# lucieDLE/TMRNet

Measured on AMD Instinct MI355X. Metric: train frames/sec, TMRNet ResNet50 seq=10 LFB=40, higher is better.
Workload: dtype fp32; 1 GPU; C2/C3: TMRNet ResNet50+LSTM+NLBlock train step; model=resnet_lstm (train_only_non-local_pretrained), global_batch=64, clips_per_gpu=64, seq_len=10, lfb_len=40, parallelism=dp1, input_transform=reference train transform (use_flip=1) on device

## Files before the change

include/tmr.h:

```cpp
#ifndef TMR_H_
#define TMR_H_

#ifdef TMR_HOST_ONLY
typedef struct ihipStream_t* hipStream_t;
#else
#include <hip/hip_runtime.h>
#endif
#include <stddef.h>
#include <stdint.h>

#ifdef __cplusplus
extern "C" {
#endif

#define TMR_ABI_VERSION 8

int tmr_abi_version(void);
const char* tmr_last_error(void);
void tmr_clear_error(void);

typedef struct tmr_conv_desc {
  int n, h, w, c;
  int k;
  int r, s, stride, pad;
  int ho, wo;
  int pad_w;
  int x_ld, y_ld;
  int math;
  int max_frames;
  int io;
  int groups;
} tmr_conv_desc;
#define TMR_MATH_F32 0
#define TMR_MATH_BF16 1
#define TMR_IO_X_BF16 1
#define TMR_IO_W_BF16 2
#define TMR_IO_DY_BF16 4
#define TMR_IO_Y_BF16 16
#define TMR_IO_BN_BF16 32
#define TMR_IO_G16 128
#define TMR_IO_WT_BF16 8
#define TMR_IO_ENGINE 256
#define TMR_IO_CLASSES 512
#define TMR_IO_TILES 1024
#define TMR_IO_WT_F32 64

int tmr_conv2d_fwd(const tmr_conv_desc* d, const float* x, const float* w_krsc,
                   const float* bias, float* y, float beta, hipStream_t stream);
int tmr_conv2d_fwd_fused(const tmr_conv_desc* d, const float* x, const float* w_krsc,
                         const float* scale, const float* shift, const float* residual, float* y,
                         int relu, hipStream_t stream);
int tmr_conv2d_fwd_stats_parts(const tmr_conv_desc* d);
int tmr_conv2d_fwd_bnstats(const tmr_conv_desc* d, const float* x, const float* w_krsc, float* y,
                           void* stats, size_t stats_bytes, hipStream_t stream);
int tmr_conv2d_dgrad(const tmr_conv_desc* d, const float* dy, const float* w_krsc, float* dx,
                     float beta, hipStream_t stream);
int tmr_conv2d_dgrad_bnbwd_parts(const tmr_conv_desc* d);
int tmr_conv2d_dgrad_bnbwd(const tmr_conv_desc* d, const float* dy, const float* w_krsc, float* dx,
                           float beta, const float* y, const float* z, const float* scale,
                           const float* shift, const float* mean, int mask, void* parts,
                           size_t parts_bytes, hipStream_t stream);
size_t tmr_conv2d_wgrad_ws_bytes(const tmr_conv_desc* d);
int tmr_conv2d_wgrad(const tmr_conv_desc* d, const float* x, const float* dy, float* dw_oihw,
                     int c_real, float beta, float* ws, size_t ws_bytes, hipStream_t stream);
int tmr_conv2d_wgrad_bnbwd_ok(const tmr_conv_desc* d, const void* x, const void* g, const void* y,
                              const void* dy_out);
int tmr_conv2d_wgrad_bnbwd(const tmr_conv_desc* d, const float* x, const float* g, const float* y,
                           const float* coef, float* dy_out, float* dw_oihw, int c_real,
                           float beta, float* ws, size_t ws_bytes, hipStream_t stream);
long tmr_wgrad_bnbwd_launches(void);
typedef struct tmr_conv_tile {
  int engine;
  int cfg;
  int bm, bn, waves;
  int tapv;
  int splits, kchunk;
  int classes;
} tmr_conv_tile;
int tmr_conv2d_tile(const tmr_conv_desc* d, int view, tmr_conv_tile* out);
int tmr_conv2d_dgrad_bnbwd_acc(const tmr_conv_desc* d, const float* dy, const float* w_krsc,
                               void* dx, float beta, const void* dx_old, int old_bf16,
                               const float* y, const float* z, const float* scale,
                               const float* shift, const float* mean, int mask, void* parts,
                               size_t parts_bytes, hipStream_t stream);
int tmr_gemm_nt(int M, int N, int K, const float* A, int lda, const float* B, int ldb,
                const float* bias, float* C, int ldc, float beta, hipStream_t stream);
int tmr_gemm_nn(int M, int N, int K, const float* A, int lda, const float* B, int ldb, float* C,
                int ldc, float beta, hipStream_t stream);
int tmr_gemm_tn(int M, int N, int K, const float* A, int lda, const float* B, int ldb, float* C,
                int ldc, float beta, hipStream_t stream);

int tmr_weight_oihw_to_krsc(const float* w, float* wk, int k, int c, int r, int s, int cpad,
                            hipStream_t stream);
int tmr_nchw_to_nhwc(const float* x, float* y, int n, int c, int h, int w, int cpad,
                     hipStream_t stream);
int tmr_nhwc_to_nchw(const float* x, float* y, int n, int c, int cstore, int h, int w,
                     hipStream_t stream);
int tmr_crop_normalize(const uint8_t* frames, const int32_t* offsets, float* out, int f, int hin,
                       int win, int seq_len, int crop, float m0, float m1, float m2, float s0,
                       float s1, float s2, hipStream_t stream);

typedef struct tmr_clip_aug {
  int32_t x1, y1;
  int32_t flip;
  int32_t rotate;
  int32_t a[6];
  int32_t jitter;
  int32_t hue_shift;
  float brightness, contrast, saturation;
  int32_t reserved;
} tmr_clip_aug;
int tmr_clip_augment(const uint8_t* frames, const tmr_clip_aug* params, int32_t* lmean, float* out,
                     int f, int hin, int win, int crop, float m0, float m1, float m2, float s0,
                     float s1, float s2, hipStream_t stream);

size_t tmr_bn_ws_bytes(int rows, int c);
int tmr_bn_fwd_stats(const float* y, int rows, int c, const float* gamma, const float* beta,
                     float* running_mean, float* running_var, float momentum, float eps,
                     float* save_mean, float* save_invstd, float* scale, float* shift, void* ws,
                     size_t ws_bytes, hipStream_t stream);
int tmr_bn_finalize(const void* partials, int nparts, int c, const float* gamma, const float* beta,
                    float* running_mean, float* running_var, float momentum, float eps,
                    float* save_mean, float* save_invstd, float* scale, float* shift,
                    hipStream_t stream);
size_t tmr_bn_parts_ws_bytes(int nparts, int c);
int tmr_bn_finalize_ws(const void* partials, int nparts, int c, const float* gamma,
                       const float* beta, float* running_mean, float* running_var, float momentum,
                       float eps, float* save_mean, float* save_invstd, float* scale, float* shift,
                       void* ws, size_t ws_bytes, hipStream_t stream);
int tmr_bn_eval_params(const float* gamma, const float* beta, const float* running_mean,
                       const float* running_var, float eps, int c, float* scale, float* shift,
                       hipStream_t stream);
int tmr_bn_apply(const float* y, const float* scale, const float* shift, const float* residual,
                 float* z, int rows, int c, int relu, hipStream_t stream);
int tmr_bn_apply2(const float* y, const float* scale, const float* shift, const float* yr,
                  const float* rscale, const float* rshift, float* z, int rows, int c, int relu,
                  hipStream_t stream);
int tmr_bn_bwd_maxpool(const float* dyp, const uint8_t* argmax, int n, int h, int w, int ho, int wo,
                       const float* y, const float* scale, const float* shift,
                       const float* save_mean, const float* save_invstd, const float* gamma,
                       float* dy, float* dgamma, float* dbeta, int c, void* ws, size_t ws_bytes,
                       hipStream_t stream);
int tmr_bn_bwd_parts(const float* g, const float* y, const void* parts, int nparts,
                     const float* save_mean, const float* save_invstd, const float* gamma,
                     float* dy, float* dgamma, float* dbeta, int rows, int c, void* ws,
                     size_t ws_bytes, hipStream_t stream);
int tmr_bn_bwd(const float* dz, const float* y, const float* z, const float* scale,
               const float* shift, const float* save_mean, const float* save_invstd,
               const float* gamma, float* dy, float* dres, float* dgamma, float* dbeta, int rows,
               int c, int relu, void* ws, size_t ws_bytes, hipStream_t stream);

int tmr_bn_apply_x(const float* y, const float* scale, const float* shift, const float* residual,
                   void* z, int rows, int c, int relu, int out_bf16, hipStream_t stream);
int tmr_bn_bwd_parts_x(const float* g, const float* y, const void* parts, int nparts,
                       const float* save_mean, const float* save_invstd, const float* gamma,
                       void* dy, float* dgamma, float* dbeta, int rows, int c, void* ws,
                       size_t ws_bytes, int out_bf16, hipStream_t stream);
size_t tmr_bn_parts_coef_offset(int nparts, int c);
int tmr_bn_bwd_x(const float* dz, const float* y, const float* z, const float* scale,
                 const float* shift, const float* save_mean, const float* save_invstd,
                 const float* gamma, void* dy, float* dres, float* dgamma, float* dbeta, int rows,
                 int c, int relu, void* ws, size_t ws_bytes, int out_bf16, hipStream_t stream);
int tmr_bn_bwd_maxpool_x(const float* dyp, const uint8_t* argmax, int n, int h, int w, int ho,
                         int wo, const float* y, const float* scale, const float* shift,
                         const float* save_mean, const float* save_invstd, const float* gamma,
                         void* dy, float* dgamma, float* dbeta, int c, void* ws, size_t ws_bytes,
                         int out_bf16, hipStream_t stream);
// ... 346 lines not shown
```

tmrnet_amd/_lib.py:

```python
import ctypes
import os

import torch

_HERE = os.path.dirname(os.path.abspath(__file__))
LIB_PATH = os.environ.get("TMR_LIB_PATH") or os.path.join(_HERE, "libtmr.so")

P = ctypes.c_void_p
I = ctypes.c_int
L = ctypes.c_long
F = ctypes.c_float
U64 = ctypes.c_uint64
SZ = ctypes.c_size_t


class ConvDesc(ctypes.Structure):
    _fields_ = [(n, ctypes.c_int) for n in
                ("n", "h", "w", "c", "k", "r", "s", "stride", "pad", "ho", "wo", "pad_w",
                 "x_ld", "y_ld", "math", "max_frames", "io", "groups")]


DP = ctypes.POINTER(ConvDesc)


class ConvTile(ctypes.Structure):
    _fields_ = [(n, ctypes.c_int) for n in
                ("engine", "cfg", "bm", "bn", "waves", "tapv", "splits", "kchunk", "classes")]


_NL_FIELDS = ("w1", "b1", "w2", "b2", "w3", "b3", "ln_w", "ln_b", "w4", "b4")


class NLBlockPtrs(ctypes.Structure):
    _fields_ = [(n, ctypes.c_void_p) for n in _NL_FIELDS]


class JpegInfo(ctypes.Structure):
    _fields_ = [("width", ctypes.c_int32), ("height", ctypes.c_int32), ("ncomp", ctypes.c_int32),
                ("sampling", ctypes.c_int32), ("blocks_w", ctypes.c_int32 * 3),
                ("blocks_h", ctypes.c_int32 * 3), ("qt", (ctypes.c_uint16 * 64) * 3),
                ("coef_bytes", ctypes.c_uint64)]


JP = ctypes.POINTER(JpegInfo)


class JpegHuff(ctypes.Structure):
    _fields_ = [("lut", ctypes.c_uint16 * 512), ("fast", ctypes.c_int32 * 512),
                ("maxcode", ctypes.c_int32 * 18), ("valoff", ctypes.c_int32 * 17),
                ("nsym", ctypes.c_int32), ("sym", ctypes.c_uint8 * 256)]


class JpegScanDesc(ctypes.Structure):
    _fields_ = [("bits_off", ctypes.c_uint64), ("tables_off", ctypes.c_uint64),
                ("nbits", ctypes.c_uint32), ("bits_bytes", ctypes.c_uint32),
                ("ntables", ctypes.c_int32), ("ncomp", ctypes.c_int32), ("sampling", ctypes.c_int32),
                ("width", ctypes.c_int32), ("height", ctypes.c_int32),
                ("blocks_w", ctypes.c_int32 * 3), ("blocks_h", ctypes.c_int32 * 3),
                ("mcu_blocks", ctypes.c_int32), ("slot_comp", ctypes.c_uint8 * 8),
                ("dc_table", ctypes.c_uint8 * 4), ("ac_table", ctypes.c_uint8 * 4),
                ("reserved", ctypes.c_uint32 * 2)]


JPEG_HOST_PASS = 4
JPEG_MAX_TABLES = 6
U32 = ctypes.c_uint32

SIGNATURES = {
    "tmr_abi_version": [],
    "tmr_last_error": [],
    "tmr_clear_error": [],
    "tmr_conv2d_fwd": [DP, P, P, P, P, F, P],
    "tmr_conv2d_fwd_fused": [DP, P, P, P, P, P, P, I, P],
    "tmr_conv2d_fwd_stats_parts": [DP],
    "tmr_conv2d_fwd_bnstats": [DP, P, P, P, P, SZ, P],
    "tmr_conv2d_dgrad": [DP, P, P, P, F, P],
    "tmr_conv2d_dgrad_bnbwd_parts": [DP],
    "tmr_conv2d_dgrad_bnbwd": [DP, P, P, P, F, P, P, P, P, P, I, P, SZ, P],
    "tmr_conv2d_wgrad_ws_bytes": [DP],
    "tmr_conv2d_wgrad": [DP, P, P, P, I, F, P, SZ, P],
    "tmr_conv2d_wgrad_bnbwd_ok": [DP, P, P, P, P],
    "tmr_conv2d_wgrad_bnbwd": [DP, P, P, P, P, P, P, I, F, P, SZ, P],
    "tmr_wgrad_bnbwd_launches": [],
    "tmr_conv2d_tile": [DP, I, ctypes.POINTER(ConvTile)],
    "tmr_bn_parts_coef_offset": [I, I],
    "tmr_conv2d_dgrad_bnbwd_acc": [DP, P, P, P, F, P, I, P, P, P, P, P, I, P, SZ, P],
    "tmr_bn_apply_x": [P, P, P, P, P, I, I, I, I, P],
    "tmr_bn_bwd_parts_x": [P, P, P, I, P, P, P, P, P, P, I, I, P, SZ, I, P],
    "tmr_bn_bwd_x": [P, P, P, P, P, P, P, P, P, P, P, P, I, I, I, P, SZ, I, P],
    "tmr_bn_bwd_maxpool_x": [P, P, I, I, I, I, I, P, P, P, P, P, P, P, P, P, I, P, SZ, I, P],
    "tmr_weight_oihw_to_krsc_x": [P, P, I, I, I, I, I, I, P],
    "tmr_weight_oihw_to_crsk_x": [P, P, I, I, I, I, I, P],
    "tmr_bn_apply_dual": [P, P, P, P, P, P, I, I, I, P],
    "tmr_bn_apply2_x": [P, P, P, P, P, P, P, P, I, I, I, P],
    "tmr_bn_apply_bits": [P, P, P, P, P, P, I, I, P],
    "tmr_bn_apply2_bits": [P, P, P, P, P, P, P, P, I, I, P],
    "tmr_maxpool2d_fwd_bn_x": [P, P, P, P, P, I, I, I, I, I, I, I, P],
    "tmr_bn_apply_a16": [P, P, P, P, P, I, I, I, P],
    "tmr_bn_apply2_a16": [P, P, P, P, P, P, P, I, I, I, P],
    "tmr_bn_apply_bits_a16": [P, P, P, P, P, P, I, I, P],
    "tmr_bn_apply2_bits_a16": [P, P, P, P, P, P, P, P, I, I, P],
    "tmr_bn_bwd_a16": [P, P, P, P, P, P, P, P, P, P, P, P, I, I, I, P, SZ, P],
    "tmr_bn_bwd_parts_a16": [P, P, P, I, P, P, P, P, P, P, I, I, P, SZ, P],
    "tmr_bn_bwd_parts_g16": [P, P, P, I, P, P, P, P, P, P, I, I, P, SZ, P],
    "tmr_bn_bwd_g16": [P, P, P, P, P, P, P, P, I, I, P, SZ, P],
    "tmr_weight_layouts_epb": [],
    "tmr_weight_layouts_multi": [P, I, I, P],
    "tmr_bn_bwd_parts_ds_ws_bytes": [I, I, I],
    "tmr_bn_bwd_parts_ds_coef_offset": [I, I, I, I],
    "tmr_bn_bwd_parts_ds": [P, P, P, I, P, P, P, P, P, P, P, P, P, P, P, P, P, I, I, I, P, SZ, P],
    "tmr_bn_apply_bits_dual": [P, P, P, P, P, P, P, I, I, P],
    "tmr_bn_apply2_bits_dual": [P, P, P, P, P, P, P, P, P, I, I, P],
    "tmr_maxpool2d_fwd_bn_dual": [P, P, P, P, P, P, I, I, I, I, I, I, P],
    "tmr_bn_bwd_parts_ds_d16": [P, P, P, I, P, P, P, P, P, P, P, P, P, P, P, P, P, I, I, P, SZ, P],
    "tmr_bn_bwd_maxpool_a16": [P, P, I, I, I, I, I, P, P, P, P, P, P, P, P, P, I, P, SZ, P],
    "tmr_maxpool2d_fwd_bn_a16": [P, P, P, P, P, I, I, I, I, I, I, P],
    "tmr_avgpool_fwd_a16": [P, P, I, I, I, P],
    "tmr_cast_f32_bf16": [P, P, ctypes.c_long, P],
    "tmr_nhwc4_to_bf16x8": [P, P, ctypes.c_long, P],
    "tmr_adam_step_multi": [P, I, ctypes.c_int64, P, P],
    "tmr_resize_ksize": [I, I],
    "tmr_resize_coeffs": [I, I, P, P, I],
    "tmr_resize_tmp_bytes": [I, I, I, I, I],
    "tmr_resize_u8": [P, I, I, I, P, SZ, P, I, I, P, P, I, P, P, I, I, I, P],
    "tmr_resize_u8_boxes": [P, I, I, I, P, P, P, L, P, SZ, P, I, I, P],
    "tmr_margin_ws_bytes": [I, I, I],
    "tmr_margin_boxes": [P, I, I, I, P, SZ, P, P],
    "tmr_margin_mask": [P, I, I, I, P, SZ, P, P],
    "tmr_frame_sums": [P, I, I, I, P, P],
    "tmr_jpeg_probe": [P, SZ, JP],
    "tmr_jpeg_entropy_decode": [P, SZ, JP, P, SZ],
    "tmr_jpeg_ws_bytes": [I, I, I, I],
    "tmr_jpeg_reconstruct": [P, P, I, I, I, I, P, SZ, P, P, I, P],
    "tmr_jpeg_scan_pack": [P, SZ, JP, P, SZ, U64, P, SZ, U64, P],
    "tmr_jpeg_entropy_ws_bytes": [I, U32, I],
    "tmr_jpeg_entropy_decode_device": [P, P, SZ, I, I, I, I, U32, I, P, P, P, SZ, P],
    "tmr_gemm_nt": [I, I, I, P, I, P, I, P, P, I, F, P],
    "tmr_gemm_nn": [I, I, I, P, I, P, I, P, I, F, P],
    "tmr_gemm_tn": [I, I, I, P, I, P, I, P, I, F, P],
    "tmr_weight_oihw_to_krsc": [P, P, I, I, I, I, I, P],
    "tmr_nchw_to_nhwc": [P, P, I, I, I, I, I, P],
    "tmr_nhwc_to_nchw": [P, P, I, I, I, I, I, P],
    "tmr_clip_augment": [P, P, P, P, I, I, I, I, F, F, F, F, F, F, P],
    "tmr_crop_normalize": [P, P, P, I, I, I, I, I, F, F, F, F, F, F, P],
    "tmr_bn_ws_bytes": [I, I],
    "tmr_bn_fwd_stats": [P, I, I, P, P, P, P, F, F, P, P, P, P, P, SZ, P],
    "tmr_bn_finalize": [P, I, I, P, P, P, P, F, F, P, P, P, P, P],
    "tmr_bn_finalize_ws": [P, I, I, P, P, P, P, F, F, P, P, P, P, P, SZ, P],
    "tmr_bn_parts_ws_bytes": [I, I],
    "tmr_bn_eval_params": [P, P, P, P, F, I, P, P, P],
    "tmr_bn_apply": [P, P, P, P, P, I, I, I, P],
    "tmr_bn_apply2": [P, P, P, P, P, P, P, I, I, I, P],
    "tmr_bn_bwd_parts": [P, P, P, I, P, P, P, P, P, P, I, I, P, SZ, P],
    "tmr_bn_bwd_maxpool": [P, P, I, I, I, I, I, P, P, P, P, P, P, P, P, P, I, P, SZ, P],
    "tmr_bn_bwd": [P, P, P, P, P, P, P, P, P, P, P, P, I, I, I, P, SZ, P],
    "tmr_maxpool2d_fwd": [P, P, P, I, I, I, I, I, I, P],
    "tmr_maxpool2d_fwd_bn": [P, P, P, P, P, I, I, I, I, I, I, P],
    "tmr_maxpool2d_bwd": [P, P, P, I, I, I, I, I, I, P],
    "tmr_avgpool_fwd": [P, P, I, I, I, P],
    "tmr_avgpool_bwd": [P, P, I, I, I, P],
    "tmr_splat_gap": [P, P, I, I, I, P],
    "tmr_splat_combine": [P, P, P, P, I, I, I, P],
    "tmr_splat_bwd": [P, P, P, P, I, I, I, P],
    "tmr_splat_bwd_apply": [P, P, P, P, I, I, I, P],
    "tmr_splat_gap_bn": [P, P, P, P, I, I, I, I, P],
    "tmr_splat_att": [P, P, I, I, P],
    "tmr_splat_combine_bn": [P, P, P, P, P, I, I, I, I, P],
    "tmr_splat_bwd_reduce_bn": [P, P, P, P, P, P, P, P, I, I, I, I, P],
    "tmr_splat_bn0_coefs": [P, P, P, P, P, P, P, P, P, I, I, I, P],
    "tmr_splat_bwd_apply_bn": [P, P, P, P, P, P, P, P, P, I, I, I, I, P],
    "tmr_avgpool2d_fwd_a16": [P, P, I, I, I, I, I, I, I, I, I, I, P],
    "tmr_splat_attn_inf": [P, P, P, P, P, P, P, P, I, I, I, P],
    "tmr_splat_combine_a16": [P, P, P, I, I, I, I, I, P],
    "tmr_fill_f32": [P, L, F, P],
    "tmr_seq_last": [P, P, I, I, I, P],
    "tmr_seq_last_bwd": [P, P, P, I, I, I, P],
    "tmr_counters_add": [P, I, ctypes.c_int64, P],
    "tmr_center_cols": [P, I, I, P, P, P],
    "tmr_axpy": [I, F, P, P, P],
    "tmr_avgpool2d_fwd": [P, P, I, I, I, I, I, I, I, I, I, I, P],
    "tmr_avgpool2d_bwd": [P, P, I, I, I, I, I, I, I, I, I, I, P],
    "tmr_col_sum": [P, I, I, I, P, F, P],
    "tmr_dropout_mask": [P, L, F, U64, U64, P],
    "tmr_softmax_max": [P, I, I, P, P, P, P],
    "tmr_ce_sum": [P, P, P, I, I, F, P, P, P, P],
    "tmr_sgd_chunk": [],
    "tmr_sgd_step_multi": [P, I, ctypes.c_int64, P, P],
    "tmr_sgd_step": [P, P, P, L, F, F, F, F, I, I, P],
    "tmr_lfb_index": [P, I, P, I, I, P, P],
    "tmr_lfb_gather": [P, P, P, L, I, P],
    "tmr_layernorm_relu_fwd": [P, P, P, P, P, P, I, I, F, P],
    "tmr_layernorm_relu_bwd": [P, P, P, P, P, P, P, P, P, I, I, P],
    "tmr_residual_mask": [P, P, P, P, L, P],
    "tmr_mask_relu_fwd": [P, P, P, L, P],
    "tmr_mask_relu_bwd": [P, P, P, P, L, P],
    "tmr_mul": [P, P, P, P, L, P],
    "tmr_nl_attn_ws_bytes": [I, I, I],
    "tmr_nl_attn_fwd": [P, P, P, P, P, I, I, I, F, P, SZ, P],
    "tmr_nl_attn_bwd": [P, P, P, P, P, P, P, I, I, I, F, P, SZ, P],
    "tmr_linear_fwd": [P, I, I, I, P, P, P, P],
    "tmr_linear_bwd": [P, P, I, I, I, P, P, P, P, F, P],
    "tmr_nlblock_saved_bytes": [I, I],
    "tmr_nlblock_ws_bytes": [I, I],
    "tmr_nlblock_fwd": [P, P, P, P, I, I, P, P, P, SZ, P, SZ, P],
    "tmr_nlblock_bwd": [P, P, P, P, P, I, I, P, P, SZ, P, P, P, P, SZ, P],
    "tmr_timeconv_saved_bytes": [I, I],
    "tmr_timeconv_ws_bytes": [I, I],
    "tmr_timeconv_fwd": [P, I, I, P, P, P, P, P, P, P, P, SZ, P, SZ, P],
    "tmr_timeconv_wgrad": [P, P, I, I, P, P, P, P, SZ, P, P, P, P, P, P, P, P, SZ, P],
    "tmr_lstm_saved_bytes": [I, I, I],
    "tmr_lstm_ws_bytes": [I, I, I, I],
    "tmr_lstm_fwd": [P, I, I, I, I, P, P, P, P, P, P, P, P, SZ, P, SZ, P],
    "tmr_lstm_bwd": [P, P, I, I, I, I, P, P, P, P, SZ, P, P, P, P, P, P, SZ, P],
    "tmr_lstm_window_ws_bytes": [I, I, I],
    "tmr_lstm_window_fwd": [P, L, P, I, I, I, P, P, P, P, SZ, P],
    "tmr_lstm_sync_status": [P,ctypes.POINTER(ctypes.c_uint), P],
    "tmr_lstm_status_or": [P, P, P],
    "tmr_test_hold_cus": [I, F, P],
    "tmr_dgrad_ws_launches": [],
    "tmr_timeconv_max5_fwd": [P, P, P, P, P, P, I, I, I, P],
    "tmr_timeconv_max5_bwd": [P, P, P, P, P, P, I, I, I, P],
    "tmr_lstm_cell_fwd": [P, I, P, P, P, I, P, P, I, I, P],
    "tmr_lstm_cell_bwd": [P, I, P, P, P, P, P, P, I, P, I, I, P],
}
_RESTYPES = {
    "tmr_last_error": ctypes.c_char_p,
    "tmr_clear_error": None,
    "tmr_conv2d_wgrad_ws_bytes": SZ,
    "tmr_dgrad_ws_launches": L,
    "tmr_wgrad_bnbwd_launches": L,
    "tmr_bn_parts_coef_offset": SZ,
    "tmr_resize_tmp_bytes": SZ,
    "tmr_margin_ws_bytes": SZ,
    "tmr_jpeg_ws_bytes": SZ,
    "tmr_jpeg_entropy_ws_bytes": SZ,
    "tmr_bn_ws_bytes": SZ,
    "tmr_bn_parts_ws_bytes": SZ,
    "tmr_bn_bwd_parts_ds_ws_bytes": SZ,
    "tmr_bn_bwd_parts_ds_coef_offset": SZ,
    "tmr_sgd_chunk": ctypes.c_int64,
    "tmr_nl_attn_ws_bytes": SZ,
    "tmr_nlblock_saved_bytes": SZ,
    "tmr_nlblock_ws_bytes": SZ,
    "tmr_timeconv_saved_bytes": SZ,
    "tmr_timeconv_ws_bytes": SZ,
    "tmr_lstm_saved_bytes": SZ,
    "tmr_lstm_ws_bytes": SZ,
    "tmr_lstm_window_ws_bytes": SZ,
}

_lib = None


def lib():
    global _lib
    if _lib is None:
        if not os.path.exists(LIB_PATH):
            raise RuntimeError(
                "libtmr.so not found at %s: build it with `make` or "
                "`python -c 'import __graft_entry__ as g; g.build()'` (no CPU fallback exists)"
                % LIB_PATH)
        h = ctypes.CDLL(LIB_PATH)
        for name, args in SIGNATURES.items():
            fn = getattr(h, name)
            fn.argtypes = args
            fn.restype = _RESTYPES.get(name, ctypes.c_int)
        _lib = h
    return _lib


def exported_symbols():
    return list(SIGNATURES)


def _conv(a):
    if isinstance(a, torch.Tensor):
        return ctypes.c_void_p(a.data_ptr())
    return a


def stream_ptr(device=None):
    return ctypes.c_void_p(torch.cuda.current_stream(device).cuda_stream)


def call(name, *args):
    fn = getattr(lib(), name)
    rc = fn(*[_conv(a) for a in args])
    if rc != 0:
        raise RuntimeError("%s failed (%d): %s" % (name, rc, lib().tmr_last_error().decode()))
    return rc


def query(name, *args):
    h = lib()
    h.tmr_clear_error()
    fn = getattr(h, name)
    v = fn(*[_conv(a) for a in args])
    err = h.tmr_last_error()
    if (_RESTYPES.get(name, ctypes.c_int) is ctypes.c_int and v < 0) or err:
        raise RuntimeError("%s failed (%d): %s" % (name, v, (err or b"").decode()))
    return v
```

tmrnet_amd/csrc/gemm16_dgrad_f32.hip:

```cpp
#include "gemm16_kernel.h"

namespace tmrg {
template int launch_gemm16<MODE_DGRAD, 1>(const GemmArgs& a, int splits, hipStream_t st);
}
```

tmrnet_amd/csrc/gemm16_kernel.h:

```cpp
#pragma once
#include "gemm16_select.h"
#include <cstring>
#include <type_traits>

namespace tmrg {

typedef short s16x4_t __attribute__((ext_vector_type(4)));
typedef short s16x8_t __attribute__((ext_vector_type(8)));
#define TMR_LDS_AS __attribute__((address_space(3)))

__device__ __forceinline__ void glds16(__amdgpu_buffer_rsrc_t r, unsigned char* dst, uint32_t voff) {
  __builtin_amdgcn_raw_ptr_buffer_load_lds(r, (TMR_LDS_AS void*)dst, 16, voff, 0, 0, 0);
}

template <int R>
__device__ __forceinline__ int mn_swz(int k) {
  return R >= 128 ? ((k & 3) << 2) : (((k >> 1) & 1) << 2);
}

__device__ __forceinline__ void store_g8(const GemmArgs& a, long off, const float (&v)[8]) {
  if (a.g16) {
    uint32_t w[4];
#pragma unroll
    for (int e = 0; e < 4; ++e)
      w[e] = (__float_as_uint(v[2 * e]) >> 16) | (__float_as_uint(v[2 * e + 1]) & 0xffff0000u);
    *reinterpret_cast<uint4*>(reinterpret_cast<__bf16*>(a.C) + off) = make_uint4(w[0], w[1], w[2], w[3]);
  } else {
    *reinterpret_cast<float4*>(a.C + off) = make_float4(v[0], v[1], v[2], v[3]);
    *reinterpret_cast<float4*>(a.C + off + 4) = make_float4(v[4], v[5], v[6], v[7]);
  }
}

__device__ __forceinline__ void load_old8(const GemmArgs& a, long off, uint4& c0, uint4& c1,
                                          bool c16) {
  const void* base = a.Cold ? a.Cold : (const void*)a.C;
  if (c16) {
    c0 = *reinterpret_cast<const uint4*>(reinterpret_cast<const __bf16*>(base) + off);
  } else {
    c0 = *reinterpret_cast<const uint4*>(reinterpret_cast<const float*>(base) + off);
    c1 = *reinterpret_cast<const uint4*>(reinterpret_cast<const float*>(base) + off + 4);
  }
}
__device__ __forceinline__ void load_old8(const GemmArgs& a, long off, uint4& c0, uint4& c1) {
  load_old8(a, off, c0, c1, a.cold16);
}
__device__ __forceinline__ void unpack_old8(const uint4& c0, const uint4& c1, float (&old)[8],
                                            bool c16) {
  if (c16) {
    const uint32_t u[4] = {c0.x, c0.y, c0.z, c0.w};
#pragma unroll
    for (int e = 0; e < 4; ++e) {
      old[2 * e] = __uint_as_float(u[e] << 16);
      old[2 * e + 1] = __uint_as_float(u[e] & 0xffff0000u);
    }
  } else {
    const uint32_t u[8] = {c0.x, c0.y, c0.z, c0.w, c1.x, c1.y, c1.z, c1.w};
#pragma unroll
    for (int e = 0; e < 8; ++e) old[e] = __uint_as_float(u[e]);
  }
}
__device__ __forceinline__ void unpack_old8(const GemmArgs& a, const uint4& c0, const uint4& c1,
                                            float (&old)[8]) {
  unpack_old8(c0, c1, old, a.cold16);
}

template <int EPF>
struct EpiForm {
  __device__ __forceinline__ static bool bn16(const GemmArgs& a) {
    return EPF == 1 ? true : (EPF == 2 ? false : a.bn16 != 0);
  }
  __device__ __forceinline__ static bool mask1(const GemmArgs& a) { return EPF == 2 ? false : a.bn_mask == 1; }
  __device__ __forceinline__ static bool mask3(const GemmArgs& a) { return EPF == 1 ? false : a.bn_mask == 3; }
  __device__ __forceinline__ static bool cold16(const GemmArgs& a) {
    return EPF == 1 ? true : (EPF == 2 ? false : a.cold16 != 0);
  }
};
inline int epi_form(const GemmArgs& a) {
  if (a.bn16 && a.bn_mask != 3 && (a.beta == 0.f || a.cold16)) return 1;
  if (!a.bn16 && a.bn_mask != 1 && !a.cold16) return 2;
  return 0;
}

#ifndef TMR_EPI_DEPTH
#define TMR_EPI_DEPTH 3
#endif
#ifndef TMR_EPI_LATE
#define TMR_EPI_LATE 0
#endif
#ifndef TMR_EPI_TOPUP
#define TMR_EPI_TOPUP 0
#endif
#ifndef TMR_EPI_TOPUP_F16
#define TMR_EPI_TOPUP_F16 5
#endif
#ifndef TMR_EPI_TOPUP_F32
#define TMR_EPI_TOPUP_F32 2
#endif
#ifndef TMR_EPI_FORMS
#define TMR_EPI_FORMS 1
#endif
#ifndef TMR_EPI_DEPTH_F16
#define TMR_EPI_DEPTH_F16 TMR_EPI_DEPTH
#endif
#ifndef TMR_EPI_LATE_F
#define TMR_EPI_LATE_F 0
#endif
template <int BM, int BN, int WM, int WN, int SMEMB, int DEPTH = TMR_EPI_DEPTH, int TOP = 0,
          int EPF = 0>
struct LdsBnbwd {
  using Form = EpiForm<EPF>;
  static constexpr int NT = 64 * WM * WN;
  static constexpr int LDC = BN + 4;
  static constexpr int CG = BN / 8;
  static constexpr int RPP = NT / CG;
  static constexpr int WR = BM / WM;
  static constexpr int RC0 = (SMEMB / 4 / LDC) / WR * WR;
  static constexpr int RCH = RC0 < WR ? WR : (RC0 < BM ? RC0 : BM);
  static constexpr int NCH = (BM + RCH - 1) / RCH;
  static constexpr int PC = (RCH + RPP - 1) / RPP;
  static constexpr int NR = NCH * PC;
  static constexpr int D = NR < DEPTH ? NR : DEPTH;
  static constexpr int DT = NR < D + TOP ? NR : D + TOP;
  static_assert(NT % CG == 0, "epilogue row partition");

  struct In {
    uint4 y0, y1, z0, z1, c0, c1;
    uint32_t bits;
    long off;
    bool ok;
  };

  __device__ __forceinline__ static void issue(const GemmArgs& a, int t, int m0, int n0, In& x) {
    const int etid = threadIdx.x;
    const int cg = etid % CG, rsub = etid / CG;
    const int ci = t / PC, j = t % PC;
    const int rr = rsub + j * RPP;
    const int nrow = (BM - ci * RCH) < RCH ? (BM - ci * RCH) : RCH;
    const int col = n0 + 8 * cg;
    const int row = m0 + ci * RCH + rr;
    x.ok = rr < nrow && col < a.N && row < a.M;
    long pix = row;
    if (x.ok && a.osy != 0) {
      const uint32_t n = fdiv((uint32_t)row, a.dHW);
      const uint32_t rem = row - n * a.dHW.d;
      const uint32_t y = fdiv(rem, a.dW);
      const uint32_t xx = rem - y * a.dW.d;
      pix = ((long)n * a.oH + (long)y * a.osy + a.oyc) * a.oW + (long)xx * a.osx + a.oxc;
    }
    x.off = pix * a.ldc + col;
    if (!x.ok) return;
    const long off = x.off;
    if (Form::bn16(a)) {
      x.y0 = *reinterpret_cast<const uint4*>(reinterpret_cast<const __bf16*>(a.bn_y) + off);
      if (Form::mask1(a))
        x.z0 = *reinterpret_cast<const uint4*>(reinterpret_cast<const __bf16*>(a.bn_z) + off);
    } else {
      x.y0 = *reinterpret_cast<const uint4*>(a.bn_y + off);
      x.y1 = *reinterpret_cast<const uint4*>(a.bn_y + off + 4);
      if (Form::mask1(a)) {
        x.z0 = *reinterpret_cast<const uint4*>(a.bn_z + off);
        x.z1 = *reinterpret_cast<const uint4*>(a.bn_z + off + 4);
      }
    }
    if (Form::mask3(a)) x.bits = reinterpret_cast<const uint32_t*>(a.bn_z)[off >> 5];
    if (a.beta != 0.f) load_old8(a, off, x.c0, x.c1, Form::cold16(a));
  }

  __device__ __forceinline__ static void prefetch(const GemmArgs& a, int m0, int n0, In (&pf)[DT]) {
#pragma unroll
    for (int t = 0; t < D; ++t) issue(a, t, m0, n0, pf[t]);
  }

  template <int TM, int TN>
  __device__ __forceinline__ static void run(const GemmArgs& a, floatx16 (&acc)[TM][TN], float* lds,
                                             int m0, int n0, In (&pf)[DT]) {
    int etid = threadIdx.x;
    asm volatile("" : "+v"(etid));
    const int lane = etid & 63, wave = etid >> 6;
    const int wm = wave / WN, wn = wave % WN;
    const int l31 = lane & 31, hh = lane >> 5;
    const int cg = etid % CG, rsub = etid / CG;
    const int col = n0 + 8 * cg;
    const bool okc = col < a.N;
    float mu[8], bsc[8], bsh[8], cs[8], cq[8];
#pragma unroll
    for (int e = 0; e < 8; ++e) {
      const int c = okc ? col + e : 0;
      mu[e] = okc ? a.bn_mean[c] : 0.f;
      bsc[e] = (okc && a.bn_mask == 2) ? a.bn_sc[c] : 0.f;
      bsh[e] = (okc && a.bn_mask == 2) ? a.bn_sh[c] : (a.bn_mask == 0 ? 1.f : 0.f);
      cs[e] = 0.f;
      cq[e] = 0.f;
    }
    const bool has_beta = a.beta != 0.f;
#pragma unroll
    for (int ci = 0; ci < NCH; ++ci) {
      __syncthreads();
      const int wr0 = wm * WR;
      if (wr0 >= ci * RCH && wr0 < ci * RCH + RCH) {
#pragma unroll
        for (int i = 0; i < TM; ++i)
#pragma unroll
          for (int j = 0; j < TN; ++j)
#pragma unroll
            for (int r = 0; r < 16; ++r) {
              const int row = wr0 - ci * RCH + 32 * i + (r & 3) + 8 * (r >> 2) + 4 * hh;
              lds[row * LDC + wn * (BN / WN) + 32 * j + l31] = acc[i][j][r];
            }
      }
      __syncthreads();
      if (ci == 0) {
#pragma unroll
        for (int t = D; t < DT; ++t) issue(a, t, m0, n0, pf[t]);
      }
#pragma unroll
      for (int j = 0; j < PC; ++j) {
        const int t = ci * PC + j;
        In& x = pf[t % DT];
        if (x.ok) {
          const long off = x.off;
          float yv[8], zv[8], old[8];
          if (Form::bn16(a)) {
            const uint32_t yu[4] = {x.y0.x, x.y0.y, x.y0.z, x.y0.w};
#pragma unroll
            for (int e = 0; e < 4; ++e) {
              yv[2 * e] = __uint_as_float(yu[e] << 16);
              yv[2 * e + 1] = __uint_as_float(yu[e] & 0xffff0000u);
            }
            if (Form::mask1(a)) {
              const uint32_t zu[4] = {x.z0.x, x.z0.y, x.z0.z, x.z0.w};
#pragma unroll
              for (int e = 0; e < 4; ++e) {
                zv[2 * e] = __uint_as_float(zu[e] << 16);
                zv[2 * e + 1] = __uint_as_float(zu[e] & 0xffff0000u);
              }
            }
          } else {
            const uint32_t yu[8] = {x.y0.x, x.y0.y, x.y0.z, x.y0.w, x.y1.x, x.y1.y, x.y1.z, x.y1.w};
#pragma unroll
            for (int e = 0; e < 8; ++e) yv[e] = __uint_as_float(yu[e]);
            if (Form::mask1(a)) {
              const uint32_t zu[8] = {x.z0.x, x.z0.y, x.z0.z, x.z0.w, x.z1.x, x.z1.y, x.z1.z, x.z1.w};
#pragma unroll
              for (int e = 0; e < 8; ++e) zv[e] = __uint_as_float(zu[e]);
            }
          }
          if (Form::mask3(a)) {
            const uint32_t b8 = x.bits >> (off & 31);
#pragma unroll
            for (int e = 0; e < 8; ++e) zv[e] = ((b8 >> e) & 1u) ? 1.f : 0.f;
          } else if (!Form::mask1(a)) {
#pragma unroll
            for (int e = 0; e < 8; ++e) zv[e] = 0.f;
          }
          if (has_beta) {
            unpack_old8(x.c0, x.c1, old, Form::cold16(a));
          } else {
#pragma unroll
            for (int e = 0; e < 8; ++e) old[e] = 0.f;
          }
          const int rr = rsub + j * RPP;
          const float4 a0 = *reinterpret_cast<const float4*>(lds + rr * LDC + 8 * cg);
          const float4 a1 = *reinterpret_cast<const float4*>(lds + rr * LDC + 8 * cg + 4);
          const float av[8] = {a0.x, a0.y, a0.z, a0.w, a1.x, a1.y, a1.z, a1.w};
          float v[8];
#pragma unroll
          for (int e = 0; e < 8; ++e) {
            float tv = fmaf(a.beta, old[e], av[e]);
            const bool keep = zv[e] + fmaf(yv[e], bsc[e], bsh[e]) > 0.f;
            tv = keep ? tv : 0.f;
            if (a.g16) tv = bf16_rne(tv);
            v[e] = tv;
            cs[e] += tv;
            cq[e] = fmaf(tv, yv[e] - mu[e], cq[e]);
          }
          store_g8(a, off, v);
        }
        if (t + DT < NR) issue(a, t + DT, m0, n0, x);
      }
    }
    __syncthreads();
    float* red = lds;
#pragma unroll
    for (int e = 0; e < 8; ++e) {
      red[(rsub * BN + 8 * cg + e) * 2] = cs[e];
      red[(rsub * BN + 8 * cg + e) * 2 + 1] = cq[e];
    }
    __syncthreads();
    for (int c = etid; c < BN; c += NT) {
      float t0 = 0.f, t1 = 0.f;
      for (int q = 0; q < RPP; ++q) {
        t0 += red[(q * BN + c) * 2];
        t1 += red[(q * BN + c) * 2 + 1];
      }
      if (n0 + c < a.N) a.bn_part[(long)(m0 / BM) * a.part_ld + n0 + c] = make_float2(t0, t1);
    }
  }
};

template <int BM, int BN, int WM, int WN, int TM, int TN>
__device__ __forceinline__ void epilogue_lds_bnbwd(const GemmArgs& a, floatx16 (&acc)[TM][TN],
                                                   float* lds, int lds_floats, int m0, int n0) {
  constexpr int NT = 64 * WM * WN;
  constexpr int LDC = BN + 4;
  constexpr int CG = BN / 8;
  constexpr int RPP = NT / CG;
  static_assert(NT % CG == 0, "threads per column group");
  int etid = threadIdx.x;
  asm volatile("" : "+v"(etid));
  const int lane = etid & 63, wave = etid >> 6;
  const int wm = wave / WN, wn = wave % WN;
  const int l31 = lane & 31, hh = lane >> 5;
  const int cg = etid % CG, rsub = etid / CG;
  const int col = n0 + 8 * cg;
  const bool okc = col < a.N;
  float mu[8], bsc[8], bsh[8], cs[8], cq[8];
#pragma unroll
  for (int e = 0; e < 8; ++e) {
    const int c = okc ? col + e : 0;
    mu[e] = okc ? a.bn_mean[c] : 0.f;
    bsc[e] = (okc && a.bn_mask == 2) ? a.bn_sc[c] : 0.f;
    bsh[e] = (okc && a.bn_mask == 2) ? a.bn_sh[c] : (a.bn_mask == 0 ? 1.f : 0.f);
    cs[e] = 0.f;
    cq[e] = 0.f;
  }
  const bool has_beta = a.beta != 0.f;
  const int rchunk = min(BM, (lds_floats / LDC) / (BM / WM) * (BM / WM));
  for (int r0 = 0; r0 < BM; r0 += rchunk) {
    __syncthreads();
    const int wr0 = wm * (BM / WM);
    if (wr0 >= r0 && wr0 < r0 + rchunk) {
#pragma unroll
      for (int i = 0; i < TM; ++i)
#pragma unroll
        for (int j = 0; j < TN; ++j)
#pragma unroll
          for (int r = 0; r < 16; ++r) {
            const int row = wr0 - r0 + 32 * i + (r & 3) + 8 * (r >> 2) + 4 * hh;
            lds[row * LDC + wn * (BN / WN) + 32 * j + l31] = acc[i][j][r];
          }
    }
    __syncthreads();
    const int nrow = min(rchunk, BM - r0);
    for (int rr = rsub; rr < nrow; rr += RPP) {
      const int row = m0 + r0 + rr;
      const bool ok = okc && row < a.M;
      long pix = row;
      if (ok && a.osy != 0) {
        const uint32_t n = fdiv((uint32_t)row, a.dHW);
        const uint32_t rem = row - n * a.dHW.d;
        const uint32_t y = fdiv(rem, a.dW);
        const uint32_t x = rem - y * a.dW.d;
        pix = ((long)n * a.oH + (long)y * a.osy + a.oyc) * a.oW + (long)x * a.osx + a.oxc;
      }
      const long off = pix * a.ldc + col;
      float yv[8], zv[8], old[8];
      if (ok) {
        if (a.bn16) {
          const uint4 yw = *reinterpret_cast<const uint4*>(reinterpret_cast<const __bf16*>(a.bn_y) + off);
          const uint32_t yu[4] = {yw.x, yw.y, yw.z, yw.w};
#pragma unroll
          for (int e = 0; e < 4; ++e) {
            yv[2 * e] = __uint_as_float(yu[e] << 16);
            yv[2 * e + 1] = __uint_as_float(yu[e] & 0xffff0000u);
          }
          if (a.bn_mask == 1) {
            const uint4 zw = *reinterpret_cast<const uint4*>(reinterpret_cast<const __bf16*>(a.bn_z) + off);
            const uint32_t zu[4] = {zw.x, zw.y, zw.z, zw.w};
#pragma unroll
            for (int e = 0; e < 4; ++e) {
              zv[2 * e] = __uint_as_float(zu[e] << 16);
              zv[2 * e + 1] = __uint_as_float(zu[e] & 0xffff0000u);
            }
          }
        } else {
          const float4 y0 = *reinterpret_cast<const float4*>(a.bn_y + off);
          const float4 y1 = *reinterpret_cast<const float4*>(a.bn_y + off + 4);
          yv[0] = y0.x; yv[1] = y0.y; yv[2] = y0.z; yv[3] = y0.w;
          yv[4] = y1.x; yv[5] = y1.y; yv[6] = y1.z; yv[7] = y1.w;
          if (a.bn_mask == 1) {
            const float4 z0 = *reinterpret_cast<const float4*>(a.bn_z + off);
            const float4 z1 = *reinterpret_cast<const float4*>(a.bn_z + off + 4);
            zv[0] = z0.x; zv[1] = z0.y; zv[2] = z0.z; zv[3] = z0.w;
            zv[4] = z1.x; zv[5] = z1.y; zv[6] = z1.z; zv[7] = z1.w;
          }
        }
        if (a.bn_mask == 3) {
          const uint32_t wrd = reinterpret_cast<const uint32_t*>(a.bn_z)[off >> 5];
          const uint32_t b8 = wrd >> (off & 31);
#pragma unroll
          for (int e = 0; e < 8; ++e) zv[e] = ((b8 >> e) & 1u) ? 1.f : 0.f;
        } else if (a.bn_mask != 1) {
#pragma unroll
          for (int e = 0; e < 8; ++e) zv[e] = 0.f;
        }
        if (has_beta) {
          uint4 c0, c1;
          load_old8(a, off, c0, c1);
          unpack_old8(a, c0, c1, old);
        } else {
#pragma unroll
          for (int e = 0; e < 8; ++e) old[e] = 0.f;
        }
        const float4 a0 = *reinterpret_cast<const float4*>(lds + rr * LDC + 8 * cg);
        const float4 a1 = *reinterpret_cast<const float4*>(lds + rr * LDC + 8 * cg + 4);
        const float av[8] = {a0.x, a0.y, a0.z, a0.w, a1.x, a1.y, a1.z, a1.w};
        float v[8];
#pragma unroll
        for (int e = 0; e < 8; ++e) {
          float t = fmaf(a.beta, old[e], av[e]);
          const bool keep = zv[e] + fmaf(yv[e], bsc[e], bsh[e]) > 0.f;
          t = keep ? t : 0.f;
          if (a.g16) t = bf16_rne(t);
          v[e] = t;
          cs[e] += t;
          cq[e] = fmaf(t, yv[e] - mu[e], cq[e]);
        }
        store_g8(a, off, v);
      }
    }
  }
  __syncthreads();
  float* red = lds;
#pragma unroll
  for (int e = 0; e < 8; ++e) {
    red[(rsub * BN + 8 * cg + e) * 2] = cs[e];
    red[(rsub * BN + 8 * cg + e) * 2 + 1] = cq[e];
  }
  __syncthreads();
  for (int c = etid; c < BN; c += NT) {
    float t0 = 0.f, t1 = 0.f;
    for (int q = 0; q < RPP; ++q) {
      t0 += red[(q * BN + c) * 2];
      t1 += red[(q * BN + c) * 2 + 1];
    }
    if (n0 + c < a.N) a.bn_part[(long)(m0 / BM) * a.part_ld + n0 + c] = make_float2(t0, t1);
  }
}

typedef float f32x4_t __attribute__((ext_vector_type(4)));

template <int BM, int BN, int WM, int WN, int NST>
constexpr int occ16() {
  return (WM * WN >= 16 || (WM * WN == 8 && (BM * BN <= 128 * 128 || NST == 1))) ? 4 : 2;
}

template <int MODE, int BM, int BN, int WM, int WN, int TAPV, int PIPE, int F32, int NST, int EPF = 0,
          int INF16 = 0, int BNW = 0>
__device__ __forceinline__ void gemm16_body(const GemmArgs& a, const int bid, const int split) {
  constexpr uint32_t ES = F32 ? 4u : 2u;
  constexpr int EPC = 16 / ES;
  constexpr int BK = 128 / ES;
  constexpr int NW = WM * WN;
  constexpr int TM = BM / WM / 32, TN = BN / WN / 32;
  constexpr bool MN = (MODE == MODE_WGRAD);
  constexpr int ABYTES = BM * 128, BBYTES = BN * 128, STAGE = ABYTES + BBYTES;
  constexpr int NIA = ABYTES / (1024 * NW), NIB = BBYTES / (1024 * NW);
  static_assert(NIA >= 1 && NIB >= 1 && NIA * 1024 * NW == ABYTES && NIB * 1024 * NW == BBYTES,
                "LDS-DMA pieces per wave");
  static_assert(TM >= 1 && TN >= 1, "wave tile");
  static_assert(!MN || (BM >= 64 && BN >= 64), "reduction-major images need >= 64 columns");
  constexpr int CPRA = BM * (int)ES / 16, CPRB = BN * (int)ES / 16;
  using Frag = typename std::conditional<F32 != 0, f32x4_t, bf16x8>::type;
  constexpr int EPI = WM * BN * 2 * 4;
  static_assert(NST == 2 || (NST == 1 && MODE != MODE_WGRAD), "one-stage form: FWD / DGRAD");
  static_assert(!BNW || (MN && F32 != 0 && PIPE == 1), "dY-producing form: the fp32 WGRAD view");
  static_assert(!BNW || ((64 * NW) % (2 * (BM / 4)) == 0), "dY-producing form: fixed piece columns");
  constexpr int LDSROWB = (BN + 4) * (BM / WM) * 4, LDSFULL = (BN + 4) * BM * 4;
  constexpr int LDSNEED = MODE != MODE_DGRAD ? 0 : (LDSFULL <= 70 * 1024 ? LDSFULL : LDSROWB);
  constexpr int SMEM1 = STAGE > EPI ? (STAGE > LDSNEED ? STAGE : LDSNEED) : (EPI > LDSNEED ? EPI : LDSNEED);
  constexpr int SMEM2 = 2 * STAGE > EPI ? 2 * STAGE : EPI;
  constexpr int SMEM = NST == 1 ? SMEM1 : (SMEM2 > LDSNEED ? SMEM2 : LDSNEED);
  constexpr int CFBYTES = BNW == 2 ? 3 * BM * 4 : 0;
  __shared__ __attribute__((aligned(1024))) unsigned char smem[SMEM + CFBYTES];

  const int tid = threadIdx.x;
  const int lane = tid & 63;
  const int wave = __builtin_amdgcn_readfirstlane(tid >> 6);
  const int wm = wave / WN, wn = wave % WN;
  const int l31 = lane & 31, hh = lane >> 5;

  const int nnt = (a.N + BN - 1) / BN;
  const int m0 = (bid / nnt) * BM;
  const int n0 = (bid % nnt) * BN;

  int kbeg = 0, kend = a.K;
  if (MODE == MODE_WGRAD) {
    kbeg = split * a.kchunk;
    kend = min(a.K, kbeg + a.kchunk);
  }
  const int ntiles = kend > kbeg ? (kend - kbeg + BK - 1) / BK : 0;

  const __amdgpu_buffer_rsrc_t rA = make_rsrc(a.A, a.Abytes);
  const __amdgpu_buffer_rsrc_t rB = make_rsrc(a.B, a.Bbytes);
  const int cmask = (1 << a.log2C) - 1;

  auto kc_row = [&](int q) { return 8 * (wave + NW * q) + (lane >> 3); };
  auto kc_chunk = [&](int q) { return (lane & 7) ^ ((kc_row(q) >> 1) & 7); };

  uint32_t apix[MN ? 1 : NIA];
  int ay[MN ? 1 : NIA], ax[MN ? 1 : NIA], ach[MN ? 1 : NIA];
  bool aok[MN ? 1 : NIA];
  uint32_t aco[MN ? NIA : 1];
  int akr[MN ? NIA : 1];
  bool acok[MN ? NIA : 1];
  if constexpr (!MN) {
#pragma unroll
    for (int q = 0; q < NIA; ++q) {
      const int m = m0 + kc_row(q);
      aok[q] = m < a.M;
      const uint32_t mm = aok[q] ? (uint32_t)m : 0u;
      const uint32_t n = fdiv(mm, a.dHW);
      const uint32_t rem = mm - n * a.dHW.d;
      const uint32_t y = fdiv(rem, a.dW);
      const uint32_t x = rem - y * a.dW.d;
      ay[q] = (int)y * a.sy;
      ax[q] = (int)x * a.sx;
      apix[q] = (uint32_t)(((int)n * a.Hs + ay[q]) * a.Ws + ax[q]) * (uint32_t)a.lds * ES;
      ach[q] = EPC * kc_chunk(q);
    }
  } else {
#pragma unroll
    for (int q = 0; q < NIA; ++q) {
      const int s = 64 * (wave + NW * q) + lane;
      const int k = s / CPRA;
      const int ch = (s % CPRA) ^ (F32 ? (k & 1) << 3 : mn_swz<BM>(k));
      const int i = m0 + EPC * ch;
      akr[q] = k;
      acok[q] = i < a.M;
      aco[q] = (uint32_t)i * ES;
    }
// ... 116 lines not shown
          const int k = kb + bch[q];
          int tap = tapB, co = coB + bch[q], rs = rsB;
          if (TAPV) {
            tap = k >> a.log2C;
            co = k & cmask;
            int ri, si;
            tap_split(a, tap, ri, si);
            rs = (a.wr0 + a.wst * ri) * a.wS + (a.ws0 + a.wst * si);
          }
          const bool ok = bok[q] && k < kend && tap < a.ntaps;
          const uint32_t off = brow[q] + (uint32_t)((rs << a.log2C) + co) * ES;
          glds16(rB, Bs + 1024 * (wave + NW * q), ok ? off : OOB);
        }
      }
    } else {
#pragma unroll
      for (int q = 0; q < NIA; ++q) {
        const int qs = FOLDQ ? 0 : q;
        const int m = kb + akr_of(q);
        const bool ok = acok[qs] && m < kend;
        const uint32_t off = (uint32_t)m * (uint32_t)a.ldb * ES + aco[qs];
        glds16(rA, As + 1024 * (wave + NW * q), ok ? off : OOB);
        if constexpr (BNW != 0)
          ypc[q] = __builtin_bit_cast(f32x4_t, __builtin_amdgcn_raw_buffer_load_b128(rY, ok ? off : OOB, 0, 0));
      }
#pragma unroll
      for (int q = 0; q < NIB; ++q) {
        const int qs = FOLDQ ? 0 : q;
        const int m = kb + bkr_of(q);
        const uint32_t mm = m < kend ? (uint32_t)m : 0u;
        const uint32_t n = fdiv(mm, a.dHW);
        const uint32_t rem = mm - n * a.dHW.d;
        const uint32_t y = fdiv(rem, a.dW);
        const uint32_t x = rem - y * a.dW.d;
        const int ys = (int)y * a.sy + bdy[qs], xs = (int)x * a.sx + bdx[qs];
        const bool ok = m < kend && bok[qs] && (unsigned)ys < (unsigned)a.Hs &&
                        (unsigned)xs < (unsigned)a.Ws;
        const uint32_t off = (uint32_t)(((int)n * a.Hs + ys) * a.Ws + xs) * (uint32_t)a.lds * ES + bco[qs];
        glds16(rB, Bs + 1024 * (wave + NW * q), ok ? off : OOB);
      }
    }
  };

  const int kx = (l31 >> 1) & 7;
  const int tg = lane >> 4, tq = (lane >> 2) & 3, tp = lane & 3;
  auto tr_frag = [&](const unsigned char* img, int R, int swz, int cb, int s) -> bf16x8 {
    const int col = cb + 16 * (tg & 1) + 4 * tp;
    const int k0 = 16 * s + 8 * (tg >> 1) + tq;
    const uint32_t cbyte = (uint32_t)((((col >> 3) ^ swz) << 4) + (col & 7) * 2);
    const s16x4_t v0 = __builtin_amdgcn_ds_read_tr16_b64_v4i16(
        (TMR_LDS_AS s16x4_t*)(img + k0 * R * 2 + cbyte));
    const s16x4_t v1 = __builtin_amdgcn_ds_read_tr16_b64_v4i16(
        (TMR_LDS_AS s16x4_t*)(img + (k0 + 4) * R * 2 + cbyte));
    const s16x8_t w = __builtin_shufflevector(v0, v1, 0, 1, 2, 3, 4, 5, 6, 7);
    return __builtin_bit_cast(bf16x8, w);
  };
  const int swzA = mn_swz<BM>(tq), swzB = mn_swz<BN>(tq);
  auto mn_frag32 = [&](const unsigned char* img, int R, int cb, int s) -> f32x4_t {
    const int col = cb + l31;
    const uint32_t cbyte = (uint32_t)((((col >> 2) ^ (hh << 3)) << 4) + (col & 3) * 4);
    f32x4_t v;
#pragma unroll
    for (int t = 0; t < 4; ++t)
      v[t] = *reinterpret_cast<const float*>(img + (8 * s + 2 * t + hh) * R * 4 + cbyte);
    return v;
  };

  floatx16 acc[TM][TN];
#pragma unroll
  for (int i = 0; i < TM; ++i)
#pragma unroll
    for (int j = 0; j < TN; ++j)
#pragma unroll
      for (int r = 0; r < 16; ++r) acc[i][j][r] = 0.f;

  constexpr bool LDSEPI = MODE == MODE_DGRAD && LDSROWB <= SMEM;
  constexpr bool PRE = LDSEPI && NW < 8;
  constexpr int LATED = EPF != 0 ? TMR_EPI_LATE_F : TMR_EPI_LATE;
  constexpr bool LATE = LDSEPI && NW == 8 && LDSNEED == LDSFULL && LATED > 0;
  using Epi = LdsBnbwd<BM, BN, WM, WN, SMEM,
                      PRE ? (EPF == 1 ? TMR_EPI_DEPTH_F16 : TMR_EPI_DEPTH) : (LATE ? 0 : 1),
                      PRE ? (EPF == 1 ? TMR_EPI_TOPUP_F16 : (EPF == 2 ? TMR_EPI_TOPUP_F32 : TMR_EPI_TOPUP))
                          : (LATE ? LATED : 0),
                      EPF>;
  typename Epi::In pf[(PRE || LATE) ? Epi::DT : 1];
  if constexpr (PRE) {
    if (a.bn_part != nullptr) Epi::prefetch(a, m0, n0, pf);
  }

  const int arow0 = wm * (BM / WM) + l31;
  const int brow0 = wn * (BN / WN) + l31;
  auto frags = [&](int buf, int s, Frag (&av)[TM], Frag (&bv)[TN]) {
    const unsigned char* As = smem + buf * STAGE;
    const unsigned char* Bs = As + ABYTES;
    const int ch = (2 * s + hh) ^ kx;
#pragma unroll
    for (int i = 0; i < TM; ++i) {
      if constexpr (!MN)
        av[i] = *reinterpret_cast<const Frag*>(As + (arow0 + 32 * i) * 128 + (ch << 4));
      else if constexpr (!F32)
        av[i] = tr_frag(As, BM, swzA, wm * (BM / WM) + 32 * i, s);
      else
        av[i] = mn_frag32(As, BM, wm * (BM / WM) + 32 * i, s);
    }
#pragma unroll
    for (int j = 0; j < TN; ++j) {
      if constexpr (!MN)
        bv[j] = *reinterpret_cast<const Frag*>(Bs + (brow0 + 32 * j) * 128 + (ch << 4));
      else if constexpr (!F32)
        bv[j] = tr_frag(Bs, BN, swzB, wn * (BN / WN) + 32 * j, s);
      else
        bv[j] = mn_frag32(Bs, BN, wn * (BN / WN) + 32 * j, s);
    }
  };
  auto mfmas = [&](const Frag (&av)[TM], const Frag (&bv)[TN]) {
    if (PIPE) __builtin_amdgcn_s_setprio(1);
    if constexpr (F32) {
#pragma unroll
      for (int t = 0; t < 4; ++t)
#pragma unroll
        for (int i = 0; i < TM; ++i)
#pragma unroll
          for (int j = 0; j < TN; ++j)
            acc[i][j] = __builtin_amdgcn_mfma_f32_32x32x2f32(av[i][t], bv[j][t], acc[i][j], 0, 0, 0);
    } else {
#pragma unroll
      for (int i = 0; i < TM; ++i)
#pragma unroll
        for (int j = 0; j < TN; ++j)
          acc[i][j] = __builtin_amdgcn_mfma_f32_32x32x16_bf16(av[i], bv[j], acc[i][j], 0, 0, 0);
    }
    if (PIPE) __builtin_amdgcn_s_setprio(0);
  };
  constexpr int KSTEPS = BK / (2 * EPC);
  static_assert(KSTEPS == 4, "four k-steps per k-tile (the PIPE 1 schedule)");
  auto compute = [&](int buf) {
#pragma unroll
    for (int s = 0; s < KSTEPS; ++s) {
      Frag av[TM], bv[TN];
      frags(buf, s, av, bv);
      mfmas(av, bv);
    }
  };

  f32x4_t dyo[BNW == 1 ? NIA : 1];
  auto bnw_apply = [&](int kt, int buf) {
    const int kb = kbeg + kt * BK;
    unsigned char* As = smem + buf * STAGE;
#pragma unroll
    for (int q = 0; q < NIA; ++q) {
      f32x4_t* pc = reinterpret_cast<f32x4_t*>(As + 1024 * (wave + NW * q) + 16 * lane);
      const int m = kb + akr_of(q);
      const bool ok = acok[FOLDQ ? 0 : q] && m < kend;
      const f32x4_t gv = *pc, yv = ypc[q];
      f32x4_t o;
#pragma unroll
      for (int e = 0; e < 4; ++e) o[e] = ok ? fmaf(cfA[e], gv[e], fmaf(cfB[e], yv[e], cfC[e])) : 0.f;
      *pc = o;
      if constexpr (BNW == 1) dyo[q] = o;
    }
  };
  auto bnw_store = [&](int kt) {
    const int kb = kbeg + kt * BK;
    const unsigned char* As = smem + (kt & 1) * STAGE;
#pragma unroll
    for (int q = 0; q < NIA; ++q) {
      const int m = kb + akr_of(q);
      const bool ok = acok[FOLDQ ? 0 : q] && m < kend;
      const uint32_t off = (uint32_t)m * (uint32_t)a.ldb * ES + aco[FOLDQ ? 0 : q];
      f32x4_t o;
      if constexpr (BNW == 1) o = dyo[q];
      else o = *reinterpret_cast<const f32x4_t*>(As + 1024 * (wave + NW * q) + 16 * lane);
      __builtin_amdgcn_raw_buffer_store_b128(__builtin_bit_cast(u32x4_t, o), rD, ok ? off : OOB, 0, 0);
    }
  };

  auto bnw_coefs = [&]() {
    const f32x4_t* cf = reinterpret_cast<const f32x4_t*>(smem + SMEM) + ((int)(aco[0] / 16) - m0 / 4);
    cfA = cf[0]; cfB = cf[BM / 4]; cfC = cf[2 * (BM / 4)];
  };

  if (ntiles > 0 && PIPE == 0) {
    stage(0, 0);
    for (int kt = 0; kt < ntiles; ++kt) {
      asm volatile("s_waitcnt vmcnt(0)" ::: "memory");
      __syncthreads();
      if (kt + 1 < ntiles) stage(kt + 1, (kt + 1) & 1);
      compute(kt & 1);
    }
  } else if (NST == 1 && ntiles > 0) {
    for (int kt = 0; kt < ntiles; ++kt) {
      if (kt > 0) __syncthreads();
      stage(kt, 0);
      asm volatile("s_waitcnt vmcnt(0)" ::: "memory");
      __syncthreads();
      compute(0);
    }
  } else if (ntiles > 0) {
    stage(0, 0);
    for (int kt = 0; kt < ntiles; ++kt) {
      if constexpr (BNW == 2) bnw_coefs();
      asm volatile("s_waitcnt vmcnt(0)" ::: "memory");
      if constexpr (BNW != 0) bnw_apply(kt, kt & 1);
      __syncthreads();
      const int buf = kt & 1;
      Frag a0[TM], b0[TN], a1[TM], b1[TN];
      frags(buf, 0, a0, b0);
      if constexpr (BNW != 0) {
        if (dyw) bnw_store(kt);
      }
      if (kt + 1 < ntiles) stage(kt + 1, buf ^ 1);
      frags(buf, 1, a1, b1);
      mfmas(a0, b0);
      frags(buf, 2, a0, b0);
      mfmas(a1, b1);
      frags(buf, 3, a1, b1);
      mfmas(a0, b0);
      mfmas(a1, b1);
    }
  }
  __syncthreads();

  if constexpr (LDSEPI) {
    if (a.bn_part != nullptr) {
      if constexpr (PRE) {
        Epi::run(a, acc, reinterpret_cast<float*>(smem), m0, n0, pf);
      } else if constexpr (LATE) {
        Epi::prefetch(a, m0, n0, pf);
        Epi::run(a, acc, reinterpret_cast<float*>(smem), m0, n0, pf);
      } else
        epilogue_lds_bnbwd<BM, BN, WM, WN, TM, TN>(a, acc, reinterpret_cast<float*>(smem), SMEM / 4,
                                                    m0, n0);
      return;
    }
  }
  epilogue_batched<MODE, BM, BN, WM, WN, TM, TN, INF16>(a, acc, reinterpret_cast<float*>(smem), m0,
                                                        n0, split);
}

template <int MODE, int BM, int BN, int WM, int WN, int TAPV, int PIPE = 1, int F32 = 0, int NST = 2,
          int EPF = 0>
__global__ __launch_bounds__(64 * WM * WN, (occ16<BM, BN, WM, WN, NST>()))
void gemm16_kernel(const GemmArgs a) {
  int bid, split;
  xcd_work(bid, split);
  gemm16_body<MODE, BM, BN, WM, WN, TAPV, PIPE, F32, NST, EPF>(a, bid, split);
}

template <int BM, int BN, int WM, int WN>
__global__ __launch_bounds__(64 * WM * WN, (occ16<BM, BN, WM, WN, 2>()))
void gemm16_wgrad_bnbwd_kernel(const GemmArgs a) {
  int bid, split;
  xcd_work(bid, split);
  gemm16_body<MODE_WGRAD, BM, BN, WM, WN, 0, 1, 1, 2, 0, 0, 1>(a, bid, split);
}

template <int BM, int BN, int WM, int WN>
__global__ __launch_bounds__(64 * WM * WN, (occ16<BM, BN, WM, WN, 2>()))
void gemm16_wgrad_bnbwd16_kernel(const GemmArgs a) {
  static_assert(WM * WN == 16, "the sixteen-wave form");
  int bid, split;
  xcd_work(bid, split);
  gemm16_body<MODE_WGRAD, BM, BN, WM, WN, 0, 1, 1, 2, 0, 0, 2>(a, bid, split);
}

__device__ __forceinline__ void par_tile(const GemmPar& p, int w, int& cls, int& t) {
  const int ch = w / PAR_G, off = w - ch * PAR_G;
  int base = 0, prev = 0;
  cls = 0;
  t = 1 << 30;
  for (int n = p.n; n > 0; --n) {
    const int tn = (p.c[n - 1].tiles + PAR_G - 1) / PAR_G;
    const int span = n * (tn - prev);
    if (ch < base + span) {
      const int q = ch - base;
      cls = q % n;
      t = (prev + q / n) * PAR_G + off;
      return;
    }
    base += span;
    prev = tn;
  }
}

template <int BM, int BN, int WM, int WN, int F32, int EPF = 0>
__global__ __launch_bounds__(64 * WM * WN, (occ16<BM, BN, WM, WN, 2>()))
void gemm16_par_kernel(const GemmPar p) {
  int w, split;
  xcd_work(w, split);
  int cls, t;
  par_tile(p, w, cls, t);
  cls = __builtin_amdgcn_readfirstlane(cls);
  t = __builtin_amdgcn_readfirstlane(t);
  if (t >= p.c[cls].tiles) return;
  GemmArgs a = p.a;
  const ParClass& c = p.c[cls];
  auto own = [](auto v) {
    asm volatile("" : "+s"(v));
    return v;
  };
  a.M = own(c.M);
  a.K = own(c.K);
  a.ntaps = own(c.ntaps);
  a.tapS = own(c.tapS);
  a.tapSinv = own(c.tapSinv);
  a.oy0 = own(c.oy0);
  a.ox0 = own(c.ox0);
  a.wr0 = own(c.wr0);
  a.ws0 = own(c.ws0);
  a.oyc = own(c.oyc);
  a.oxc = own(c.oxc);
  a.dHW = FastDiv{own(c.dHW.d), own(c.dHW.m), own(c.dHW.s)};
  a.dW = FastDiv{own(c.dW.d), own(c.dW.m), own(c.dW.s)};
  a.bn_part = own(c.bn_part);
  gemm16_body<MODE_DGRAD, BM, BN, WM, WN, 0, 1, F32, 2, EPF>(a, t, 0);
}

}
#include "gemm16_ws.h"
namespace tmrg {

template <int MODE, int BM, int BN, int WM, int WN, int F32>
int launch16_cfg(const GemmArgs& a, bool tapv, dim3 grid, hipStream_t st) {
  const dim3 blk(64 * WM * WN);
  if constexpr (MODE == MODE_FWD && F32 == 0) {
    if (a.c16 && a.scale) return launch16_inf16<BM, BN, WM, WN>(a, tapv, grid, st);
  }
  constexpr int kmax = 64;
  if constexpr (MODE == MODE_FWD && F32 == 0 && WM * WN == 4 &&
                ((BM == 128 && BN == 128) || (BM == 256 && BN == 64))) {
    if (!tapv && a.K > 0 && a.K <= kmax) {
      hipLaunchKernelGGL((gemm16_kernel<MODE, BM, BN, WM, WN, 0, 1, F32, 1>), grid, blk, 0, st, a);
      TMR_CHECK_LAUNCH("gemm16_kernel (one stage)");
      return 0;
    }
  }
  if constexpr (MODE == MODE_FWD && F32 == 0 && BM == 256 && BN == 256) {
    if (!tapv && a.K > 0 && a.K <= kmax) {
      const dim3 g2((unsigned)(cdiv(a.M, 256) * cdiv(a.N, 128)), grid.y, 1);
      hipLaunchKernelGGL((gemm16_kernel<MODE, 256, 128, 4, 2, 0, 1, F32, 1>), g2, dim3(512), 0, st, a);
      TMR_CHECK_LAUNCH("gemm16_kernel (one stage, 256x128)");
      return 0;
    }
  }
  constexpr bool FORMS = MODE == MODE_DGRAD && TMR_EPI_FORMS &&
                         (WM * WN == 4 || (WM * WN == 8 && TMR_EPI_LATE_F > 0));
// ... 166 lines not shown
```

tmrnet_amd/csrc/gemm16_select.h:

```cpp
#pragma once
#include "gemm_kernel.h"

namespace tmrg {

struct Cfg16 { int bm, bn, waves; };
constexpr Cfg16 kCfgs16[] = {{256, 256, 8}, {256, 128, 8}, {128, 128, 4}, {256, 64, 4},
                              {64, 256, 4}, {64, 64, 4},
                              {256, 256, 16},
                              {128, 128, 8}};

inline bool use32(const GemmArgs& a, int mode) {
  if (a.prec != TMR_MATH_F32 || a.sab) return false;
  if (mode == MODE_DGRAD) return a.wt != 0;
  if (!a.dma32) return false;
  if ((((uintptr_t)a.A | (uintptr_t)a.B) & 15) != 0) return false;
  if (mode == MODE_WGRAD)
    return a.M % 4 == 0 && a.log2C >= 2 && a.ldb % 4 == 0 && a.lds % 4 == 0 && a.N % 4 == 0;
  return a.lds % 4 == 0 && a.ldb % 4 == 0 && a.log2C >= 2 && (a.ntaps != 1 || a.K % 4 == 0);
}

inline bool use16(const GemmArgs& a, int mode) {
  if (a.prec == TMR_MATH_F32) return use32(a, mode);
  if (a.prec != TMR_MATH_BF16 || a.sab != 3) return false;
  if (mode == MODE_DGRAD && !a.wt) return false;
// ... 13 lines not shown
  if (forced >= 0 && forced < (int)(sizeof(kCfgs16) / sizeof(kCfgs16[0]))) return forced;
  int cfg;
  if (f32 && mode == MODE_WGRAD) {
    if (M <= 64) return (N <= 64 || N >= 512) ? 5 : 4;
    if (N <= 64) return 5;
    if (M >= 256 && N >= 256 && 2.0 * M * N * K >= 100e9) return 6;
    return 7;
  }
  if (f32 && M >= 256 && mode == MODE_DGRAD && N >= 512) {
    static const int wide = env_int("TMR_DGRAD32_WIDE_CFG", 7);
    return cfg16_tiles(M, N, wide) >= 256 ? wide : 2;
  }
  if (f32 && M >= 256 && mode == MODE_FWD && N == 128)
    return cfg16_tiles(M, N, 7) >= 256 ? 7 : 2;
  if (mode == MODE_WGRAD) {
    if (M <= 64) cfg = N <= 64 ? 5 : (N >= 512 ? 4 : 2);
    else if (N <= 64) cfg = 3;
    else cfg = (M >= 256 && N >= 1024 && K * cfg16_tiles(M, N, 6) >= (1L << 21)) ? 6 : 7;
  } else if (N <= 64) {
    cfg = M >= 256 ? 3 : 5;
  } else if (mode == MODE_FWD && N >= 256 && M >= 256) {
    cfg = 6;
  } else {
    cfg = 2;
  }
  if (mode != MODE_WGRAD && cfg16_tiles(M, N, cfg) < (f32 && cfg == 6 ? 224 : 256)) {
    for (const int c2 : {1, 2, 5}) {
      if ((long)kCfgs16[c2].bm * kCfgs16[c2].bn >= (long)kCfgs16[cfg].bm * kCfgs16[cfg].bn ||
          cfg16_tiles(M, N, c2) <= cfg16_tiles(M, N, cfg))
        continue;
      cfg = c2;
      if (cfg16_tiles(M, N, cfg) >= 256) break;
    }
  }
  return cfg;
}

inline bool tapv16(const GemmArgs& a, int mode, bool f32) {
  const int bk = f32 ? 32 : 64;
  return mode != MODE_WGRAD && a.ntaps > 1 && ((1 << a.log2C) % bk) != 0;
}

inline int gemm_tile_bm(const GemmArgs& a, int mode) {
  return use16(a, mode) ? kCfgs16[pick_cfg16(a.M, a.N, a.K, mode, a.prec == TMR_MATH_F32)].bm
                        : kCfgs[pick_cfg(a.M, a.N, a.K, mode)].bm;
}
inline long gemm_tiles(const GemmArgs& a, int mode) {
  return use16(a, mode) ? cfg16_tiles(a.M, a.N, pick_cfg16(a.M, a.N, a.K, mode, a.prec == TMR_MATH_F32))
                        : cfg_tiles(a.M, a.N, pick_cfg(a.M, a.N, a.K, mode));
}

constexpr int PAR_MAX = 4;
struct ParClass {
  int M, K, ntaps, tapS, tapSinv, oy0, ox0, wr0, ws0, oyc, oxc, tiles;
  FastDiv dHW, dW;
  float2* bn_part;
};
struct GemmPar {
  GemmArgs a;
  ParClass c[PAR_MAX];
  int n;
};
constexpr int PAR_G = 64;

extern long g_dgrad_ws_launches;

template <int F32>
int launch_gemm16_par(const GemmArgs* as, int n, hipStream_t st);
extern template int launch_gemm16_par<0>(const GemmArgs*, int, hipStream_t);
extern template int launch_gemm16_par<1>(const GemmArgs*, int, hipStream_t);
template <int MODE, int F32>
int launch_gemm16(const GemmArgs& a, int splits, hipStream_t st);
extern template int launch_gemm16<MODE_FWD, 0>(const GemmArgs&, int, hipStream_t);
extern template int launch_gemm16<MODE_FWD, 1>(const GemmArgs&, int, hipStream_t);
extern template int launch_gemm16<MODE_DGRAD, 0>(const GemmArgs&, int, hipStream_t);
extern template int launch_gemm16<MODE_DGRAD, 1>(const GemmArgs&, int, hipStream_t);
extern template int launch_gemm16<MODE_WGRAD, 0>(const GemmArgs&, int, hipStream_t);
extern template int launch_gemm16<MODE_WGRAD, 1>(const GemmArgs&, int, hipStream_t);

inline bool wgrad_bnbwd_cfg(int cfg) { return cfg == 4 || cfg == 5 || cfg == 6 || cfg == 7; }
int launch_gemm16_wgrad_bnbwd(const GemmArgs& a, int splits, hipStream_t st);
extern long g_wgrad_bnbwd_launches;

template <int BM, int BN, int WM, int WN>
int launch16_inf16(const GemmArgs& a, bool tapv, dim3 grid, hipStream_t st);
extern template int launch16_inf16<256, 128, 4, 2>(const GemmArgs&, bool, dim3, hipStream_t);
extern template int launch16_inf16<128, 128, 2, 2>(const GemmArgs&, bool, dim3, hipStream_t);
extern template int launch16_inf16<256, 64, 4, 1>(const GemmArgs&, bool, dim3, hipStream_t);
extern template int launch16_inf16<64, 256, 1, 4>(const GemmArgs&, bool, dim3, hipStream_t);
extern template int launch16_inf16<128, 128, 4, 2>(const GemmArgs&, bool, dim3, hipStream_t);
extern template int launch16_inf16<64, 64, 2, 2>(const GemmArgs&, bool, dim3, hipStream_t);
extern template int launch16_inf16<256, 256, 2, 4>(const GemmArgs&, bool, dim3, hipStream_t);
extern template int launch16_inf16<256, 256, 4, 4>(const GemmArgs&, bool, dim3, hipStream_t);

}
```

tmrnet_amd/csrc/gemm16_ws.h:

```cpp
#pragma once

namespace tmrg {

#ifndef TMR_DGRAD_WS
#define TMR_DGRAD_WS 1
#endif
constexpr int WS_NWG = 256;
#ifndef TMR_WS_EXP
#define TMR_WS_EXP 0
#endif

__device__ __forceinline__ void ws_barrier() {
  asm volatile("s_waitcnt lgkmcnt(0)" ::: "memory");
  __builtin_amdgcn_s_barrier();
  asm volatile("" ::: "memory");
}

template <int F32, int NKC, int MSK, int BETA>
__global__ __launch_bounds__(512) void dgrad_ws_kernel(const GemmArgs a) {
  constexpr bool BN16 = !F32, C16 = !F32, G16 = !F32;
  constexpr int BM = 128, BN = 128, NW = 4, WN = 2;
  constexpr uint32_t ES = F32 ? 4u : 2u;
  constexpr int EPC = 16 / ES, BK = 128 / ES;
  constexpr int TM = 2, TN = 2;
  constexpr int ABYTES = BM * 128, STAGE = 2 * ABYTES;
  constexpr int NIA = ABYTES / (1024 * NW);
  constexpr int NST = 3;
  constexpr int LDC = BN;
  constexpr int STG = BM * LDC * 4;
  constexpr int CG = BN / 8, RPP = 256 / CG, NR = BM / RPP;
  constexpr int R = NR / NKC;
  static_assert(NR == 8 && R * NKC == NR, "consumer row groups");
  static_assert(RPP * BN * 8 <= STAGE, "the partial sums fit a stage");
  using Frag = typename std::conditional<F32 != 0, f32x4_t, bf16x8>::type;
  __shared__ __attribute__((aligned(1024))) unsigned char smem[NST * STAGE + STG];
  float* const stg = reinterpret_cast<float*>(smem + NST * STAGE);
  auto scol = [](int row, int c) { return c ^ (((row >> 2) & 1) << 5); };

  const int tid = threadIdx.x;
  const int wave = __builtin_amdgcn_readfirstlane(tid >> 6);
  const int nnt = a.N / BN;
  const int mt = (a.M + BM - 1) / BM;
  const int xcd = blockIdx.x & 7, slot = blockIdx.x >> 3;
  const int mlo = (int)((long)mt * xcd / 8), mhi = (int)((long)mt * (xcd + 1) / 8);
  const int nt = slot % nnt, ms = slot / nnt, mstr = (WS_NWG / 8) / nnt;
  const int ntl = mhi - mlo > ms ? (mhi - mlo - ms + mstr - 1) / mstr : 0;
  const int n0 = nt * BN;
  const int nk = (a.K + BK - 1) / BK;
  const int kpg = nk / NKC;

  if (wave < NW) {
    const int lane = tid & 63;
    const int wm = wave / WN, wn = wave % WN;
    const int l31 = lane & 31, hh = lane >> 5;
    const __amdgpu_buffer_rsrc_t rA = make_rsrc(a.A, a.Abytes);
    const __amdgpu_buffer_rsrc_t rB = make_rsrc(a.B, a.Bbytes);
    int prow[NIA], pch[NIA];
    uint32_t boff[NIA];
#pragma unroll
    for (int q = 0; q < NIA; ++q) {
      prow[q] = 8 * (wave + NW * q) + (lane >> 3);
      pch[q] = EPC * ((lane & 7) ^ ((prow[q] >> 1) & 7));
      boff[q] = (uint32_t)(n0 + prow[q]) * (uint32_t)a.ldbt * ES + (uint32_t)pch[q] * ES;
    }
    auto stage_q = [&](int m0, int kt, int buf, int q) {
      const int kb = kt * BK;
      unsigned char* As = smem + buf * STAGE;
      unsigned char* Bs = As + ABYTES;
      const int m = m0 + prow[q];
      const bool ok = m < a.M && kb + pch[q] < a.K;
      const uint32_t off = (uint32_t)m * (uint32_t)a.lds * ES + (uint32_t)(kb + pch[q]) * ES;
      glds16(rA, As + 1024 * (wave + NW * q), ok ? off : OOB);
      const bool okb = kb + pch[q] < a.K;
      glds16(rB, Bs + 1024 * (wave + NW * q), okb ? boff[q] + (uint32_t)kb * ES : OOB);
    };
    auto stage = [&](int m0, int kt, int buf) {
#pragma unroll
      for (int q = 0; q < NIA; ++q) stage_q(m0, kt, buf, q);
    };
    const int kx = (l31 >> 1) & 7;
    const int arow0 = wm * (BM / 2) + l31;
    const int brow0 = wn * (BN / WN) + l31;
    auto frags = [&](int buf, int s, Frag (&av)[TM], Frag (&bv)[TN]) {
      const unsigned char* As = smem + buf * STAGE;
      const unsigned char* Bs = As + ABYTES;
      const int ch = (2 * s + hh) ^ kx;
#pragma unroll
      for (int i = 0; i < TM; ++i)
        av[i] = *reinterpret_cast<const Frag*>(As + (arow0 + 32 * i) * 128 + (ch << 4));
#pragma unroll
      for (int j = 0; j < TN; ++j)
        bv[j] = *reinterpret_cast<const Frag*>(Bs + (brow0 + 32 * j) * 128 + (ch << 4));
    };
    floatx16 acc[TM][TN];
#pragma unroll
    for (int i = 0; i < TM; ++i)
#pragma unroll
      for (int j = 0; j < TN; ++j)
#pragma unroll
        for (int r = 0; r < 16; ++r) acc[i][j][r] = 0.f;
    auto mfmas = [&](const Frag (&av)[TM], const Frag (&bv)[TN]) {
      if constexpr (TMR_WS_EXP == 2) {
        asm volatile("" ::"v"(av[0]), "v"(bv[0]), "v"(av[TM - 1]), "v"(bv[TN - 1]));
        return;
      }
      __builtin_amdgcn_s_setprio(1);
      if constexpr (F32) {
#pragma unroll
        for (int t = 0; t < 4; ++t)
#pragma unroll
          for (int i = 0; i < TM; ++i)
#pragma unroll
            for (int j = 0; j < TN; ++j)
              acc[i][j] = __builtin_amdgcn_mfma_f32_32x32x2f32(av[i][t], bv[j][t], acc[i][j], 0, 0, 0);
      } else {
#pragma unroll
        for (int i = 0; i < TM; ++i)
#pragma unroll
          for (int j = 0; j < TN; ++j)
            acc[i][j] = __builtin_amdgcn_mfma_f32_32x32x16_bf16(av[i], bv[j], acc[i][j], 0, 0, 0);
      }
      __builtin_amdgcn_s_setprio(0);
    };
    const int ng = ntl * nk;
    auto stage_g = [&](int G) {
      const int ti = G / nk;
      stage((mlo + ms + ti * mstr) * BM, G - ti * nk, G % NST);
    };

    if (ntl > 0) {
      stage_g(0);
      if (ng > 1) stage_g(1);
      int g = 0;
      for (int i = 0; i < ntl; ++i) {
        for (int kt = 0; kt < nk; ++kt) {
          if (g + 1 < ng)
            asm volatile("s_waitcnt vmcnt(%0)" ::"n"(2 * NIA) : "memory");
          else
            asm volatile("s_waitcnt vmcnt(0)" ::: "memory");
          ws_barrier();
          const int buf = g % NST;
          Frag a0[TM], b0[TN], a1[TM], b1[TN];
          frags(buf, 0, a0, b0);
          if (g + 2 < ng) stage_g(g + 2);
          frags(buf, 1, a1, b1);
          mfmas(a0, b0);
          frags(buf, 2, a0, b0);
          mfmas(a1, b1);
          frags(buf, 3, a1, b1);
          mfmas(a0, b0);
          mfmas(a1, b1);
          ++g;
        }
        ws_barrier();
#pragma unroll
        for (int i2 = 0; i2 < TM; ++i2)
#pragma unroll
          for (int j = 0; j < TN; ++j)
#pragma unroll
            for (int r = 0; r < 16; ++r) {
              const int row = wm * (BM / 2) + 32 * i2 + (r & 3) + 8 * (r >> 2) + 4 * hh;
              stg[row * LDC + scol(row, wn * (BN / WN) + 32 * j + l31)] = acc[i2][j][r];
              acc[i2][j][r] = 0.f;
            }
        ws_barrier();
      }
    }
    ws_barrier();
    ws_barrier();
    return;
  }

  const int etid = tid - 64 * NW;
  const int cg = etid % CG, rsub = etid / CG;
  const int col = n0 + 8 * cg;
  float mu[8], bsc[8], bsh[8], cs[8], cq[8];
#pragma unroll
  for (int e = 0; e < 8; ++e) {
    mu[e] = a.bn_mean[col + e];
    bsc[e] = MSK == 2 ? a.bn_sc[col + e] : 0.f;
    bsh[e] = MSK == 2 ? a.bn_sh[col + e] : (MSK == 0 ? 1.f : 0.f);
    cs[e] = 0.f;
    cq[e] = 0.f;
  }
  const uint32_t span = G16 ? a.Cbytes / 2u : a.Cbytes / 4u;
  constexpr uint32_t ey = BN16 ? 2u : 4u, eo = C16 ? 2u : 4u, ec = G16 ? 2u : 4u;
  auto rsrc = [](const void* p, uint32_t bytes) {
    return __builtin_amdgcn_make_buffer_rsrc(const_cast<void*>(p), (short)0, (int)bytes, 0x00020000);
  };
  const __amdgpu_buffer_rsrc_t rY = rsrc(a.bn_y, span * ey);
  const __amdgpu_buffer_rsrc_t rZ = rsrc(a.bn_z ? (const void*)a.bn_z : (const void*)a.bn_y,
                                         MSK == 3 ? (span + 31u) / 32u * 4u : span * ey);
  const __amdgpu_buffer_rsrc_t rO = rsrc(a.Cold ? a.Cold : (const void*)a.C, span * eo);
  const __amdgpu_buffer_rsrc_t rC = rsrc(a.C, span * ec);
  auto ld16 = [](__amdgpu_buffer_rsrc_t r, uint32_t off) {
    return __builtin_bit_cast(uint4, __builtin_amdgcn_raw_buffer_load_b128(r, off, 0, 0));
  };
  struct In {
    uint4 y0, y1, z0, z1, c0, c1;
    uint32_t bits;
    uint32_t off;
    bool ok;
  };
  In pf[NR];
  auto issue = [&](int m0, int j, In& x, bool live) {
    const int row = m0 + rsub + j * RPP;
    x.ok = live && row < a.M;
    x.off = (uint32_t)row * (uint32_t)a.ldc + (uint32_t)col;
    const uint32_t o = x.off;
    x.y0 = ld16(rY, x.ok ? o * ey : OOB);
    if constexpr (!BN16) x.y1 = ld16(rY, x.ok ? o * ey + 16u : OOB);
    if constexpr (MSK == 1) {
      x.z0 = ld16(rZ, x.ok ? o * ey : OOB);
      if constexpr (!BN16) x.z1 = ld16(rZ, x.ok ? o * ey + 16u : OOB);
    }
    if constexpr (MSK == 3)
      x.bits = __builtin_amdgcn_raw_buffer_load_b32(rZ, x.ok ? (o >> 5) * 4u : OOB, 0, 0);
    if constexpr (BETA != 0) {
      x.c0 = ld16(rO, x.ok ? o * eo : OOB);
      if constexpr (!C16) x.c1 = ld16(rO, x.ok ? o * eo + 16u : OOB);
    }
  };
  auto consume = [&](const In& x, int j) {
    float yv[8], zv[8], old[8];
    if constexpr (BN16) {
      const uint32_t yu[4] = {x.y0.x, x.y0.y, x.y0.z, x.y0.w};
#pragma unroll
      for (int e = 0; e < 4; ++e) {
        yv[2 * e] = __uint_as_float(yu[e] << 16);
        yv[2 * e + 1] = __uint_as_float(yu[e] & 0xffff0000u);
      }
      if constexpr (MSK == 1) {
        const uint32_t zu[4] = {x.z0.x, x.z0.y, x.z0.z, x.z0.w};
#pragma unroll
        for (int e = 0; e < 4; ++e) {
          zv[2 * e] = __uint_as_float(zu[e] << 16);
          zv[2 * e + 1] = __uint_as_float(zu[e] & 0xffff0000u);
        }
      }
    } else {
      const uint32_t yu[8] = {x.y0.x, x.y0.y, x.y0.z, x.y0.w, x.y1.x, x.y1.y, x.y1.z, x.y1.w};
#pragma unroll
      for (int e = 0; e < 8; ++e) yv[e] = __uint_as_float(yu[e]);
      if constexpr (MSK == 1) {
        const uint32_t zu[8] = {x.z0.x, x.z0.y, x.z0.z, x.z0.w, x.z1.x, x.z1.y, x.z1.z, x.z1.w};
#pragma unroll
        for (int e = 0; e < 8; ++e) zv[e] = __uint_as_float(zu[e]);
      }
    }
    if constexpr (MSK == 3) {
      const uint32_t b8 = x.bits >> (x.off & 31u);
#pragma unroll
      for (int e = 0; e < 8; ++e) zv[e] = ((b8 >> e) & 1u) ? 1.f : 0.f;
    } else if constexpr (MSK != 1) {
#pragma unroll
      for (int e = 0; e < 8; ++e) zv[e] = 0.f;
    }
    if constexpr (BETA != 0) {
      unpack_old8(x.c0, x.c1, old, C16);
    } else {
#pragma unroll
      for (int e = 0; e < 8; ++e) old[e] = 0.f;
    }
    const int rr = rsub + j * RPP;
    const float* srow = stg + rr * LDC + scol(rr, 8 * cg);
    const float4 a0 = *reinterpret_cast<const float4*>(srow);
    const float4 a1 = *reinterpret_cast<const float4*>(srow + 4);
    const float av[8] = {a0.x, a0.y, a0.z, a0.w, a1.x, a1.y, a1.z, a1.w};
    float v[8];
#pragma unroll
    for (int e = 0; e < 8; ++e) {
      float tv = fmaf(a.beta, old[e], av[e]);
      const bool keep = zv[e] + fmaf(yv[e], bsc[e], bsh[e]) > 0.f;
      tv = keep ? tv : 0.f;
      if constexpr (G16) tv = bf16_rne(tv);
      v[e] = tv;
      const float s1 = cs[e] + tv, s2 = fmaf(tv, yv[e] - mu[e], cq[e]);
      cs[e] = x.ok ? s1 : cs[e];
      cq[e] = x.ok ? s2 : cq[e];
    }
    const uint32_t so = x.ok ? x.off * ec : OOB;
    if constexpr (G16) {
      uint32_t w[4];
#pragma unroll
      for (int e = 0; e < 4; ++e)
        w[e] = (__float_as_uint(v[2 * e]) >> 16) | (__float_as_uint(v[2 * e + 1]) & 0xffff0000u);
      const u32x4_t q = {w[0], w[1], w[2], w[3]};
      __builtin_amdgcn_raw_buffer_store_b128(q, rC, so, 0, 0);
    } else {
      const u32x4_t q0 = {__float_as_uint(v[0]), __float_as_uint(v[1]), __float_as_uint(v[2]),
                          __float_as_uint(v[3])};
      const u32x4_t q1 = {__float_as_uint(v[4]), __float_as_uint(v[5]), __float_as_uint(v[6]),
                          __float_as_uint(v[7])};
      __builtin_amdgcn_raw_buffer_store_b128(q0, rC, so, 0, 0);
      __builtin_amdgcn_raw_buffer_store_b128(q1, rC, x.ok ? so + 16u : OOB, 0, 0);
    }
  };
  float* red = nullptr;
  auto put_red = [&](int gl) {
    red = reinterpret_cast<float*>(smem + (gl % NST) * STAGE);
#pragma unroll
    for (int e = 0; e < 8; ++e) {
      red[(rsub * BN + 8 * cg + e) * 2] = cs[e];
      red[(rsub * BN + 8 * cg + e) * 2 + 1] = cq[e];
      cs[e] = 0.f;
      cq[e] = 0.f;
    }
  };
  auto finalize = [&](int mi) {
    if (etid < BN) {
      float t0 = 0.f, t1 = 0.f;
      for (int q = 0; q < RPP; ++q) {
        t0 += red[(q * BN + etid) * 2];
        t1 += red[(q * BN + etid) * 2 + 1];
      }
      a.bn_part[(long)mi * a.part_ld + n0 + etid] = make_float2(t0, t1);
    }
  };
  if (ntl > 0) {
#pragma unroll
    for (int j = 0; j < NR; ++j) issue((mlo + ms) * BM, j, pf[j], true);
    for (int kt = 0; kt < nk; ++kt) ws_barrier();
    ws_barrier();
    ws_barrier();
    for (int i = 1; i <= ntl; ++i) {
      const bool more = i < ntl;
      const int m0 = (mlo + ms + i * mstr) * BM;
      const int kg = more ? kpg : 0;
#pragma unroll
      for (int jj = 0; jj < NKC; ++jj) {
        for (int u = 0; u < kg; ++u) ws_barrier();
#pragma unroll
        for (int r = 0; r < R; ++r) {
          const int j = jj * R + r;
          if constexpr (TMR_WS_EXP == 1) continue;
          consume(pf[j], j);
          __builtin_amdgcn_sched_barrier(0);
          issue(m0, j, pf[j], more);
          __builtin_amdgcn_sched_barrier(0);
        }
      }
      ws_barrier();
      put_red(more ? (i + 1) * nk - 1 : i * nk - 1);
      ws_barrier();
      finalize(mlo + ms + (i - 1) * mstr);
    }
  } else {
    ws_barrier();
    ws_barrier();
  }

}

template <int F32>
int launch_dgrad_ws(const GemmArgs& a, int cfg, hipStream_t st) {
  static const int on = env_int("TMR_DGRAD_WS", TMR_DGRAD_WS);
  if (!on || a.io_tiles || a.bn_part == nullptr) return -1;
  if (kCfgs16[cfg].bm != 128) return -1;
  if (a.ntaps != 1 || a.osy != 1 || a.osx != 1 || a.oyc != 0 || a.oxc != 0 || a.oy0 != 0 ||
      a.ox0 != 0 || a.wr0 != 0 || a.ws0 != 0 || a.sy != 1 || a.sx != 1 ||
      (long)a.Hs * a.Ws != (long)a.dHW.d || a.Ws != (int)a.dW.d || a.oH != a.Hs || a.oW != a.Ws)
    return -1;
  if (a.N % 128 != 0 || (WS_NWG / 8) % (a.N / 128) != 0) return -1;
  constexpr int bk = F32 ? 32 : 64;
  if (a.K <= 0 || a.K % bk != 0) return -1;
  const int nk = a.K / bk;
  if (cdiv(a.M, 128) * (long)(a.N / 128) < 2L * WS_NWG) return -1;
  const bool beta1 = a.beta == 1.f;
  const dim3 grid(WS_NWG), blk(512);
  auto go = [&](auto kern) {
    hipLaunchKernelGGL(kern, grid, blk, 0, st, a);
    TMR_CHECK_LAUNCH("dgrad_ws_kernel");
    __atomic_fetch_add(&g_dgrad_ws_launches, 1L, __ATOMIC_RELAXED);
    return 0;
  };
  if constexpr (F32) {
    if (a.bn16 || a.g16 || a.cold16) return -1;
    static const int mfma_bound = env_int("TMR_DGRAD_WS_MFMA", 0);
    if (a.bn_mask == 3 && beta1) {
      if (nk == 2) return go(dgrad_ws_kernel<1, 2, 3, 1>);
      if (nk == 4) return go(dgrad_ws_kernel<1, 4, 3, 1>);
      if (mfma_bound && nk % 8 == 0) return go(dgrad_ws_kernel<1, 8, 3, 1>);
    } else if (mfma_bound && a.bn_mask == 2 && a.beta == 0.f && nk % 8 == 0) {
      return go(dgrad_ws_kernel<1, 8, 2, 0>);
    }
  } else {
    if (!a.bn16 || !a.g16 || a.bn_mask != 1 || !beta1 || !(a.Cold == nullptr || a.cold16))
      return -1;
    if (nk == 1) return go(dgrad_ws_kernel<0, 1, 1, 1>);
    if (nk == 2) return go(dgrad_ws_kernel<0, 2, 1, 1>);
    if (nk == 4) return go(dgrad_ws_kernel<0, 4, 1, 1>);
  }
  return -1;
}

}
```

tmrnet_amd/csrc/gemm_conv.hip:

```cpp
#include "direct_conv.h"
#include "gemm16_select.h"

#include <type_traits>

using namespace tmrg;

namespace {

__device__ __forceinline__ float split_sum(const float* __restrict__ slabs, int nsplit, long slab,
                                           long src) {
  float s = 0.f;
  int p = 0;
  for (; p + 8 <= nsplit; p += 8) {
    float v[8];
#pragma unroll
    for (int u = 0; u < 8; ++u) v[u] = slabs[(p + u) * slab + src];
#pragma unroll
    for (int u = 0; u < 8; ++u) s += v[u];
  }
  for (; p < nsplit; ++p) s += slabs[p * slab + src];
  return s;
}

__global__ void wgrad_reduce_kernel(const float* __restrict__ slabs, int nsplit, long slab,
// ... 196 lines not shown
    TMR_CHECK_ARG(!(a.c16 && (beta != 0.f || bias)),
                  "tmr_conv2d_fwd: a bf16 output (TMR_IO_Y_BF16) takes no beta / bias");
    return launch_gemm<MODE_FWD>(a, al, 1, stream);
  });
}

TMR_API int tmr_conv2d_fwd_fused(const tmr_conv_desc* d, const float* x, const float* w_krsc,
                                 const float* scale, const float* shift, const float* residual,
                                 float* y, int relu, hipStream_t stream) {
  TMR_CHECK_ARG(d, "tmr_conv2d_fwd_fused: null descriptor");
  TMR_CHECK_ARG(scale && shift, "tmr_conv2d_fwd_fused: null BatchNorm scale/shift");
  TMR_CHECK_ARG(!residual || residual != y, "tmr_conv2d_fwd_fused: residual must not alias y");
  return for_slices(d, [&](const tmr_conv_desc& c, int g, int f0) -> int {
    const long o = (long)g * c.k;
    GemmArgs a;
    bool al;
    const int rc = conv_fwd_args(&c, adv(x, x_off(c, g, f0), esz_x(d)), adv(w_krsc, w_off(c, g), esz_w(d)),
                                 shift + o, adv(y, y_off(c, g, f0), esz_y(d)), 0.f, a, al);
    if (rc) return rc;
    a.scale = scale + o;
    a.res = adv(residual, y_off(c, g, f0), esz_y(d));
    a.relu = relu;
    if (a.c16) {
      TMR_CHECK_ARG(use16(a, MODE_FWD),
                    "tmr_conv2d_fwd_fused: a bf16 output (TMR_IO_Y_BF16) needs bf16 x and w "
                    "(TMR_IO_X_BF16 | TMR_IO_W_BF16), channels and row strides multiples of 8");
      TMR_CHECK_ARG(a.N % 2 == 0 && a.ldc % 2 == 0 && (((uintptr_t)a.C | (uintptr_t)a.res) & 3) == 0,
                    "tmr_conv2d_fwd_fused: a bf16 output needs even channels / y_ld and 4-B "
                    "aligned y and residual");
      a.Cbytes = clamp_bytes_e(span((long)c.n * c.ho * c.wo, a.ldc, c.k), 2);
    }
    return launch_gemm<MODE_FWD>(a, al, 1, stream);
  });
}

TMR_API int tmr_conv2d_fwd_stats_parts(const tmr_conv_desc* d) {
  if (!d || d->n <= 0) {
    tmr_set_error("tmr_conv2d_fwd_stats_parts: null or empty descriptor");
    return -1;
  }
  if (const auto* f = direct_view(d, &DirectConv::fwd)) return f->parts(d);
  int parts = 0;
  const auto count = [&](const tmr_conv_desc& c, int, int) {
    parts += stats_parts_of(&c);
    return 0;
  };
  return for_slices(d, count, true) ? -1 : parts;
}

TMR_API int tmr_conv2d_fwd_bnstats(const tmr_conv_desc* d, const float* x, const float* w_krsc,
                                   float* y, void* stats, size_t stats_bytes, hipStream_t stream) {
  TMR_CHECK_ARG(d, "tmr_conv2d_fwd_bnstats: null descriptor");
  TMR_CHECK_ARG(yld_of(d) == d->k, "tmr_conv2d_fwd_bnstats: output must be dense (y_ld == k)");
  const int np = tmr_conv2d_fwd_stats_parts(d);
  TMR_CHECK_ARG(np >= 0, "tmr_conv2d_fwd_bnstats: bad descriptor");
  const size_t need = (size_t)np * d->k * sizeof(float4);
  TMR_CHECK_ARG(stats && stats_bytes >= need, "tmr_conv2d_fwd_bnstats: stats buffer too small (%zu < %zu)",
                stats_bytes, need);
  if (const auto* f = direct_view(d, &DirectConv::fwd)) return f->run(d, x, w_krsc, y, stats, stream);
  float4* st = nullptr;
  return for_slices(d, [&](const tmr_conv_desc& c, int g, int f0) -> int {
    if (f0 == 0) st = (float4*)stats + (long)g * c.k;
    GemmArgs a;
    bool al;
    const int rc = conv_fwd_args(&c, adv(x, x_off(c, g, f0), esz_x(d)), adv(w_krsc, w_off(c, g), esz_w(d)),
                                 nullptr, adv(y, y_off(c, g, f0), esz_y(d)), 0.f, a, al);
    if (rc) return rc;
    a.stats = st;
    a.part_ld = d->k;
    st += (long)stats_parts_of(&c) * d->k;
    return launch_gemm<MODE_FWD>(a, al, 1, stream);
  });
}

struct BnBwdFuse {
  const float *y, *z, *sc, *sh, *mean;
  int mask;
  float2* part;
  long nparts;
  bool count_only;
  int part_ld;
  const void* old;
  int old16;
};

static void tile_of(const GemmArgs& a, int mode, tmr_conv_tile* t) {
  const bool f32 = a.prec == TMR_MATH_F32;
  if (use16(a, mode)) {
    t->engine = 2;
    t->cfg = pick_cfg16(a.M, a.N, a.K, mode, f32);
    const Cfg16 c = kCfgs16[t->cfg];
    t->bm = c.bm; t->bn = c.bn; t->waves = c.waves;
    t->tapv = tapv16(a, mode, f32) ? 1 : 0;
  } else {
    t->engine = 1;
    t->cfg = pick_cfg(a.M, a.N, a.K, mode);
    const TileCfg c = kCfgs[t->cfg];
    t->bm = c.bm; t->bn = c.bn; t->waves = c.waves;
    t->tapv = 0;
  }
}

static int conv_dgrad_impl(const tmr_conv_desc* d, const float* dy, const float* w_krsc,
                           float* dx, float beta, hipStream_t stream, BnBwdFuse* fz = nullptr,
                           tmr_conv_tile* plan = nullptr) {
  TMR_CHECK_ARG(d->math == TMR_MATH_F32 || d->math == TMR_MATH_BF16, "tmr_conv2d: bad math mode %d", d->math);
  const int lk = ilog2_exact(d->k);
  TMR_CHECK_ARG(lk >= 2, "tmr_conv2d_dgrad: output channels %d must be a power of two >= 4", d->k);
  TMR_CHECK_ARG(d->c % 4 == 0, "tmr_conv2d_dgrad: input channels %d must be a multiple of 4", d->c);
  TMR_CHECK_ARG(!(d->io & TMR_IO_WT_BF16) || !(d->io & TMR_IO_W_BF16),
                "tmr_conv2d_dgrad: TMR_IO_WT_BF16 and TMR_IO_W_BF16 are exclusive weight layouts");
  TMR_CHECK_ARG(!(d->io & TMR_IO_WT_F32) ||
                    (d->math == TMR_MATH_F32 && (d->io & ~(TMR_IO_ENGINE | TMR_IO_CLASSES | TMR_IO_TILES)) == TMR_IO_WT_F32),
                "tmr_conv2d_dgrad: TMR_IO_WT_F32 (fp32 transposed weights) needs TMR_MATH_F32 and "
                "no bf16-stored operand");
  TMR_CHECK_ARG((d->io & ~(TMR_IO_WT_F32 | TMR_IO_ENGINE | TMR_IO_CLASSES | TMR_IO_TILES)) == 0 ||
                    d->math == TMR_MATH_BF16,
                "tmr_conv2d: bf16-stored operands (io %d) need TMR_MATH_BF16", d->io);
  const int st = d->stride;
  const bool par = st == 2 && !(d->io & TMR_IO_CLASSES);
  GemmArgs pend[PAR_MAX];
  bool pend_al[PAR_MAX];
  int npend = 0;
  long best_m = -1;
  for (int ph = 0; ph < st; ++ph) {
    for (int pw = 0; pw < st; ++pw) {
      int r0 = -1, nR = 0, s0 = -1, nS = 0;
      for (int r = 0; r < d->r; ++r)
        if (((ph + d->pad - r) % st + st) % st == 0) { if (r0 < 0) r0 = r; ++nR; }
      for (int s = 0; s < d->s; ++s)
        if (((pw + d->pad_w - s) % st + st) % st == 0) { if (s0 < 0) s0 = s; ++nS; }
      const int hg = (d->h - ph + st - 1) / st, wg = (d->w - pw + st - 1) / st;
      if (hg <= 0 || wg <= 0) continue;
      GemmArgs a{};
      a.A = dy; a.B = w_krsc; a.C = dx; a.bias = nullptr;
      a.M = d->n * hg * wg; a.N = d->c; a.K = nR * nS * d->k;
      a.log2C = lk;
      set_taps(a, nR, nS);
      if (nR == 0 || nS == 0) { a.K = 0; a.ntaps = 0; }
      a.oy0 = nR ? (ph + d->pad - r0) / st : 0;
      a.ox0 = nS ? (pw + d->pad_w - s0) / st : 0;
      a.dyr = -1; a.dxs = -1;
      a.wr0 = r0 < 0 ? 0 : r0; a.ws0 = s0 < 0 ? 0 : s0; a.wst = st; a.wS = d->s;
      set_grid(a, d->n, hg, wg);
      a.Hs = d->ho; a.Ws = d->wo; a.sy = 1; a.sx = 1;
      a.lds = yld_of(d); a.ldb = d->r * d->s * d->c; a.ldc = xld_of(d); a.beta = beta;
      a.Abytes = clamp_bytes_e(span((long)d->n * d->ho * d->wo, a.lds, d->k), esz_dy(d));
      a.prec = d->math;
      a.Bbytes = clamp_bytes_e((long)d->k * d->r * d->s * d->c, esz_w(d));
      a.sab = ((d->io & TMR_IO_DY_BF16) ? 1 : 0) | ((d->io & (TMR_IO_W_BF16 | TMR_IO_WT_BF16)) ? 2 : 0);
      if (d->io & (TMR_IO_WT_BF16 | TMR_IO_WT_F32)) {
        a.wt = 1;
        a.ldbt = d->r * d->s * d->k;
      }
      a.Cbytes = clamp_bytes(span((long)d->n * d->h * d->w, a.ldc, d->c));
      a.oH = d->h; a.oW = d->w; a.osy = st; a.osx = st; a.oyc = ph; a.oxc = pw;
      if (plan) {
        if (a.K > 0) {
          ++plan->classes;
          if (a.M > best_m) {
            best_m = a.M;
            tile_of(a, MODE_DGRAD, plan);
          }
        }
        continue;
      }
      if (a.K == 0 && beta == 1.f && !fz) continue;
      if (fz) {
        const long nmt = cdiv(a.M, gemm_tile_bm(a, MODE_DGRAD));
        if (fz->count_only) { fz->nparts += nmt; continue; }
        a.bn_y = fz->y; a.bn_z = fz->z; a.bn_sc = fz->sc; a.bn_sh = fz->sh; a.bn_mean = fz->mean;
        a.bn_mask = fz->mask;
        a.bn16 = (d->io & TMR_IO_BN_BF16) ? 1 : 0;
        if (d->io & TMR_IO_G16) {
          a.g16 = 1;
          a.Cbytes = clamp_bytes_e(span((long)d->n * d->h * d->w, a.ldc, d->c), 2);
        }
        a.bn_part = fz->part;
        a.part_ld = fz->part_ld;
        a.Cold = fz->old;
        a.cold16 = fz->old16;
        a.io_tiles = (d->io & TMR_IO_TILES) ? 1 : 0;
        fz->part += nmt * fz->part_ld;
        fz->nparts += nmt;
      }
      bool al = aligned16(dy) && aligned16(w_krsc) && aligned16(dx) && a.lds % 4 == 0;
      if (par) {
        pend[npend] = a;
        pend_al[npend++] = al;
        continue;
      }
      const int rc = launch_gemm<MODE_DGRAD>(a, al, 1, stream);
      if (rc) return rc;
    }
  }
  if (npend > 0) {
    int rc = launch_gemm_dgrad_par(pend, npend, stream);
    if (rc < 0) {
      rc = 0;
      for (int i = 0; i < npend && rc == 0; ++i)
        rc = launch_gemm<MODE_DGRAD>(pend[i], pend_al[i], 1, stream);
    }
    if (rc) return rc;
  }
  return 0;
}

static int dgrad_bnbwd_run(const tmr_conv_desc* d, const float* dy, const float* w_krsc, float* dx,
                           float beta, const BnBwdFuse& fz, long* nparts, hipStream_t stream) {
  float2* part = nullptr;
  const auto slice = [&](const tmr_conv_desc& c, int g, int f0) -> int {
    const long o = (long)g * c.c, px = x_off(c, g, f0);
    if (f0 == 0) part = adv(fz.part, o, sizeof(float2));
    BnBwdFuse s = fz;
    s.y = adv(fz.y, px, esz_bn(d));
    s.z = fz.mask == 3 ? (const float*)((const uint32_t*)fz.z + px / 32) : adv(fz.z, px, esz_bn(d));
    s.sc = adv(fz.sc, o, 4); s.sh = adv(fz.sh, o, 4); s.mean = adv(fz.mean, o, 4);
    s.old = adv(fz.old, px, fz.old16 ? 2 : 4);
    s.part = part;
    s.nparts = 0;
    const int rc = conv_dgrad_impl(&c, adv(dy, y_off(c, g, f0), esz_dy(d)), adv(w_krsc, w_off(c, g), esz_w(d)),
                                   adv(dx, px, esz_dx(d)), beta, stream, &s);
    part = s.part;
    if (nparts) *nparts += s.nparts;
    return rc;
  };
  return for_slices(d, slice, fz.count_only);
}

long tmrg::g_dgrad_ws_launches = 0;
TMR_API long tmr_dgrad_ws_launches(void) { return __atomic_load_n(&g_dgrad_ws_launches, __ATOMIC_RELAXED); }

TMR_API int tmr_conv2d_dgrad_bnbwd_parts(const tmr_conv_desc* d) {
  if (!d || d->n <= 0) {
    tmr_set_error("tmr_conv2d_dgrad_bnbwd_parts: null or empty descriptor");
    return -1;
  }
  if (const auto* f = direct_view(d, &DirectConv::dgrad)) return f->parts(d);
  BnBwdFuse fz{};
  fz.count_only = true;
  long np = 0;
  if (dgrad_bnbwd_run(d, nullptr, nullptr, nullptr, 1.f, fz, &np, nullptr)) return -1;
  return (int)np;
}

static int dgrad_bnbwd_entry(const tmr_conv_desc* d, const float* dy, const float* w_krsc,
                             float* dx, float beta, const void* dx_old, int old_bf16,
                             const float* y, const float* z, const float* scale,
                             const float* shift, const float* mean, int mask, void* parts,
                             size_t parts_bytes, hipStream_t stream) {
  TMR_CHECK_ARG(xld_of(d) == d->c, "tmr_conv2d_dgrad_bnbwd: dx must be dense (x_ld == c)");
  TMR_CHECK_ARG(ngroups(d) == 1 || mask != 3,
                "tmr_conv2d_dgrad_bnbwd: a grouped dgrad takes no ReLU-mask bits");
  TMR_CHECK_ARG(y && mean && parts, "tmr_conv2d_dgrad_bnbwd: null y / mean / parts");
  TMR_CHECK_ARG(!(d->io & TMR_IO_G16) ||
                    (d->math == TMR_MATH_BF16 && (d->io & TMR_IO_WT_BF16) &&
                     (d->c / ngroups(d)) % 8 == 0),
                "tmr_conv2d_dgrad_bnbwd: a bf16 gradient (TMR_IO_G16) needs bf16 math on the LDS-DMA "
                "engine (TMR_IO_WT_BF16), channels per group a multiple of 8");
  TMR_CHECK_ARG(!dx_old || ngroups(d) == 1, "tmr_conv2d_dgrad_bnbwd: a separate old dx takes no groups");
  TMR_CHECK_ARG(ngroups(d) == 1 || beta == 0.f || !(d->io & TMR_IO_G16),
                "tmr_conv2d_dgrad_bnbwd: a grouped dgrad accumulates (beta != 0) into fp32 dx only");
  TMR_CHECK_ARG(mask == 0 || (mask == 1 && z) || (mask == 2 && scale && shift) || (mask == 3 && z),
                "tmr_conv2d_dgrad_bnbwd: mask %d needs z (1, 3: bits) or scale/shift (2)", mask);
  TMR_CHECK_ARG(mask != 3 || ((d->io & (TMR_IO_WT_F32 | TMR_IO_WT_BF16)) &&
                              ((long)d->h * d->w * d->c) % 32 == 0),
                "tmr_conv2d_dgrad_bnbwd: ReLU-mask bits (mask 3) need the LDS-DMA dgrad "
                "(TMR_IO_WT_F32 / TMR_IO_WT_BF16) and h*w*c a multiple of 32");
  const int np = tmr_conv2d_dgrad_bnbwd_parts(d);
  TMR_CHECK_ARG(np >= 0 && parts_bytes >= (size_t)np * d->c * sizeof(float2),
                "tmr_conv2d_dgrad_bnbwd: parts buffer too small");
  if (const auto* f = direct_view(d, &DirectConv::dgrad)) {
    TMR_CHECK_ARG(!dx_old && !((d->io & TMR_IO_G16) && beta != 0.f),
                  "tmr_conv2d_dgrad_bnbwd: the direct 3x3 dgrad takes no old dx / "
                  "accumulating bf16 gradient");
    return f->run(d, dy, w_krsc, dx, beta, y, z, scale, shift, mean, mask, parts, stream);
  }
  BnBwdFuse fz{};
  fz.y = y; fz.z = z; fz.sc = scale; fz.sh = shift; fz.mean = mean; fz.mask = mask;
  fz.part = (float2*)parts;
  fz.part_ld = d->c;
  fz.old = dx_old;
  fz.old16 = beta != 0.f ? old_bf16 : 0;
  return dgrad_bnbwd_run(d, dy, w_krsc, dx, beta, fz, nullptr, stream);
}

TMR_API int tmr_conv2d_dgrad_bnbwd(const tmr_conv_desc* d, const float* dy, const float* w_krsc,
                                   float* dx, float beta, const float* y, const float* z,
                                   const float* scale, const float* shift, const float* mean,
                                   int mask, void* parts, size_t parts_bytes, hipStream_t stream) {
  TMR_CHECK_ARG(d, "tmr_conv2d_dgrad_bnbwd: null descriptor");
  return dgrad_bnbwd_entry(d, dy, w_krsc, dx, beta, nullptr, (d->io & TMR_IO_G16) ? 1 : 0, y, z,
                           scale, shift, mean, mask, parts, parts_bytes, stream);
}

TMR_API int tmr_conv2d_dgrad_bnbwd_acc(const tmr_conv_desc* d, const float* dy,
                                       const float* w_krsc, void* dx, float beta,
                                       const void* dx_old, int old_bf16, const float* y,
                                       const float* z, const float* scale, const float* shift,
                                       const float* mean, int mask, void* parts,
                                       size_t parts_bytes, hipStream_t stream) {
  TMR_CHECK_ARG(d, "tmr_conv2d_dgrad_bnbwd_acc: null descriptor");
  TMR_CHECK_ARG(beta != 0.f && dx_old && ((uintptr_t)dx_old & 15) == 0 &&
                    (d->io & TMR_IO_G16) && (d->io & TMR_IO_WT_BF16),
                "tmr_conv2d_dgrad_bnbwd_acc: needs beta != 0, a 16-B aligned old dx and a bf16 "
                "output (TMR_IO_G16) on the bf16 LDS-DMA engine (TMR_IO_WT_BF16)");
  return dgrad_bnbwd_entry(d, dy, w_krsc, (float*)dx, beta, dx_old, old_bf16 ? 1 : 0, y, z, scale,
                           shift, mean, mask, parts, parts_bytes, stream);
}

TMR_API int tmr_conv2d_dgrad(const tmr_conv_desc* d, const float* dy, const float* w_krsc,
                             float* dx, float beta, hipStream_t stream) {
  TMR_CHECK_ARG(d, "tmr_conv2d_dgrad: null descriptor");
  return for_slices(d, [&](const tmr_conv_desc& c, int g, int f0) {
    return conv_dgrad_impl(&c, adv(dy, y_off(c, g, f0), esz_dy(d)), adv(w_krsc, w_off(c, g), esz_w(d)),
                           dx + x_off(c, g, f0), beta, stream);
  });
}

static void wgrad_fill(const tmr_conv_desc* d, GemmArgs& a) {
  a = GemmArgs{};
  a.M = d->k; a.N = d->r * d->s * d->c; a.K = d->n * d->ho * d->wo;
  a.log2C = ilog2_exact(d->c);
  set_taps(a, d->r, d->s);
  a.oy0 = -d->pad; a.ox0 = -d->pad_w; a.dyr = 1; a.dxs = 1;
  set_grid(a, d->n, d->ho, d->wo);
  a.Hs = d->h; a.Ws = d->w; a.sy = d->stride; a.sx = d->stride;
  a.lds = xld_of(d); a.ldb = yld_of(d); a.ldc = a.N; a.beta = 0.f;
  a.Abytes = clamp_bytes_e(span((long)d->n * d->ho * d->wo, a.ldb, d->k), esz_dy(d));
  a.prec = d->math;
  a.Bbytes = clamp_bytes_e(span((long)d->n * d->h * d->w, a.lds, d->c), esz_x(d));
  a.sab = ((d->io & TMR_IO_DY_BF16) ? 1 : 0) | ((d->io & TMR_IO_X_BF16) ? 2 : 0);
  a.dma32 = d->math == TMR_MATH_F32;
}

static int wgrad_plan(const tmr_conv_desc* d, int* splits, int* kchunk, long* slab) {
  const long Mred = (long)d->n * d->ho * d->wo;
  const long Mo = d->k, No = (long)d->r * d->s * d->c;
  GemmArgs a;
  wgrad_fill(d, a);
  const long tiles = gemm_tiles(a, MODE_WGRAD);
  static const long target = env_int("TMR_WGRAD_TARGET", 512);
  static const long minrows = env_int("TMR_WGRAD_MINROWS", 1024);
  long sp = target / (tiles > 0 ? tiles : 1);
  if (sp < 1) sp = 1;
  long maxsp = Mred / minrows;
  if (maxsp < 1) maxsp = 1;
  if (sp > maxsp) sp = maxsp;
  long kc = (Mred + sp - 1) / sp;
  kc = (kc + 63) / 64 * 64;
  sp = (Mred + kc - 1) / kc;
  *splits = (int)sp;
  *kchunk = (int)kc;
  *slab = Mo * No;
  return 0;
}

static const DirectConv::Wgrad* direct_wgrad(const tmr_conv_desc* d, int c_real) {
  const DirectConv::Wgrad* f = direct_view(d, &DirectConv::wgrad);
  return f && (c_real == 0 || f->c_real == 0 || f->c_real == c_real) ? f : nullptr;
}

TMR_API size_t tmr_conv2d_wgrad_ws_bytes(const tmr_conv_desc* d) {
  if (!d || d->n <= 0 || d->k <= 0 || d->c <= 0 || d->r <= 0 || d->s <= 0) {
    tmr_set_error("tmr_conv2d_wgrad_ws_bytes: null or empty descriptor");
    return 0;
  }
  size_t bytes = 0;
  const auto plan = [&](const tmr_conv_desc& c, int, int) {
    int sp, kc;
    long slab;
    wgrad_plan(&c, &sp, &kc, &slab);
    if ((size_t)sp * slab * sizeof(float) > bytes) bytes = (size_t)sp * slab * sizeof(float);
    return 0;
  };
  if (for_slices(d, plan, true)) return 0;
  if (const auto* f = direct_wgrad(d, 0))
    if (bytes < f->ws_bytes(d)) bytes = f->ws_bytes(d);
  return bytes;
}

static int wgrad_reduce(const tmr_conv_desc* d, const float* ws, int sp, long slab, float* dw_oihw,
                        int c_real, float beta, hipStream_t stream) {
  const int ntaps = d->r * d->s;
  if (ntaps > 1 && ntaps <= kReduceTaps) {
    hipLaunchKernelGGL(wgrad_reduce_taps_kernel, dim3(d->k, cdiv(c_real, 64)), dim3(256), 0,
                       stream, ws, sp, slab, dw_oihw, ntaps, d->c, c_real, beta);
    TMR_CHECK_LAUNCH("wgrad_reduce_taps_kernel");
    return 0;
  }
  long total = (long)d->k * ntaps * c_real;
// ... 211 lines not shown
```

tmrnet_amd/ops.py:

```python
import contextlib
import threading
import weakref

import numpy as np
import torch

from ._lib import call, query, stream_ptr, ConvDesc, ConvTile
from . import health
import ctypes

f32 = torch.float32

PROF = None


class _prof:
    def __init__(self, kind, flops, shape=None, nbytes=0):
        self.kind, self.flops, self.shape, self.nbytes = kind, flops, shape, nbytes

    def __enter__(self):
        if PROF is not None:
            self.e0 = torch.cuda.Event(enable_timing=True)
            self.e1 = torch.cuda.Event(enable_timing=True)
            self.e0.record()
# ... 233 lines not shown
         float(momentum), float(eps), mean, inv, scale, shift, ws, ctypes.c_size_t(ws.numel() * 8),
         stream_ptr())
    return mean, inv, scale, shift


def conv_dgrad(dy, w_krsc, in_hw, stride, pad, out=None, beta=0.0, pad_w=None, math="fp32",
               wt=False, groups=1):
    _req_op(w_krsc, "w")
    n, ho, wo, k = dy.shape
    k2, r, s, c = _dgrad_w(w_krsc, wt, groups)
    h, w = in_hw
    d = conv_desc(n, h, w, c, k, r, s, stride, pad, pad_w, math=math, io=_io(None, w_krsc, dy, wt),
                  groups=groups)
    assert (d.ho, d.wo) == (ho, wo), ((d.ho, d.wo), (ho, wo))
    if out is None:
        out = _empty((n, h, w, c), dy)
    d.x_ld = _nhwc_ld(out, "dx")
    d.y_ld = _nhwc_ld(dy, "dy")
    with _prof("conv_dgrad" + _SUFFIX[math], 2.0 * n * ho * wo * k * r * s * c / groups, (n, h, w, c, k, r, stride),
               _esz(dy) * n * ho * wo * k + _esz(w_krsc) * w_krsc.numel()
               + 4 * n * h * w * c * (2 if beta else 1)):
        call("tmr_conv2d_dgrad", ctypes.byref(d), dy, w_krsc, out, float(beta), stream_ptr())
    return out


def conv_dgrad_bnbwd(dy, w_krsc, in_hw, stride, pad, y, mean, mask, z=None, scale=None,
                     shift=None, out=None, beta=0.0, math="fp32", wt=False, groups=1,
                     g16=False, old=None):
    if old is not None:
        if not (g16 and beta != 0.0 and out is None and groups == 1):
            raise RuntimeError("conv_dgrad_bnbwd: a separate old dx needs g16, beta, no out / "
                               "groups")
        if old.dtype not in (f32, BF16) or not old.is_contiguous():
            raise RuntimeError("conv_dgrad_bnbwd: old dx must be a contiguous fp32 / bf16 tensor")
    if g16 and groups > 1 and beta != 0.0:
        raise RuntimeError("conv_dgrad_bnbwd: a grouped dgrad accumulates (beta != 0) into an fp32 "
                           "dx only")
    _req_op(w_krsc, "w"); _req_op(y, "y"); _req(mean, "mean")
    if mask == 3:
        if z is None or z.dtype != torch.int32 or z.numel() * 32 < y.numel():
            raise RuntimeError("conv_dgrad_bnbwd: mask 3 takes the int32 ReLU-mask bits of y's shape")
    elif z is not None and z.dtype != y.dtype:
        raise RuntimeError("conv_dgrad_bnbwd: y and z must have one dtype")
    n, ho, wo, k = dy.shape
    k2, r, s, c = _dgrad_w(w_krsc, wt, groups)
    h, w = in_hw
    d = conv_desc(n, h, w, c, k, r, s, stride, pad, math=math,
                  io=_io(None, w_krsc, dy, wt) | (IO_BN if y.dtype == BF16 else 0)
                  | (IO_G16 if g16 else 0), groups=groups)
    assert (d.ho, d.wo) == (ho, wo), ((d.ho, d.wo), (ho, wo))
    if out is None:
        out = _empty((n, h, w, c), dy, dtype=BF16 if g16 else f32)
    elif out.dtype != (BF16 if g16 else f32):
        raise RuntimeError("conv_dgrad_bnbwd: dx must be %s" % ("bf16 (g16)" if g16 else "fp32"))
    if tuple(y.shape) != tuple(out.shape) or (z is not None and mask != 3
                                              and tuple(z.shape) != tuple(out.shape)):
        raise RuntimeError("conv_dgrad_bnbwd: y/z must have dx's shape %s" % (tuple(out.shape),))
    if old is not None and tuple(old.shape) != tuple(out.shape):
        raise RuntimeError("conv_dgrad_bnbwd: old dx must have dx's shape %s" % (tuple(out.shape),))
    d.x_ld = _nhwc_ld(out, "dx")
    d.y_ld = _nhwc_ld(dy, "dy")
    nparts = query("tmr_conv2d_dgrad_bnbwd_parts", ctypes.byref(d))
    if nparts < 0:
        raise RuntimeError("tmr_conv2d_dgrad_bnbwd_parts failed")
    parts = torch.empty((max(nparts, 1), c, 2), dtype=f32, device=dy.device)
    with _prof("conv_dgrad" + _SUFFIX[math], 2.0 * n * ho * wo * k * r * s * c / groups, (n, h, w, c, k, r, stride),
               _esz(dy) * n * ho * wo * k + _esz(w_krsc) * w_krsc.numel()
               + (2 if g16 else 4) * n * h * w * c
               + ((old.element_size() if old is not None else (2 if g16 else 4)) * n * h * w * c
                  if beta else 0)
               + y.element_size() * n * h * w * c * (2 if z is not None and mask != 3 else 1)
               + (n * h * w * c // 8 if mask == 3 else 0)):
        if old is not None:
            call("tmr_conv2d_dgrad_bnbwd_acc", ctypes.byref(d), dy, w_krsc, out, float(beta), old,
                 int(old.dtype == BF16), y, z, scale, shift, mean, int(mask), parts,
                 ctypes.c_size_t(parts.numel() * 4), stream_ptr())
        else:
            call("tmr_conv2d_dgrad_bnbwd", ctypes.byref(d), dy, w_krsc, out, float(beta), y, z,
                 scale, shift, mean, int(mask), parts, ctypes.c_size_t(parts.numel() * 4),
                 stream_ptr())
    return out, parts, nparts


def bn_bwd_maxpool(dyp, am, y, scale, shift, mean, inv, gamma, bf16=False):
    n, h, w, c = y.shape
    _, ho, wo, _ = dyp.shape
    ws, nb = _bn_ws(n * h * w, c, y.device)
    if y.dtype == BF16:
        dy = torch.empty_like(y)
        dgamma = _empty((c,), dyp); dbeta = _empty((c,), dyp)
        call("tmr_bn_bwd_maxpool_a16", dyp, am, n, h, w, ho, wo, y, scale, shift, mean, inv, gamma,
             dy, dgamma, dbeta, c, ws, ctypes.c_size_t(nb), stream_ptr())
        return dy, dgamma, dbeta
    dy = torch.empty_like(y, dtype=torch.bfloat16 if bf16 else y.dtype)
    dgamma = _empty((c,), y); dbeta = _empty((c,), y)
    call("tmr_bn_bwd_maxpool_x", dyp, am, n, h, w, ho, wo, y, scale, shift, mean, inv, gamma, dy,
         dgamma, dbeta, c, ws, ctypes.c_size_t(nb), int(bf16), stream_ptr())
    return dy, dgamma, dbeta


def bn_bwd_parts_ds(g, y, parts, nparts, mean, inv, gamma, yd, mean_d, inv_d, gamma_d,
                    fold3=False, foldd=False, dy16=False):
    if dy16:
        if fold3 or foldd:
            raise RuntimeError("bn_bwd_parts_ds: bf16 dy's (dy16) take no wgrad fold")
        c = y.shape[-1]
        rows = y.numel() // c
        if not (g.dtype == y.dtype == yd.dtype == f32 and g.shape == y.shape == yd.shape
                and g.is_contiguous() and y.is_contiguous() and yd.is_contiguous()):
            raise RuntimeError("bn_bwd_parts_ds: dy16 takes contiguous fp32 g, y and y_ds of one "
                               "shape")
        nb = query("tmr_bn_bwd_parts_ds_ws_bytes", int(nparts), rows, c)
        ws = torch.empty(((nb + 7) // 8,), dtype=torch.float64, device=y.device)
        dy, dyd = torch.empty_like(y, dtype=BF16), torch.empty_like(yd, dtype=BF16)
        dg, db = _empty((c,), mean), _empty((c,), mean)
        dgd, dbd = _empty((c,), mean), _empty((c,), mean)
        call("tmr_bn_bwd_parts_ds_d16", g, y, parts, int(nparts), mean, inv, gamma, dy, dg, db, yd,
             mean_d, inv_d, gamma_d, dyd, dgd, dbd, rows, c, ws, ctypes.c_size_t(ws.numel() * 8),
             stream_ptr())
        return dy, dg, db, dyd, dgd, dbd
    if fold3 or foldd:
        return bn_bwd_parts_ds_coef(g, y, parts, nparts, mean, inv, gamma, yd, mean_d, inv_d,
                                    gamma_d, apply3=not fold3, applyd=not foldd)
    c = y.shape[-1]
    rows = y.numel() // c
    t = y.dtype
    if not (g.dtype == t and yd.dtype == t and t in (f32, BF16) and g.shape == y.shape == yd.shape
            and g.is_contiguous() and y.is_contiguous() and yd.is_contiguous()):
        raise RuntimeError("bn_bwd_parts_ds: g, y and y_ds must be contiguous tensors of one shape "
                           "and one dtype (fp32 or bf16)")
    nb = query("tmr_bn_bwd_parts_ds_ws_bytes", int(nparts), rows, c)
    ws = torch.empty(((nb + 7) // 8,), dtype=torch.float64, device=y.device)
    dy, dyd = torch.empty_like(y), torch.empty_like(yd)
    dg, db = _empty((c,), mean), _empty((c,), mean)
    dgd, dbd = _empty((c,), mean), _empty((c,), mean)
    call("tmr_bn_bwd_parts_ds", g, y, parts, int(nparts), mean, inv, gamma, dy, dg, db, yd, mean_d,
         inv_d, gamma_d, dyd, dgd, dbd, rows, c, int(t == BF16), ws, ctypes.c_size_t(ws.numel() * 8),
         stream_ptr())
    return dy, dg, db, dyd, dgd, dbd


def bn_bwd_parts_ds_coef(g, y, parts, nparts, mean, inv, gamma, yd, mean_d, inv_d, gamma_d,
                         apply3=False, applyd=False):
    c = y.shape[-1]
    rows = y.numel() // c
    if not (g.dtype == y.dtype == yd.dtype == f32 and g.shape == y.shape == yd.shape
            and g.is_contiguous() and y.is_contiguous() and yd.is_contiguous()):
        raise RuntimeError("bn_bwd_parts_ds_coef: g, y and y_ds must be contiguous fp32 tensors of "
                           "one shape")
    if apply3 and applyd:
        raise RuntimeError("bn_bwd_parts_ds_coef: both outputs are bn_bwd_parts_ds")
    nb = query("tmr_bn_bwd_parts_ds_ws_bytes", int(nparts), rows, c)
    off3 = query("tmr_bn_bwd_parts_ds_coef_offset", int(nparts), rows, c, 0)
    offd = query("tmr_bn_bwd_parts_ds_coef_offset", int(nparts), rows, c, 1)
    ws = torch.empty(((nb + 7) // 8,), dtype=torch.float64, device=y.device)
    dy = torch.empty_like(y) if apply3 else None
    dyd = torch.empty_like(yd) if applyd else None
    dg, db = _empty((c,), mean), _empty((c,), mean)
    dgd, dbd = _empty((c,), mean), _empty((c,), mean)
    call("tmr_bn_bwd_parts_ds", g, y, parts, int(nparts), mean, inv, gamma, dy, dg, db, yd, mean_d,
         inv_d, gamma_d, dyd, dgd, dbd, rows, c, 0, ws, ctypes.c_size_t(ws.numel() * 8),
         stream_ptr())
    wf = ws.view(f32)
    return (wf[off3 // 4: off3 // 4 + 3 * c], dg, db, wf[offd // 4: offd // 4 + 3 * c], dgd, dbd,
            dy, dyd)

# ... 966 lines not shown
```

tmrnet_amd/trunk.py:

```python
import os
import weakref

import torch
import torch.nn as nn

from . import ops


class Bottleneck(nn.Module):
    expansion = 4

    def __init__(self, inplanes, planes, stride=1, downsample=None):
        super().__init__()
        self.conv1 = nn.Conv2d(inplanes, planes, 1, bias=False)
        self.bn1 = nn.BatchNorm2d(planes)
        self.conv2 = nn.Conv2d(planes, planes, 3, stride=stride, padding=1, bias=False)
        self.bn2 = nn.BatchNorm2d(planes)
        self.conv3 = nn.Conv2d(planes, planes * 4, 1, bias=False)
        self.bn3 = nn.BatchNorm2d(planes * 4)
        self.relu = nn.ReLU(inplace=True)
        self.downsample = downsample
        self.stride = stride


def _make_layer(inplanes, planes, blocks, stride):
    downsample = None
    if stride != 1 or inplanes != planes * 4:
        downsample = nn.Sequential(nn.Conv2d(inplanes, planes * 4, 1, stride=stride, bias=False),
                                   nn.BatchNorm2d(planes * 4))
    layers = [Bottleneck(inplanes, planes, stride, downsample)]
    for _ in range(1, blocks):
        layers.append(Bottleneck(planes * 4, planes))
    return nn.Sequential(*layers)


_GRAD_READY = weakref.WeakKeyDictionary()


def set_grad_ready(share, fn):
    if fn is None:
        _GRAD_READY.pop(share, None)
    else:
        _GRAD_READY[share] = fn


def get_grad_ready(share):
    return _GRAD_READY.get(share, getattr(share, "grad_ready", None))

def _bn_momentum(bn):
    if bn.momentum is None:
        raise NotImplementedError("BatchNorm2d(momentum=None) (cumulative average) is not supported")
    return bn.momentum


BF16_STORE = os.environ.get("TMR_BF16_STORE", "1") != "0"


def _store16(math):
    return math == "bf16" and BF16_STORE


FULL16 = True

ACT16 = os.environ.get("TMR_BF16_ACT", "1") != "0"


G16 = os.environ.get("TMR_G16", "1") != "0"

R16 = os.environ.get("TMR_BF16_RESGRAD", "1") != "0"

DS_DUAL = True

WGRAD_BNBWD = True

WGRAD_BNBWD_DS = True
WGRAD_BNBWD_DS_MIN = 8_000_000


def _ds_fold(g, r3, rd):
    if not (WGRAD_BNBWD and WGRAD_BNBWD_DS and g.dtype == torch.float32
            and r3["math"] == "fp32" and rd["math"] == "fp32" and g.numel() >= WGRAD_BNBWD_DS_MIN):
        return False, False

    def ok(rec):
        kr, ks = rec["conv"].weight.shape[2:]
        return (rec.get("groups", 1) == 1 and
                ops.conv_wgrad_bnbwd_ok(rec["x"], g, rec["y"], kr, ks, rec["stride"], rec["pad"]))
    return ok(r3), ok(rd)


def _ds_dual(g, r3, rd):
    y = r3["y"]
    return (DS_DUAL and g.is_contiguous() and g.dtype == y.dtype == rd["y"].dtype
            and y.shape == rd["y"].shape and y.shape[-1] % 8 == 0
            and (_ds_dy16(r3, rd) or not (_store16(r3["math"]) and y.dtype == torch.float32)))


def _ds_dy16(r3, rd):
    return bool(r3.get("dy16") and rd.get("dy16") and r3["y"].dtype == torch.float32)



def _dma32(math):
    return math == "fp32"




def _full16(math):
    return _store16(math) and FULL16


BWD16 = "bf16-bwd"


def _fwd_math(precision):
    return "fp32" if precision == BWD16 else precision


def _act16(math):
    return _full16(math) and ACT16


def _infer16(share):
    return bool(not share.training and share.precision != BWD16 and _full16(share.precision)
                and getattr(share, "infer_act16", False))


def _conv_bn(x, conv, bn, stride, pad, relu, training, residual=None, recs=None, math="fp32",
             defer=False, branch=None, nbt=None, dual=False, groups=1, y16=False, bwd16=False,
             x16=None):
    w = conv.weight
    k, c, r, s = w.shape
    if bwd16 and not (training and recs is not None and math == "fp32" and groups == 1
                      and not dual and not y16):
        raise RuntimeError("bwd16 is the train-mode fp32 forward of an ungrouped conv with a "
                           "recorded backward")
    cs = x.shape[3]
    s16 = _store16(math)
    if r == 1 and s == 1 and c == cs and not s16:
        wk = w.detach().contiguous().view(k, 1, 1, c)
    else:
        wk = ops.weight_to_krsc(w.detach().contiguous(), cpad=cs // groups, bf16=s16)
    if groups > 1 and not training and not y16:
        raise RuntimeError("grouped convs run in the train-mode trunk and the bf16-activation "
                           "inference trunk (y16) only")
    if training:
        y, stats, nparts = ops.conv_fwd_bnstats(x, wk, stride, pad, c_real=c * groups, math=math,
                                                y16=_act16(math), groups=groups)
        mean, inv, scale, shift = ops.bn_finalize(
            stats, nparts, bn.weight.detach(), bn.bias.detach(), bn.running_mean,
            bn.running_var, _bn_momentum(bn), bn.eps)
        if nbt is None:
            bn.num_batches_tracked.add_(1)
        else:
            nbt.append(bn.num_batches_tracked)
    else:
        scale, shift = ops.bn_eval_params(bn.weight.detach(), bn.bias.detach(), bn.running_mean,
                                          bn.running_var, bn.eps)
        return ops.conv_fwd_fused(x, wk, stride, pad, scale, shift, residual, relu, c_real=c,
                                  math=math, y16=y16, groups=groups)
    zbits = None
    bits = (recs is not None and relu and not dual and _dma32(math) and y.dtype == torch.float32
            and (residual is not None or branch is not None))
    z16 = None
    if defer:
        z = None
    elif bwd16 and bits and branch is not None:
        z, zbits, z16 = ops.bn_apply2_bits_dual(y, scale, shift, branch[0], branch[1], branch[2])
    elif bwd16 and bits:
        z, zbits, z16 = ops.bn_apply_bits_dual(y, scale, shift, residual)
    elif bwd16:
        if residual is not None or branch is not None:
            raise RuntimeError("bwd16: a residual unit without ReLU has no dual apply")
        z, z16 = ops.bn_apply_dual(y, scale, shift, None, relu)
    elif branch is not None and bits:
        z, zbits = ops.bn_apply2_bits(y, scale, shift, branch[0], branch[1], branch[2])
    elif bits:
        z, zbits = ops.bn_apply_bits(y, scale, shift, residual)
    elif branch is not None:
        z = ops.bn_apply2(y, scale, shift, branch[0], branch[1], branch[2], relu, dual=dual)
    elif dual:
        z = ops.bn_apply_dual(y, scale, shift, residual, relu)
    else:
        z = ops.bn_apply(y, scale, shift, residual, relu, bf16=s16 and residual is None)
    if recs is not None:
        has_res = residual is not None or branch is not None
        if bwd16:
            wt = ops.weight_to_crsk(w.detach().contiguous()) if c % 8 == 0 else None
        elif groups > 1 and ((_full16(math) and x.dtype == torch.bfloat16) or _dma32(math)):
            wt = ops.weight_to_crsk_grouped(w.detach().contiguous(), groups,
                                            bf16=x.dtype == torch.bfloat16)
        elif _full16(math) and x.dtype == torch.bfloat16:
            wt = ops.weight_to_crsk(w.detach().contiguous())
        elif _dma32(math) and c % 8 == 0 and x.dtype == torch.float32:
            wt = ops.weight_to_crsk(w.detach().contiguous(), bf16=False)
        else:
            wt = None
        recs.append({"x": x16 if (bwd16 and x16 is not None) else x, "wk": wk, "wt": wt, "y": y,
                     "z": (z[0] if dual else z) if has_res else None, "zbits": zbits,
                     "scale": scale, "shift": shift, "mean": mean, "inv": inv,
                     "stride": stride, "pad": pad, "relu": relu, "conv": conv, "bn": bn,
                     "c_real": c, "math": "bf16" if bwd16 else math, "groups": groups,
                     "res": has_res, "dy16": bwd16})
    if defer:
        return y, scale, shift
    return (z, z16) if bwd16 else z


def _conv_bn_bwd(rec, dz, grads, want_dres=False, dx_out=None, dx_beta=0.0, need_dx=True,
                 dres_inplace=False, parts=None, fuse_prev=None, pool=None, dy=None, g16=False,
                 r16=False, fold=False, gcoef=None):
    conv, bn = rec["conv"], rec["bn"]
    s16 = rec.get("dy16", False) or _store16(rec["math"])
    dy_given = dy is not None or gcoef is not None
    dw = None
    kr, ks = conv.weight.shape[2:]
    if gcoef is not None:
        dw, dy = ops.conv_wgrad_bnbwd(rec["x"], gcoef[0], rec["y"], gcoef[1], kr, ks, rec["stride"],
                                      rec["pad"], c_real=rec["c_real"])
        dres = None
    elif dy_given:
        dres = None
    elif pool is not None:
        dy, dg, db = ops.bn_bwd_maxpool(pool[0], pool[1], rec["y"], rec["scale"], rec["shift"],
                                        rec["mean"], rec["inv"], bn.weight.detach(), bf16=s16)
        dres = None
    elif (parts is not None and fold and WGRAD_BNBWD and rec["math"] == "fp32"
          and rec.get("groups", 1) == 1
          and ops.conv_wgrad_bnbwd_ok(rec["x"], dz, rec["y"], kr, ks, rec["stride"], rec["pad"])):
        coef, dg, db = ops.bn_bwd_parts_coef(rec["y"], parts[0], parts[1], rec["mean"],
                                             rec["inv"], bn.weight.detach())
        dw, dy = ops.conv_wgrad_bnbwd(rec["x"], dz, rec["y"], coef, kr, ks, rec["stride"],
                                      rec["pad"], c_real=rec["c_real"])
        dres = dz if want_dres else None
    elif parts is not None:
        dy, dg, db = ops.bn_bwd_parts(dz, rec["y"], parts[0], parts[1], rec["mean"], rec["inv"],
                                      bn.weight.detach(), bf16=s16)
        dres = dz if want_dres else None
    else:
        dy, dres, dg, db = ops.bn_bwd(dz, rec["y"], rec["z"], rec["mean"], rec["inv"],
                                      bn.weight.detach(), rec["relu"], want_dres=want_dres,
                                      dres_out=dz if dres_inplace else None,
                                      scale=rec["scale"], shift=rec["shift"], bf16=s16)
    if not dy_given:
        grads[bn.weight] = dg
        grads[bn.bias] = db
    x = rec["x"]
    k, c, r, s = conv.weight.shape
    grp = rec.get("groups", 1)
    grads[conv.weight] = dw if dw is not None else ops.conv_wgrad(
        x, dy, r, s, rec["stride"], rec["pad"], c_real=rec["c_real"], math=rec["math"],
        groups=grp)
    dx, fused = None, None
    if need_dx:
        hw = (x.shape[1], x.shape[2])
        wt = rec.get("wt") is not None
        wdg = rec["wt"] if wt else rec["wk"]
        if fuse_prev is not None:
            p = fuse_prev
            mask = (1 if p.get("res", p["z"] is not None) else 2) if p["relu"] else 0
            zm = p["z"]
            if mask == 1 and wt and p.get("zbits") is not None:
                mask, zm = 3, p["zbits"]
            elif mask == 1 and zm is None:
                raise RuntimeError("a residual unit's ReLU mask needs its saved z or its bits on "
                                   "the LDS-DMA dgrad")
            bf8 = (wt and p["y"].dtype == torch.bfloat16 and
                   (p["y"].shape[-1] // grp) % 8 == 0)
            gb = (g16 and G16 and mask == 2 and dx_out is None and dx_beta == 0.0 and bf8)
            rb = (r16 and R16 and mask in (1, 3) and dx_out is not None and dx_beta == 1.0 and bf8
                  and grp == 1)
            old = None
            if rb and dx_out.dtype != torch.bfloat16:
                old, dx_out = dx_out, None
            dx, pp, npp = ops.conv_dgrad_bnbwd(dy, wdg, hw, rec["stride"], rec["pad"],
                                               p["y"], p["mean"], mask, z=zm,
                                               scale=p["scale"], shift=p["shift"], out=dx_out,
                                               beta=dx_beta, math=rec["math"],
                                               wt=wt, groups=grp, g16=gb or rb, old=old)
            fused = (pp, npp)
        else:
            dx = ops.conv_dgrad(dy, wdg, hw, rec["stride"], rec["pad"], out=dx_out,
                                beta=dx_beta, math=rec["math"], wt=wt, groups=grp)
    return dx, dres, fused


class TrunkFn(torch.autograd.Function):

    @staticmethod
    def forward(ctx, x4, share, keep, *params):
        with ops.layout_session(share, ("resnet50", share.training, bool(keep),
                                 share.precision, _infer16(share))):
            return TrunkFn._forward(ctx, x4, share, keep, params)

    @staticmethod
    def _forward(ctx, x4, share, keep, params):
        training = share.training
        keep = keep and training
        recs = [] if keep else None
        nbt = []
        conv1, bn1, layers = share.trunk_parts()
        mt = _fwd_math(share.precision)
        bw = bool(keep and share.precision == BWD16)
        a16 = training and _act16(mt)
        f16 = training and _full16(mt) and not a16
        i16 = _infer16(share)
        if training:
            xs = ops.nhwc4_to_bf16x8(x4) if (a16 and ops.engine_forced()) else x4
            y0, sc0, sh0 = _conv_bn(xs, conv1, bn1, 2, 3, True, training, recs=recs, math=mt,
                                    defer=True, nbt=nbt, bwd16=bw)
            if bw:
                p, h16, am = ops.maxpool_fwd_bn_dual(y0, sc0, sh0)
            else:
                p, am = ops.maxpool_fwd_bn(y0, sc0, sh0, bf16=f16)
            stem_hw = (y0.shape[1], y0.shape[2])
        elif i16:
            z = _conv_bn(ops.nhwc4_to_bf16x8(x4), conv1, bn1, 2, 3, True, training, math=mt,
                         y16=True)
            p, am = ops.maxpool_fwd_bn(z, torch.ones_like(bn1.running_mean),
                                       torch.zeros_like(bn1.running_mean))
            stem_hw = (z.shape[1], z.shape[2])
        else:
            z = _conv_bn(x4, conv1, bn1, 2, 3, True, training, recs=recs, math=mt, nbt=nbt)
            p, am = ops.maxpool_fwd(z)
            stem_hw = (z.shape[1], z.shape[2])
        h, hx = (None, p) if f16 else (p, p)
        if not bw:
            h16 = None
        z1h = z2h = None
        blocks = []
        for layer in layers:
            for blk in layer:
                brec = [] if keep else None
                z1 = _conv_bn(hx, blk.conv1, blk.bn1, 1, 0, True, training, recs=brec, math=mt,
                              nbt=nbt, y16=i16, bwd16=bw, x16=h16)
                if bw:
                    z1, z1h = z1
                z2 = _conv_bn(z1, blk.conv2, blk.bn2, blk.stride, 1, True, training, recs=brec,
                              math=mt, nbt=nbt, y16=i16, bwd16=bw, x16=z1h)
                if bw:
                    z2, z2h = z2
                if blk.downsample is not None:
                    idn = _conv_bn(hx, blk.downsample[0], blk.downsample[1], blk.stride, 0, False,
                                   training, recs=brec, math=mt, defer=training, nbt=nbt,
                                   y16=i16, bwd16=bw, x16=h16)
                else:
                    if h is None:
                        raise RuntimeError("identity residual of the stem output (no downsample)")
                    idn = h
                if isinstance(idn, tuple):
                    h = _conv_bn(z2, blk.conv3, blk.bn3, 1, 0, True, training, branch=idn,
                                 recs=brec, math=mt, nbt=nbt, dual=f16, bwd16=bw, x16=z2h)
                else:
                    h = _conv_bn(z2, blk.conv3, blk.bn3, 1, 0, True, training, residual=idn,
                                 recs=brec, math=mt, nbt=nbt, dual=f16, y16=i16, bwd16=bw,
                                 x16=z2h)
                if bw:
                    h, h16 = h
                    hx = h
                    if blocks:
                        blocks[-1][1][-1]["z"] = None
                    del z1, z2, idn
                else:
                    h, hx = h if f16 else (h, h)
                blocks.append((blk, brec))
        feat = ops.avgpool_fwd(h)
        ops.counters_add_one(nbt)
        ctx.keep = keep
        if keep:
            ctx.share = share
            ctx.params = params
            ctx.stem = recs
            ctx.pool = (am, stem_hw)
            ctx.blocks = blocks
            ctx.last_hw = (h.shape[1], h.shape[2])
        return feat

    @staticmethod
    def backward(ctx, dfeat):
        if not ctx.keep:
            raise RuntimeError("trunk backward needs train mode and a forward with grad enabled")
        grads = {}
        g = ops.avgpool_bwd(dfeat.contiguous(), ctx.last_hw)
        blocks = ctx.blocks
        pending = None
        ready = get_grad_ready(ctx.share)
        while blocks:
            blk, brec = blocks.pop()
            has_ds = blk.downsample is not None
            r1, r2 = brec[0], brec[1]
            rd = brec[2] if has_ds else None
            r3 = brec[-1]
            prev3 = blocks[-1][1][-1] if blocks else None
            dyd = gcd = None
            if (has_ds and _ds_dual(g, r3, rd) and pending is not None):
                bargs = (g, r3["y"], pending[0], pending[1], r3["mean"], r3["inv"],
                         r3["bn"].weight.detach(), rd["y"], rd["mean"], rd["inv"],
                         rd["bn"].weight.detach())
                f3, fd = _ds_fold(g, r3, rd)
                gc3 = None
                if f3 or fd:
                    c3, dg3, db3, cd, dgd, dbd, dy3, dyd = ops.bn_bwd_parts_ds(
                        *bargs, fold3=f3, foldd=fd)
                    gc3 = (g, c3) if f3 else None
                    gcd = (g, cd) if fd else None
                else:
                    dy3, dg3, db3, dyd, dgd, dbd = ops.bn_bwd_parts_ds(
                        *bargs, dy16=_ds_dy16(r3, rd))
                grads[r3["bn"].weight], grads[r3["bn"].bias] = dg3, db3
                grads[rd["bn"].weight], grads[rd["bn"].bias] = dgd, dbd
                dz2, _, fz2 = _conv_bn_bwd(r3, None, grads, fuse_prev=r2, g16=True, dy=dy3, gcoef=gc3)
                dres = g
                del dy3, gc3
            else:
                dz2, dres, fz2 = _conv_bn_bwd(r3, g, grads, want_dres=True, dres_inplace=True,
                                              parts=pending, fuse_prev=r2, g16=True, fold=True)
            dz1, _, fz1 = _conv_bn_bwd(r2, dz2, grads, parts=fz2, fuse_prev=r1, g16=True,
                                      fold=True)
            del dz2
            if has_ds:
                if dyd is not None or gcd is not None:
                    dx, _, _ = _conv_bn_bwd(rd, None, grads, dy=dyd, gcoef=gcd)
                    del dyd, gcd
                else:
                    dx, _, _ = _conv_bn_bwd(rd, dres, grads)
                dx, _, pending = _conv_bn_bwd(r1, dz1, grads, parts=fz1, dx_out=dx, dx_beta=1.0,
                                              fuse_prev=prev3, r16=True, fold=True)
            else:
                dx, _, pending = _conv_bn_bwd(r1, dz1, grads, parts=fz1, dx_out=dres, dx_beta=1.0,
                                              fuse_prev=prev3, r16=True, fold=True)
            del dz1, brec, dres
            g = dx
            if ready is not None:
                ready([(p, grads[p]) for p in blk.parameters() if p in grads])
        dh = g
        am, stem_hw = ctx.pool
        _conv_bn_bwd(ctx.stem[0], None, grads, need_dx=False, pool=(dh, am))
        out = [grads.get(p) for p in ctx.params]
        ctx.blocks = ctx.stem = None
        return (None, None, None) + tuple(out)


_CHILD_NAMES = ("conv1", "bn1", "relu", "maxpool", "layer1", "layer2", "layer3", "layer4",
                "avgpool")


class ResNet50Share(nn.Sequential):

    def __init__(self, indexed=False, precision="fp32"):
        super().__init__()
        if precision not in ("fp32", "bf16", BWD16):
            raise ValueError("precision must be 'fp32', 'bf16' or 'bf16-bwd', got %r" % (precision,))
        self.precision = precision
        self.infer_act16 = False
        mods = (nn.Conv2d(3, 64, 7, stride=2, padding=3, bias=False), nn.BatchNorm2d(64),
                nn.ReLU(inplace=True), nn.MaxPool2d(3, stride=2, padding=1),
                _make_layer(64, 64, 3, 1), _make_layer(256, 128, 4, 2),
                _make_layer(512, 256, 6, 2), _make_layer(1024, 512, 3, 2),
                nn.AdaptiveAvgPool2d((1, 1)))
        for i, (name, m) in enumerate(zip(_CHILD_NAMES, mods)):
            self.add_module(str(i) if indexed else name, m)
        for m in self.modules():
            if isinstance(m, nn.Conv2d):
                nn.init.kaiming_normal_(m.weight, mode="fan_out", nonlinearity="relu")
            elif isinstance(m, nn.BatchNorm2d):
                nn.init.constant_(m.weight, 1)
                nn.init.constant_(m.bias, 0)

    def trunk_parts(self):
        ch = list(self.children())
        return ch[0], ch[1], ch[4:8]

    def features_nhwc4(self, x4):
        params = list(self.parameters())
        keep = torch.is_grad_enabled() and any(p.requires_grad for p in params)
        return TrunkFn.apply(x4, self, keep, *params)

    def forward(self, x):
        x = x.reshape(-1, 3, x.shape[-2], x.shape[-1]).contiguous()
        x4 = ops.nchw_to_nhwc(x, cpad=4)
        feat = self.features_nhwc4(x4)
        return feat.view(feat.shape[0], feat.shape[1], 1, 1)


def resnet50_share():
    return ResNet50Share()
```

Before: 3888 frames/s.

## Keep strided downsample dgrad compact and fold it into conv1 dgrad epilogue

In bottleneck blocks with a stride-2 1x1 downsample, the downsample dgrad is now computed at the output resolution instead of being scattered into a full-resolution dx that is three-quarters zeros. The following conv1 dgrad with fused BN backward then reads this compact tensor as its beta=1 'old' input. An even-row/column parity test selects the rows that carry a value, and the others load out-of-bounds as zero. This is meant to cut writing and reading a large, mostly zero fp32 tensor in the largest downsample blocks. In exchange it adds new kernel instantiations, a shared included kernel body, and a size threshold that limits the path to big activations.

New measurement: 3909 frames/s, median of 6. No clear change (+0.5%).

```diff
diff --git a/include/tmr.h b/include/tmr.h
--- a/include/tmr.h
+++ b/include/tmr.h
@@ -83,6 +83,13 @@
                                const float* y, const float* z, const float* scale,
                                const float* shift, const float* mean, int mask, void* parts,
                                size_t parts_bytes, hipStream_t stream);
+int tmr_conv2d_dgrad_bnbwd_oldc_ok(const tmr_conv_desc* d, const void* dx, const void* old_compact,
+                                   size_t old_bytes, float beta, int mask);
+int tmr_conv2d_dgrad_bnbwd_oldc(const tmr_conv_desc* d, const float* dy, const float* w_crsk,
+                                float* dx, float beta, const float* old_compact, size_t old_bytes,
+                                const float* y, const void* zbits, const float* mean, int mask,
+                                void* parts, size_t parts_bytes, hipStream_t stream);
+long tmr_dgrad_oldc_launches(void);
 int tmr_gemm_nt(int M, int N, int K, const float* A, int lda, const float* B, int ldb,
                 const float* bias, float* C, int ldc, float beta, hipStream_t stream);
 int tmr_gemm_nn(int M, int N, int K, const float* A, int lda, const float* B, int ldb, float* C,
diff --git a/tmrnet_amd/_lib.py b/tmrnet_amd/_lib.py
--- a/tmrnet_amd/_lib.py
+++ b/tmrnet_amd/_lib.py
@@ -82,6 +82,9 @@
     "tmr_conv2d_wgrad_bnbwd_ok": [DP, P, P, P, P],
     "tmr_conv2d_wgrad_bnbwd": [DP, P, P, P, P, P, P, I, F, P, SZ, P],
     "tmr_wgrad_bnbwd_launches": [],
+    "tmr_conv2d_dgrad_bnbwd_oldc_ok": [DP, P, P, SZ, F, I],
+    "tmr_conv2d_dgrad_bnbwd_oldc": [DP, P, P, P, F, P, SZ, P, P, P, I, P, SZ, P],
+    "tmr_dgrad_oldc_launches": [],
     "tmr_conv2d_tile": [DP, I, ctypes.POINTER(ConvTile)],
     "tmr_bn_parts_coef_offset": [I, I],
     "tmr_conv2d_dgrad_bnbwd_acc": [DP, P, P, P, F, P, I, P, P, P, P, P, I, P, SZ, P],
@@ -229,6 +232,7 @@
     "tmr_conv2d_wgrad_ws_bytes": SZ,
     "tmr_dgrad_ws_launches": L,
     "tmr_wgrad_bnbwd_launches": L,
+    "tmr_dgrad_oldc_launches": L,
     "tmr_bn_parts_coef_offset": SZ,
     "tmr_resize_tmp_bytes": SZ,
     "tmr_margin_ws_bytes": SZ,
diff --git a/tmrnet_amd/csrc/gemm16_dgrad_f32.hip b/tmrnet_amd/csrc/gemm16_dgrad_f32.hip
--- a/tmrnet_amd/csrc/gemm16_dgrad_f32.hip
+++ b/tmrnet_amd/csrc/gemm16_dgrad_f32.hip
@@ -2,4 +2,34 @@
 
 namespace tmrg {
 template int launch_gemm16<MODE_DGRAD, 1>(const GemmArgs& a, int splits, hipStream_t st);
+
+int launch_gemm16_dgrad_oldc(const GemmArgs& a, hipStream_t st) {
+  TMR_CHECK_ARG(use16(a, MODE_DGRAD) && a.prec == TMR_MATH_F32, "dgrad_oldc: not an fp32 LDS-DMA dgrad");
+  TMR_CHECK_ARG(dgrad_rows_identity(a) && a.dW.d % 2 == 0 && (a.dHW.d / a.dW.d) % 2 == 0,
+                "dgrad_oldc: a 1x1 stride-1 dgrad on an even grid");
+  TMR_CHECK_ARG(a.bn_part && a.bn_mask == 3 && a.beta == 1.f && !a.bn16 && !a.g16 && !a.cold16,
+                "dgrad_oldc: the fp32 mask-bits beta-1 form only");
+  TMR_CHECK_ARG(a.Cold && ((uintptr_t)a.Cold & 15) == 0, "dgrad_oldc: D must be 16-B aligned");
+  const int cfg = pick_cfg16(a.M, a.N, a.K, MODE_DGRAD, true);
+  TMR_CHECK_ARG(dgrad_oldc_cfg(cfg), "dgrad_oldc: tile config %d has no compact-old form", cfg);
+  if (const int rc = check16<MODE_DGRAD, 1>(a, cfg)) return rc;
+  const Cfg16 c = kCfgs16[cfg];
+  const dim3 grid(cdiv(a.M, c.bm) * cdiv(a.N, c.bn), 1, 1);
+  if (grid.x == 0) return 0;
+  const int nk = a.K / 32;
+  if (dgrad_ws_shape<1>(a, cfg) && (nk == 2 || nk == 4)) {
+    if (nk == 2) hipLaunchKernelGGL((dgrad_ws_oldc_kernel<2>), dim3(WS_NWG), dim3(512), 0, st, a);
+    else hipLaunchKernelGGL((dgrad_ws_oldc_kernel<4>), dim3(WS_NWG), dim3(512), 0, st, a);
+    TMR_CHECK_LAUNCH("dgrad_ws_oldc_kernel");
+    return 0;
+  }
+  switch (cfg) {
+    case 2: hipLaunchKernelGGL((gemm16_dgrad_oldc_kernel<128, 128, 2, 2>), grid, dim3(256), 0, st, a); break;
+    case 5: hipLaunchKernelGGL((gemm16_dgrad_oldc_kernel<64, 64, 2, 2>), grid, dim3(256), 0, st, a); break;
+    case 7: hipLaunchKernelGGL((gemm16_dgrad_oldc_kernel<128, 128, 4, 2>), grid, dim3(512), 0, st, a); break;
+    default: break;
+  }
+  TMR_CHECK_LAUNCH("gemm16_dgrad_oldc_kernel");
+  return 0;
 }
+}
diff --git a/tmrnet_amd/csrc/gemm16_kernel.h b/tmrnet_amd/csrc/gemm16_kernel.h
--- a/tmrnet_amd/csrc/gemm16_kernel.h
+++ b/tmrnet_amd/csrc/gemm16_kernel.h
@@ -105,9 +105,29 @@
 #ifndef TMR_EPI_LATE_F
 #define TMR_EPI_LATE_F 0
 #endif
+__device__ __forceinline__ bool old_compact_row(const GemmArgs& a, uint32_t row, uint32_t& drow) {
+  const uint32_t q = fdiv(row, a.dW);
+  const uint32_t w = row - q * a.dW.d;
+  drow = (q >> 1) * (a.dW.d >> 1) + (w >> 1);
+  return ((q | w) & 1u) == 0u;
+}
+__device__ __forceinline__ __amdgpu_buffer_rsrc_t old_compact_rsrc(const GemmArgs& a) {
+  return make_rsrc(reinterpret_cast<const float*>(a.Cold), (uint32_t)a.M * (uint32_t)a.ldc);
+}
+__device__ __forceinline__ void load_old8_compact(const GemmArgs& a, uint32_t row, int col, uint4& c0,
+                                                  uint4& c1) {
+  uint32_t drow;
+  const bool tap = old_compact_row(a, row, drow);
+  const __amdgpu_buffer_rsrc_t rD = old_compact_rsrc(a);
+  const uint32_t od = (drow * (uint32_t)a.ldc + (uint32_t)col) * 4u;
+  c0 = __builtin_bit_cast(uint4, __builtin_amdgcn_raw_buffer_load_b128(rD, tap ? od : OOB, 0, 0));
+  c1 = __builtin_bit_cast(uint4, __builtin_amdgcn_raw_buffer_load_b128(rD, tap ? od + 16u : OOB, 0, 0));
+}
+
 template <int BM, int BN, int WM, int WN, int SMEMB, int DEPTH = TMR_EPI_DEPTH, int TOP = 0,
-          int EPF = 0>
+          int EPF = 0, int OSP = 0>
 struct LdsBnbwd {
+  static_assert(!OSP || EPF != 1, "the parity-sparse old dx: fp32 forms");
   using Form = EpiForm<EPF>;
   static constexpr int NT = 64 * WM * WN;
   static constexpr int LDC = BN + 4;
@@ -140,7 +160,7 @@
     const int row = m0 + ci * RCH + rr;
     x.ok = rr < nrow && col < a.N && row < a.M;
     long pix = row;
-    if (x.ok && a.osy != 0) {
+    if (!OSP && x.ok && a.osy != 0) {
       const uint32_t n = fdiv((uint32_t)row, a.dHW);
       const uint32_t rem = row - n * a.dHW.d;
       const uint32_t y = fdiv(rem, a.dW);
@@ -163,7 +183,11 @@
       }
     }
     if (Form::mask3(a)) x.bits = reinterpret_cast<const uint32_t*>(a.bn_z)[off >> 5];
-    if (a.beta != 0.f) load_old8(a, off, x.c0, x.c1, Form::cold16(a));
+    if constexpr (OSP) {
+      load_old8_compact(a, (uint32_t)row, col, x.c0, x.c1);
+    } else if (a.beta != 0.f) {
+      load_old8(a, off, x.c0, x.c1, Form::cold16(a));
+    }
   }
 
   __device__ __forceinline__ static void prefetch(const GemmArgs& a, int m0, int n0, In (&pf)[DT]) {
@@ -298,7 +322,7 @@
   }
 };
 
-template <int BM, int BN, int WM, int WN, int TM, int TN>
+template <int BM, int BN, int WM, int WN, int TM, int TN, int OSP = 0>
 __device__ __forceinline__ void epilogue_lds_bnbwd(const GemmArgs& a, floatx16 (&acc)[TM][TN],
                                                    float* lds, int lds_floats, int m0, int n0) {
   constexpr int NT = 64 * WM * WN;
@@ -346,7 +370,7 @@
       const int row = m0 + r0 + rr;
       const bool ok = okc && row < a.M;
       long pix = row;
-      if (ok && a.osy != 0) {
+      if (!OSP && ok && a.osy != 0) {
         const uint32_t n = fdiv((uint32_t)row, a.dHW);
         const uint32_t rem = row - n * a.dHW.d;
         const uint32_t y = fdiv(rem, a.dW);
@@ -394,7 +418,11 @@
 #pragma unroll
           for (int e = 0; e < 8; ++e) zv[e] = 0.f;
         }
-        if (has_beta) {
+        if constexpr (OSP) {
+          uint4 c0, c1;
+          load_old8_compact(a, (uint32_t)row, col, c0, c1);
+          unpack_old8(c0, c1, old, false);
+        } else if (has_beta) {
           uint4 c0, c1;
           load_old8(a, off, c0, c1);
           unpack_old8(a, c0, c1, old);
@@ -446,7 +474,7 @@
 }
 
 template <int MODE, int BM, int BN, int WM, int WN, int TAPV, int PIPE, int F32, int NST, int EPF = 0,
-          int INF16 = 0, int BNW = 0>
+          int INF16 = 0, int BNW = 0, int OSP = 0>
 __device__ __forceinline__ void gemm16_body(const GemmArgs& a, const int bid, const int split) {
   constexpr uint32_t ES = F32 ? 4u : 2u;
   constexpr int EPC = 16 / ES;
@@ -729,7 +757,8 @@
                       PRE ? (EPF == 1 ? TMR_EPI_DEPTH_F16 : TMR_EPI_DEPTH) : (LATE ? 0 : 1),
                       PRE ? (EPF == 1 ? TMR_EPI_TOPUP_F16 : (EPF == 2 ? TMR_EPI_TOPUP_F32 : TMR_EPI_TOPUP))
                           : (LATE ? LATED : 0),
-                      EPF>;
+                      EPF, OSP>;
+  static_assert(!OSP || (LDSEPI && F32 != 0), "the parity-sparse old dx: fp32 LDS-staged dgrads");
   typename Epi::In pf[(PRE || LATE) ? Epi::DT : 1];
   if constexpr (PRE) {
     if (a.bn_part != nullptr) Epi::prefetch(a, m0, n0, pf);
@@ -876,8 +905,8 @@
         Epi::prefetch(a, m0, n0, pf);
         Epi::run(a, acc, reinterpret_cast<float*>(smem), m0, n0, pf);
       } else
-        epilogue_lds_bnbwd<BM, BN, WM, WN, TM, TN>(a, acc, reinterpret_cast<float*>(smem), SMEM / 4,
-                                                    m0, n0);
+        epilogue_lds_bnbwd<BM, BN, WM, WN, TM, TN, OSP>(a, acc, reinterpret_cast<float*>(smem),
+                                                         SMEM / 4, m0, n0);
       return;
     }
   }
@@ -909,6 +938,15 @@
   int bid, split;
   xcd_work(bid, split);
   gemm16_body<MODE_WGRAD, BM, BN, WM, WN, 0, 1, 1, 2, 0, 0, 2>(a, bid, split);
+}
+
+template <int BM, int BN, int WM, int WN>
+__global__ __launch_bounds__(64 * WM * WN, (occ16<BM, BN, WM, WN, 2>()))
+void gemm16_dgrad_oldc_kernel(const GemmArgs a) {
+  int bid, split;
+  xcd_work(bid, split);
+  gemm16_body<MODE_DGRAD, BM, BN, WM, WN, 0, 1, 1, 2, (WM * WN == 4 && TMR_EPI_FORMS) ? 2 : 0, 0, 0, 1>(
+      a, bid, split);
 }
 
 __device__ __forceinline__ void par_tile(const GemmPar& p, int w, int& cls, int& t) {
diff --git a/tmrnet_amd/csrc/gemm16_select.h b/tmrnet_amd/csrc/gemm16_select.h
--- a/tmrnet_amd/csrc/gemm16_select.h
+++ b/tmrnet_amd/csrc/gemm16_select.h
@@ -119,6 +119,10 @@
 int launch_gemm16_wgrad_bnbwd(const GemmArgs& a, int splits, hipStream_t st);
 extern long g_wgrad_bnbwd_launches;
 
+inline bool dgrad_oldc_cfg(int cfg) { return cfg == 2 || cfg == 5 || cfg == 7; }
+int launch_gemm16_dgrad_oldc(const GemmArgs& a, hipStream_t st);
+extern long g_dgrad_oldc_launches;
+
 template <int BM, int BN, int WM, int WN>
 int launch16_inf16(const GemmArgs& a, bool tapv, dim3 grid, hipStream_t st);
 extern template int launch16_inf16<256, 128, 4, 2>(const GemmArgs&, bool, dim3, hipStream_t);
diff --git a/tmrnet_amd/csrc/gemm16_ws.h b/tmrnet_amd/csrc/gemm16_ws.h
--- a/tmrnet_amd/csrc/gemm16_ws.h
+++ b/tmrnet_amd/csrc/gemm16_ws.h
@@ -18,354 +18,40 @@
 
 template <int F32, int NKC, int MSK, int BETA>
 __global__ __launch_bounds__(512) void dgrad_ws_kernel(const GemmArgs a) {
-  constexpr bool BN16 = !F32, C16 = !F32, G16 = !F32;
-  constexpr int BM = 128, BN = 128, NW = 4, WN = 2;
-  constexpr uint32_t ES = F32 ? 4u : 2u;
-  constexpr int EPC = 16 / ES, BK = 128 / ES;
-  constexpr int TM = 2, TN = 2;
-  constexpr int ABYTES = BM * 128, STAGE = 2 * ABYTES;
-  constexpr int NIA = ABYTES / (1024 * NW);
-  constexpr int NST = 3;
-  constexpr int LDC = BN;
-  constexpr int STG = BM * LDC * 4;
-  constexpr int CG = BN / 8, RPP = 256 / CG, NR = BM / RPP;
-  constexpr int R = NR / NKC;
-  static_assert(NR == 8 && R * NKC == NR, "consumer row groups");
-  static_assert(RPP * BN * 8 <= STAGE, "the partial sums fit a stage");
-  using Frag = typename std::conditional<F32 != 0, f32x4_t, bf16x8>::type;
-  __shared__ __attribute__((aligned(1024))) unsigned char smem[NST * STAGE + STG];
-  float* const stg = reinterpret_cast<float*>(smem + NST * STAGE);
-  auto scol = [](int row, int c) { return c ^ (((row >> 2) & 1) << 5); };
+  constexpr int OSP = 0;
+#include "gemm16_ws_body.h"
+}
 
-  const int tid = threadIdx.x;
-  const int wave = __builtin_amdgcn_readfirstlane(tid >> 6);
-  const int nnt = a.N / BN;
-  const int mt = (a.M + BM - 1) / BM;
-  const int xcd = blockIdx.x & 7, slot = blockIdx.x >> 3;
-  const int mlo = (int)((long)mt * xcd / 8), mhi = (int)((long)mt * (xcd + 1) / 8);
-  const int nt = slot % nnt, ms = slot / nnt, mstr = (WS_NWG / 8) / nnt;
-  const int ntl = mhi - mlo > ms ? (mhi - mlo - ms + mstr - 1) / mstr : 0;
-  const int n0 = nt * BN;
-  const int nk = (a.K + BK - 1) / BK;
-  const int kpg = nk / NKC;
+template <int NKC>
+__global__ __launch_bounds__(512) void dgrad_ws_oldc_kernel(const GemmArgs a) {
+  constexpr int F32 = 1, MSK = 3, BETA = 1, OSP = 1;
+#include "gemm16_ws_body.h"
+}
 
-  if (wave < NW) {
-    const int lane = tid & 63;
-    const int wm = wave / WN, wn = wave % WN;
-    const int l31 = lane & 31, hh = lane >> 5;
-    const __amdgpu_buffer_rsrc_t rA = make_rsrc(a.A, a.Abytes);
-    const __amdgpu_buffer_rsrc_t rB = make_rsrc(a.B, a.Bbytes);
-    int prow[NIA], pch[NIA];
-    uint32_t boff[NIA];
-#pragma unroll
-    for (int q = 0; q < NIA; ++q) {
-      prow[q] = 8 * (wave + NW * q) + (lane >> 3);
-      pch[q] = EPC * ((lane & 7) ^ ((prow[q] >> 1) & 7));
-      boff[q] = (uint32_t)(n0 + prow[q]) * (uint32_t)a.ldbt * ES + (uint32_t)pch[q] * ES;
-    }
-    auto stage_q = [&](int m0, int kt, int buf, int q) {
-      const int kb = kt * BK;
-      unsigned char* As = smem + buf * STAGE;
-      unsigned char* Bs = As + ABYTES;
-      const int m = m0 + prow[q];
-      const bool ok = m < a.M && kb + pch[q] < a.K;
-      const uint32_t off = (uint32_t)m * (uint32_t)a.lds * ES + (uint32_t)(kb + pch[q]) * ES;
-      glds16(rA, As + 1024 * (wave + NW * q), ok ? off : OOB);
-      const bool okb = kb + pch[q] < a.K;
-      glds16(rB, Bs + 1024 * (wave + NW * q), okb ? boff[q] + (uint32_t)kb * ES : OOB);
-    };
-    auto stage = [&](int m0, int kt, int buf) {
-#pragma unroll
-      for (int q = 0; q < NIA; ++q) stage_q(m0, kt, buf, q);
-    };
-    const int kx = (l31 >> 1) & 7;
-    const int arow0 = wm * (BM / 2) + l31;
-    const int brow0 = wn * (BN / WN) + l31;
-    auto frags = [&](int buf, int s, Frag (&av)[TM], Frag (&bv)[TN]) {
-      const unsigned char* As = smem + buf * STAGE;
-      const unsigned char* Bs = As + ABYTES;
-      const int ch = (2 * s + hh) ^ kx;
-#pragma unroll
-      for (int i = 0; i < TM; ++i)
-        av[i] = *reinterpret_cast<const Frag*>(As + (arow0 + 32 * i) * 128 + (ch << 4));
-#pragma unroll
-      for (int j = 0; j < TN; ++j)
-        bv[j] = *reinterpret_cast<const Frag*>(Bs + (brow0 + 32 * j) * 128 + (ch << 4));
-    };
-    floatx16 acc[TM][TN];
-#pragma unroll
-    for (int i = 0; i < TM; ++i)
-#pragma unroll
-      for (int j = 0; j < TN; ++j)
-#pragma unroll
-        for (int r = 0; r < 16; ++r) acc[i][j][r] = 0.f;
-    auto mfmas = [&](const Frag (&av)[TM], const Frag (&bv)[TN]) {
-      if constexpr (TMR_WS_EXP == 2) {
-        asm volatile("" ::"v"(av[0]), "v"(bv[0]), "v"(av[TM - 1]), "v"(bv[TN - 1]));
-        return;
-      }
-      __builtin_amdgcn_s_setprio(1);
-      if constexpr (F32) {
-#pragma unroll
-        for (int t = 0; t < 4; ++t)
-#pragma unroll
-          for (int i = 0; i < TM; ++i)
-#pragma unroll
-            for (int j = 0; j < TN; ++j)
-              acc[i][j] = __builtin_amdgcn_mfma_f32_32x32x2f32(av[i][t], bv[j][t], acc[i][j], 0, 0, 0);
-      } else {
-#pragma unroll
-        for (int i = 0; i < TM; ++i)
-#pragma unroll
-          for (int j = 0; j < TN; ++j)
-            acc[i][j] = __builtin_amdgcn_mfma_f32_32x32x16_bf16(av[i], bv[j], acc[i][j], 0, 0, 0);
-      }
-      __builtin_amdgcn_s_setprio(0);
-    };
-    const int ng = ntl * nk;
-    auto stage_g = [&](int G) {
-      const int ti = G / nk;
-      stage((mlo + ms + ti * mstr) * BM, G - ti * nk, G % NST);
-    };
+inline bool dgrad_rows_identity(const GemmArgs& a) {
+  return a.ntaps == 1 && a.osy == 1 && a.osx == 1 && a.oyc == 0 && a.oxc == 0 && a.oy0 == 0 &&
+         a.ox0 == 0 && a.wr0 == 0 && a.ws0 == 0 && a.sy == 1 && a.sx == 1 &&
+         (long)a.Hs * a.Ws == (long)a.dHW.d && a.Ws == (int)a.dW.d && a.oH == a.Hs && a.oW == a.Ws;
+}
 
-    if (ntl > 0) {
-      stage_g(0);
-      if (ng > 1) stage_g(1);
-      int g = 0;
-      for (int i = 0; i < ntl; ++i) {
-        for (int kt = 0; kt < nk; ++kt) {
-          if (g + 1 < ng)
-            asm volatile("s_waitcnt vmcnt(%0)" ::"n"(2 * NIA) : "memory");
-          else
-            asm volatile("s_waitcnt vmcnt(0)" ::: "memory");
-          ws_barrier();
-          const int buf = g % NST;
-          Frag a0[TM], b0[TN], a1[TM], b1[TN];
-          frags(buf, 0, a0, b0);
-          if (g + 2 < ng) stage_g(g + 2);
-          frags(buf, 1, a1, b1);
-          mfmas(a0, b0);
-          frags(buf, 2, a0, b0);
-          mfmas(a1, b1);
-          frags(buf, 3, a1, b1);
-          mfmas(a0, b0);
-          mfmas(a1, b1);
-          ++g;
-        }
-        ws_barrier();
-#pragma unroll
-        for (int i2 = 0; i2 < TM; ++i2)
-#pragma unroll
-          for (int j = 0; j < TN; ++j)
-#pragma unroll
-            for (int r = 0; r < 16; ++r) {
-              const int row = wm * (BM / 2) + 32 * i2 + (r & 3) + 8 * (r >> 2) + 4 * hh;
-              stg[row * LDC + scol(row, wn * (BN / WN) + 32 * j + l31)] = acc[i2][j][r];
-              acc[i2][j][r] = 0.f;
-            }
-        ws_barrier();
-      }
-    }
-    ws_barrier();
-    ws_barrier();
-    return;
-  }
-
-  const int etid = tid - 64 * NW;
-  const int cg = etid % CG, rsub = etid / CG;
-  const int col = n0 + 8 * cg;
-  float mu[8], bsc[8], bsh[8], cs[8], cq[8];
-#pragma unroll
-  for (int e = 0; e < 8; ++e) {
-    mu[e] = a.bn_mean[col + e];
-    bsc[e] = MSK == 2 ? a.bn_sc[col + e] : 0.f;
-    bsh[e] = MSK == 2 ? a.bn_sh[col + e] : (MSK == 0 ? 1.f : 0.f);
-    cs[e] = 0.f;
-    cq[e] = 0.f;
-  }
-  const uint32_t span = G16 ? a.Cbytes / 2u : a.Cbytes / 4u;
-  constexpr uint32_t ey = BN16 ? 2u : 4u, eo = C16 ? 2u : 4u, ec = G16 ? 2u : 4u;
-  auto rsrc = [](const void* p, uint32_t bytes) {
-    return __builtin_amdgcn_make_buffer_rsrc(const_cast<void*>(p), (short)0, (int)bytes, 0x00020000);
-  };
-  const __amdgpu_buffer_rsrc_t rY = rsrc(a.bn_y, span * ey);
-  const __amdgpu_buffer_rsrc_t rZ = rsrc(a.bn_z ? (const void*)a.bn_z : (const void*)a.bn_y,
-                                         MSK == 3 ? (span + 31u) / 32u * 4u : span * ey);
-  const __amdgpu_buffer_rsrc_t rO = rsrc(a.Cold ? a.Cold : (const void*)a.C, span * eo);
-  const __amdgpu_buffer_rsrc_t rC = rsrc(a.C, span * ec);
-  auto ld16 = [](__amdgpu_buffer_rsrc_t r, uint32_t off) {
-    return __builtin_bit_cast(uint4, __builtin_amdgcn_raw_buffer_load_b128(r, off, 0, 0));
-  };
-  struct In {
-    uint4 y0, y1, z0, z1, c0, c1;
-    uint32_t bits;
-    uint32_t off;
-    bool ok;
-  };
-  In pf[NR];
-  auto issue = [&](int m0, int j, In& x, bool live) {
-    const int row = m0 + rsub + j * RPP;
-    x.ok = live && row < a.M;
-    x.off = (uint32_t)row * (uint32_t)a.ldc + (uint32_t)col;
-    const uint32_t o = x.off;
-    x.y0 = ld16(rY, x.ok ? o * ey : OOB);
-    if constexpr (!BN16) x.y1 = ld16(rY, x.ok ? o * ey + 16u : OOB);
-    if constexpr (MSK == 1) {
-      x.z0 = ld16(rZ, x.ok ? o * ey : OOB);
-      if constexpr (!BN16) x.z1 = ld16(rZ, x.ok ? o * ey + 16u : OOB);
-    }
-    if constexpr (MSK == 3)
-      x.bits = __builtin_amdgcn_raw_buffer_load_b32(rZ, x.ok ? (o >> 5) * 4u : OOB, 0, 0);
-    if constexpr (BETA != 0) {
-      x.c0 = ld16(rO, x.ok ? o * eo : OOB);
-      if constexpr (!C16) x.c1 = ld16(rO, x.ok ? o * eo + 16u : OOB);
-    }
-  };
-  auto consume = [&](const In& x, int j) {
-    float yv[8], zv[8], old[8];
-    if constexpr (BN16) {
-      const uint32_t yu[4] = {x.y0.x, x.y0.y, x.y0.z, x.y0.w};
-#pragma unroll
-      for (int e = 0; e < 4; ++e) {
-        yv[2 * e] = __uint_as_float(yu[e] << 16);
-        yv[2 * e + 1] = __uint_as_float(yu[e] & 0xffff0000u);
-      }
-      if constexpr (MSK == 1) {
-        const uint32_t zu[4] = {x.z0.x, x.z0.y, x.z0.z, x.z0.w};
-#pragma unroll
-        for (int e = 0; e < 4; ++e) {
-          zv[2 * e] = __uint_as_float(zu[e] << 16);
-          zv[2 * e + 1] = __uint_as_float(zu[e] & 0xffff0000u);
-        }
-      }
-    } else {
-      const uint32_t yu[8] = {x.y0.x, x.y0.y, x.y0.z, x.y0.w, x.y1.x, x.y1.y, x.y1.z, x.y1.w};
-#pragma unroll
-      for (int e = 0; e < 8; ++e) yv[e] = __uint_as_float(yu[e]);
-      if constexpr (MSK == 1) {
-        const uint32_t zu[8] = {x.z0.x, x.z0.y, x.z0.z, x.z0.w, x.z1.x, x.z1.y, x.z1.z, x.z1.w};
-#pragma unroll
-        for (int e = 0; e < 8; ++e) zv[e] = __uint_as_float(zu[e]);
-      }
-    }
-    if constexpr (MSK == 3) {
-      const uint32_t b8 = x.bits >> (x.off & 31u);
-#pragma unroll
-      for (int e = 0; e < 8; ++e) zv[e] = ((b8 >> e) & 1u) ? 1.f : 0.f;
-    } else if constexpr (MSK != 1) {
-#pragma unroll
-      for (int e = 0; e < 8; ++e) zv[e] = 0.f;
-    }
-    if constexpr (BETA != 0) {
-      unpack_old8(x.c0, x.c1, old, C16);
-    } else {
-#pragma unroll
-      for (int e = 0; e < 8; ++e) old[e] = 0.f;
-    }
-    const int rr = rsub + j * RPP;
-    const float* srow = stg + rr * LDC + scol(rr, 8 * cg);
-    const float4 a0 = *reinterpret_cast<const float4*>(srow);
-    const float4 a1 = *reinterpret_cast<const float4*>(srow + 4);
-    const float av[8] = {a0.x, a0.y, a0.z, a0.w, a1.x, a1.y, a1.z, a1.w};
-    float v[8];
-#pragma unroll
-    for (int e = 0; e < 8; ++e) {
-      float tv = fmaf(a.beta, old[e], av[e]);
-      const bool keep = zv[e] + fmaf(yv[e], bsc[e], bsh[e]) > 0.f;
-      tv = keep ? tv : 0.f;
-      if constexpr (G16) tv = bf16_rne(tv);
-      v[e] = tv;
-      const float s1 = cs[e] + tv, s2 = fmaf(tv, yv[e] - mu[e], cq[e]);
-      cs[e] = x.ok ? s1 : cs[e];
-      cq[e] = x.ok ? s2 : cq[e];
-    }
-    const uint32_t so = x.ok ? x.off * ec : OOB;
-    if constexpr (G16) {
-      uint32_t w[4];
-#pragma unroll
-      for (int e = 0; e < 4; ++e)
-        w[e] = (__float_as_uint(v[2 * e]) >> 16) | (__float_as_uint(v[2 * e + 1]) & 0xffff0000u);
-      const u32x4_t q = {w[0], w[1], w[2], w[3]};
-      __builtin_amdgcn_raw_buffer_store_b128(q, rC, so, 0, 0);
-    } else {
-      const u32x4_t q0 = {__float_as_uint(v[0]), __float_as_uint(v[1]), __float_as_uint(v[2]),
-                          __float_as_uint(v[3])};
-      const u32x4_t q1 = {__float_as_uint(v[4]), __float_as_uint(v[5]), __float_as_uint(v[6]),
-                          __float_as_uint(v[7])};
-      __builtin_amdgcn_raw_buffer_store_b128(q0, rC, so, 0, 0);
-      __builtin_amdgcn_raw_buffer_store_b128(q1, rC, x.ok ? so + 16u : OOB, 0, 0);
-    }
-  };
-  float* red = nullptr;
-  auto put_red = [&](int gl) {
-    red = reinterpret_cast<float*>(smem + (gl % NST) * STAGE);
-#pragma unroll
-    for (int e = 0; e < 8; ++e) {
-      red[(rsub * BN + 8 * cg + e) * 2] = cs[e];
-      red[(rsub * BN + 8 * cg + e) * 2 + 1] = cq[e];
-      cs[e] = 0.f;
-      cq[e] = 0.f;
-    }
-  };
-  auto finalize = [&](int mi) {
-    if (etid < BN) {
-      float t0 = 0.f, t1 = 0.f;
-      for (int q = 0; q < RPP; ++q) {
-        t0 += red[(q * BN + etid) * 2];
-        t1 += red[(q * BN + etid) * 2 + 1];
-      }
-      a.bn_part[(long)mi * a.part_ld + n0 + etid] = make_float2(t0, t1);
-    }
-  };
-  if (ntl > 0) {
-#pragma unroll
-    for (int j = 0; j < NR; ++j) issue((mlo + ms) * BM, j, pf[j], true);
-    for (int kt = 0; kt < nk; ++kt) ws_barrier();
-    ws_barrier();
-    ws_barrier();
-    for (int i = 1; i <= ntl; ++i) {
-      const bool more = i < ntl;
-      const int m0 = (mlo + ms + i * mstr) * BM;
-      const int kg = more ? kpg : 0;
-#pragma unroll
-      for (int jj = 0; jj < NKC; ++jj) {
-        for (int u = 0; u < kg; ++u) ws_barrier();
-#pragma unroll
-        for (int r = 0; r < R; ++r) {
-          const int j = jj * R + r;
-          if constexpr (TMR_WS_EXP == 1) continue;
-          consume(pf[j], j);
-          __builtin_amdgcn_sched_barrier(0);
-          issue(m0, j, pf[j], more);
-          __builtin_amdgcn_sched_barrier(0);
-        }
-      }
-      ws_barrier();
-      put_red(more ? (i + 1) * nk - 1 : i * nk - 1);
-      ws_barrier();
-      finalize(mlo + ms + (i - 1) * mstr);
-    }
-  } else {
-    ws_barrier();
-    ws_barrier();
-  }
-
+template <int F32>
+bool dgrad_ws_shape(const GemmArgs& a, int cfg) {
+  static const int on = env_int("TMR_DGRAD_WS", TMR_DGRAD_WS);
+  if (!on || a.io_tiles || a.bn_part == nullptr) return false;
+  if (kCfgs16[cfg].bm != 128) return false;
+  if (!dgrad_rows_identity(a)) return false;
+  if (a.N % 128 != 0 || (WS_NWG / 8) % (a.N / 128) != 0) return false;
+  constexpr int bk = F32 ? 32 : 64;
+  if (a.K <= 0 || a.K % bk != 0) return false;
+  if (cdiv(a.M, 128) * (long)(a.N / 128) < 2L * WS_NWG) return false;
+  return true;
 }
 
 template <int F32>
 int launch_dgrad_ws(const GemmArgs& a, int cfg, hipStream_t st) {
-  static const int on = env_int("TMR_DGRAD_WS", TMR_DGRAD_WS);
-  if (!on || a.io_tiles || a.bn_part == nullptr) return -1;
-  if (kCfgs16[cfg].bm != 128) return -1;
-  if (a.ntaps != 1 || a.osy != 1 || a.osx != 1 || a.oyc != 0 || a.oxc != 0 || a.oy0 != 0 ||
-      a.ox0 != 0 || a.wr0 != 0 || a.ws0 != 0 || a.sy != 1 || a.sx != 1 ||
-      (long)a.Hs * a.Ws != (long)a.dHW.d || a.Ws != (int)a.dW.d || a.oH != a.Hs || a.oW != a.Ws)
-    return -1;
-  if (a.N % 128 != 0 || (WS_NWG / 8) % (a.N / 128) != 0) return -1;
+  if (!dgrad_ws_shape<F32>(a, cfg)) return -1;
   constexpr int bk = F32 ? 32 : 64;
-  if (a.K <= 0 || a.K % bk != 0) return -1;
   const int nk = a.K / bk;
-  if (cdiv(a.M, 128) * (long)(a.N / 128) < 2L * WS_NWG) return -1;
   const bool beta1 = a.beta == 1.f;
   const dim3 grid(WS_NWG), blk(512);
   auto go = [&](auto kern) {
diff --git a/tmrnet_amd/csrc/gemm16_ws_body.h b/tmrnet_amd/csrc/gemm16_ws_body.h
--- /dev/null
+++ b/tmrnet_amd/csrc/gemm16_ws_body.h
@@ -0,0 +1,338 @@
+  static_assert(!OSP || (F32 != 0 && MSK == 3 && BETA != 0), "the parity-sparse old gradient's form");
+  constexpr bool BN16 = !F32, C16 = !F32, G16 = !F32;
+  constexpr int BM = 128, BN = 128, NW = 4, WN = 2;
+  constexpr uint32_t ES = F32 ? 4u : 2u;
+  constexpr int EPC = 16 / ES, BK = 128 / ES;
+  constexpr int TM = 2, TN = 2;
+  constexpr int ABYTES = BM * 128, STAGE = 2 * ABYTES;
+  constexpr int NIA = ABYTES / (1024 * NW);
+  constexpr int NST = 3;
+  constexpr int LDC = BN;
+  constexpr int STG = BM * LDC * 4;
+  constexpr int CG = BN / 8, RPP = 256 / CG, NR = BM / RPP;
+  constexpr int R = NR / NKC;
+  static_assert(NR == 8 && R * NKC == NR, "consumer row groups");
+  static_assert(RPP * BN * 8 <= STAGE, "the partial sums fit a stage");
+  using Frag = typename std::conditional<F32 != 0, f32x4_t, bf16x8>::type;
+  __shared__ __attribute__((aligned(1024))) unsigned char smem[NST * STAGE + STG];
+  float* const stg = reinterpret_cast<float*>(smem + NST * STAGE);
+  auto scol = [](int row, int c) { return c ^ (((row >> 2) & 1) << 5); };
+
+  const int tid = threadIdx.x;
+  const int wave = __builtin_amdgcn_readfirstlane(tid >> 6);
+  const int nnt = a.N / BN;
+  const int mt = (a.M + BM - 1) / BM;
+  const int xcd = blockIdx.x & 7, slot = blockIdx.x >> 3;
+  const int mlo = (int)((long)mt * xcd / 8), mhi = (int)((long)mt * (xcd + 1) / 8);
+  const int nt = slot % nnt, ms = slot / nnt, mstr = (WS_NWG / 8) / nnt;
+  const int ntl = mhi - mlo > ms ? (mhi - mlo - ms + mstr - 1) / mstr : 0;
+  const int n0 = nt * BN;
+  const int nk = (a.K + BK - 1) / BK;
+  const int kpg = nk / NKC;
+
+  if (wave < NW) {
+    const int lane = tid & 63;
+    const int wm = wave / WN, wn = wave % WN;
+    const int l31 = lane & 31, hh = lane >> 5;
+    const __amdgpu_buffer_rsrc_t rA = make_rsrc(a.A, a.Abytes);
+    const __amdgpu_buffer_rsrc_t rB = make_rsrc(a.B, a.Bbytes);
+    int prow[NIA], pch[NIA];
+    uint32_t boff[NIA];
+#pragma unroll
+    for (int q = 0; q < NIA; ++q) {
+      prow[q] = 8 * (wave + NW * q) + (lane >> 3);
+      pch[q] = EPC * ((lane & 7) ^ ((prow[q] >> 1) & 7));
+      boff[q] = (uint32_t)(n0 + prow[q]) * (uint32_t)a.ldbt * ES + (uint32_t)pch[q] * ES;
+    }
+    auto stage_q = [&](int m0, int kt, int buf, int q) {
+      const int kb = kt * BK;
+      unsigned char* As = smem + buf * STAGE;
+      unsigned char* Bs = As + ABYTES;
+      const int m = m0 + prow[q];
+      const bool ok = m < a.M && kb + pch[q] < a.K;
+      const uint32_t off = (uint32_t)m * (uint32_t)a.lds * ES + (uint32_t)(kb + pch[q]) * ES;
+      glds16(rA, As + 1024 * (wave + NW * q), ok ? off : OOB);
+      const bool okb = kb + pch[q] < a.K;
+      glds16(rB, Bs + 1024 * (wave + NW * q), okb ? boff[q] + (uint32_t)kb * ES : OOB);
+    };
+    auto stage = [&](int m0, int kt, int buf) {
+#pragma unroll
+      for (int q = 0; q < NIA; ++q) stage_q(m0, kt, buf, q);
+    };
+    const int kx = (l31 >> 1) & 7;
+    const int arow0 = wm * (BM / 2) + l31;
+    const int brow0 = wn * (BN / WN) + l31;
+    auto frags = [&](int buf, int s, Frag (&av)[TM], Frag (&bv)[TN]) {
+      const unsigned char* As = smem + buf * STAGE;
+      const unsigned char* Bs = As + ABYTES;
+      const int ch = (2 * s + hh) ^ kx;
+#pragma unroll
+      for (int i = 0; i < TM; ++i)
+        av[i] = *reinterpret_cast<const Frag*>(As + (arow0 + 32 * i) * 128 + (ch << 4));
+#pragma unroll
+      for (int j = 0; j < TN; ++j)
+        bv[j] = *reinterpret_cast<const Frag*>(Bs + (brow0 + 32 * j) * 128 + (ch << 4));
+    };
+    floatx16 acc[TM][TN];
+#pragma unroll
+    for (int i = 0; i < TM; ++i)
+#pragma unroll
+      for (int j = 0; j < TN; ++j)
+#pragma unroll
+        for (int r = 0; r < 16; ++r) acc[i][j][r] = 0.f;
+    auto mfmas = [&](const Frag (&av)[TM], const Frag (&bv)[TN]) {
+      if constexpr (TMR_WS_EXP == 2) {
+        asm volatile("" ::"v"(av[0]), "v"(bv[0]), "v"(av[TM - 1]), "v"(bv[TN - 1]));
+        return;
+      }
+      __builtin_amdgcn_s_setprio(1);
+      if constexpr (F32) {
+#pragma unroll
+        for (int t = 0; t < 4; ++t)
+#pragma unroll
+          for (int i = 0; i < TM; ++i)
+#pragma unroll
+            for (int j = 0; j < TN; ++j)
+              acc[i][j] = __builtin_amdgcn_mfma_f32_32x32x2f32(av[i][t], bv[j][t], acc[i][j], 0, 0, 0);
+      } else {
+#pragma unroll
+        for (int i = 0; i < TM; ++i)
+#pragma unroll
+          for (int j = 0; j < TN; ++j)
+            acc[i][j] = __builtin_amdgcn_mfma_f32_32x32x16_bf16(av[i], bv[j], acc[i][j], 0, 0, 0);
+      }
+      __builtin_amdgcn_s_setprio(0);
+    };
+    const int ng = ntl * nk;
+    auto stage_g = [&](int G) {
+      const int ti = G / nk;
+      stage((mlo + ms + ti * mstr) * BM, G - ti * nk, G % NST);
+    };
+
+    if (ntl > 0) {
+      stage_g(0);
+      if (ng > 1) stage_g(1);
+      int g = 0;
+      for (int i = 0; i < ntl; ++i) {
+        for (int kt = 0; kt < nk; ++kt) {
+          if (g + 1 < ng)
+            asm volatile("s_waitcnt vmcnt(%0)" ::"n"(2 * NIA) : "memory");
+          else
+            asm volatile("s_waitcnt vmcnt(0)" ::: "memory");
+          ws_barrier();
+          const int buf = g % NST;
+          Frag a0[TM], b0[TN], a1[TM], b1[TN];
+          frags(buf, 0, a0, b0);
+          if (g + 2 < ng) stage_g(g + 2);
+          frags(buf, 1, a1, b1);
+          mfmas(a0, b0);
+          frags(buf, 2, a0, b0);
+          mfmas(a1, b1);
+          frags(buf, 3, a1, b1);
+          mfmas(a0, b0);
+          mfmas(a1, b1);
+          ++g;
+        }
+        ws_barrier();
+#pragma unroll
+        for (int i2 = 0; i2 < TM; ++i2)
+#pragma unroll
+          for (int j = 0; j < TN; ++j)
+#pragma unroll
+            for (int r = 0; r < 16; ++r) {
+              const int row = wm * (BM / 2) + 32 * i2 + (r & 3) + 8 * (r >> 2) + 4 * hh;
+              stg[row * LDC + scol(row, wn * (BN / WN) + 32 * j + l31)] = acc[i2][j][r];
+              acc[i2][j][r] = 0.f;
+            }
+        ws_barrier();
+      }
+    }
+    ws_barrier();
+    ws_barrier();
+    return;
+  }
+
+  const int etid = tid - 64 * NW;
+  const int cg = etid % CG, rsub = etid / CG;
+  const int col = n0 + 8 * cg;
+  float mu[8], bsc[8], bsh[8], cs[8], cq[8];
+#pragma unroll
+  for (int e = 0; e < 8; ++e) {
+    mu[e] = a.bn_mean[col + e];
+    bsc[e] = MSK == 2 ? a.bn_sc[col + e] : 0.f;
+    bsh[e] = MSK == 2 ? a.bn_sh[col + e] : (MSK == 0 ? 1.f : 0.f);
+    cs[e] = 0.f;
+    cq[e] = 0.f;
+  }
+  const uint32_t span = G16 ? a.Cbytes / 2u : a.Cbytes / 4u;
+  constexpr uint32_t ey = BN16 ? 2u : 4u, eo = C16 ? 2u : 4u, ec = G16 ? 2u : 4u;
+  auto rsrc = [](const void* p, uint32_t bytes) {
+    return __builtin_amdgcn_make_buffer_rsrc(const_cast<void*>(p), (short)0, (int)bytes, 0x00020000);
+  };
+  const __amdgpu_buffer_rsrc_t rY = rsrc(a.bn_y, span * ey);
+  const __amdgpu_buffer_rsrc_t rZ = rsrc(a.bn_z ? (const void*)a.bn_z : (const void*)a.bn_y,
+                                         MSK == 3 ? (span + 31u) / 32u * 4u : span * ey);
+  const __amdgpu_buffer_rsrc_t rO = rsrc(a.Cold ? a.Cold : (const void*)a.C, OSP ? span : span * eo);
+  const __amdgpu_buffer_rsrc_t rC = rsrc(a.C, span * ec);
+  auto ld16 = [](__amdgpu_buffer_rsrc_t r, uint32_t off) {
+    return __builtin_bit_cast(uint4, __builtin_amdgcn_raw_buffer_load_b128(r, off, 0, 0));
+  };
+  struct In {
+    uint4 y0, y1, z0, z1, c0, c1;
+    uint32_t bits;
+    uint32_t off;
+    bool ok;
+  };
+  In pf[NR];
+  auto issue = [&](int m0, int j, In& x, bool live) {
+    const int row = m0 + rsub + j * RPP;
+    x.ok = live && row < a.M;
+    x.off = (uint32_t)row * (uint32_t)a.ldc + (uint32_t)col;
+    const uint32_t o = x.off;
+    x.y0 = ld16(rY, x.ok ? o * ey : OOB);
+    if constexpr (!BN16) x.y1 = ld16(rY, x.ok ? o * ey + 16u : OOB);
+    if constexpr (MSK == 1) {
+      x.z0 = ld16(rZ, x.ok ? o * ey : OOB);
+      if constexpr (!BN16) x.z1 = ld16(rZ, x.ok ? o * ey + 16u : OOB);
+    }
+    if constexpr (MSK == 3)
+      x.bits = __builtin_amdgcn_raw_buffer_load_b32(rZ, x.ok ? (o >> 5) * 4u : OOB, 0, 0);
+    if constexpr (OSP) {
+      uint32_t drow;
+      const bool tap = old_compact_row(a, (uint32_t)row, drow) && x.ok;
+      const uint32_t od = (drow * (uint32_t)a.ldc + (uint32_t)col) * 4u;
+      x.c0 = ld16(rO, tap ? od : OOB);
+      x.c1 = ld16(rO, tap ? od + 16u : OOB);
+    } else if constexpr (BETA != 0) {
+      x.c0 = ld16(rO, x.ok ? o * eo : OOB);
+      if constexpr (!C16) x.c1 = ld16(rO, x.ok ? o * eo + 16u : OOB);
+    }
+  };
+  auto consume = [&](const In& x, int j) {
+    float yv[8], zv[8], old[8];
+    if constexpr (BN16) {
+      const uint32_t yu[4] = {x.y0.x, x.y0.y, x.y0.z, x.y0.w};
+#pragma unroll
+      for (int e = 0; e < 4; ++e) {
+        yv[2 * e] = __uint_as_float(yu[e] << 16);
+        yv[2 * e + 1] = __uint_as_float(yu[e] & 0xffff0000u);
+      }
+      if constexpr (MSK == 1) {
+        const uint32_t zu[4] = {x.z0.x, x.z0.y, x.z0.z, x.z0.w};
+#pragma unroll
+        for (int e = 0; e < 4; ++e) {
+          zv[2 * e] = __uint_as_float(zu[e] << 16);
+          zv[2 * e + 1] = __uint_as_float(zu[e] & 0xffff0000u);
+        }
+      }
+    } else {
+      const uint32_t yu[8] = {x.y0.x, x.y0.y, x.y0.z, x.y0.w, x.y1.x, x.y1.y, x.y1.z, x.y1.w};
+#pragma unroll
+      for (int e = 0; e < 8; ++e) yv[e] = __uint_as_float(yu[e]);
+      if constexpr (MSK == 1) {
+        const uint32_t zu[8] = {x.z0.x, x.z0.y, x.z0.z, x.z0.w, x.z1.x, x.z1.y, x.z1.z, x.z1.w};
+#pragma unroll
+        for (int e = 0; e < 8; ++e) zv[e] = __uint_as_float(zu[e]);
+      }
+    }
+    if constexpr (MSK == 3) {
+      const uint32_t b8 = x.bits >> (x.off & 31u);
+#pragma unroll
+      for (int e = 0; e < 8; ++e) zv[e] = ((b8 >> e) & 1u) ? 1.f : 0.f;
+    } else if constexpr (MSK != 1) {
+#pragma unroll
+      for (int e = 0; e < 8; ++e) zv[e] = 0.f;
+    }
+    if constexpr (BETA != 0) {
+      unpack_old8(x.c0, x.c1, old, C16);
+    } else {
+#pragma unroll
+      for (int e = 0; e < 8; ++e) old[e] = 0.f;
+    }
+    const int rr = rsub + j * RPP;
+    const float* srow = stg + rr * LDC + scol(rr, 8 * cg);
+    const float4 a0 = *reinterpret_cast<const float4*>(srow);
+    const float4 a1 = *reinterpret_cast<const float4*>(srow + 4);
+    const float av[8] = {a0.x, a0.y, a0.z, a0.w, a1.x, a1.y, a1.z, a1.w};
+    float v[8];
+#pragma unroll
+    for (int e = 0; e < 8; ++e) {
+      float tv = fmaf(a.beta, old[e], av[e]);
+      const bool keep = zv[e] + fmaf(yv[e], bsc[e], bsh[e]) > 0.f;
+      tv = keep ? tv : 0.f;
+      if constexpr (G16) tv = bf16_rne(tv);
+      v[e] = tv;
+      const float s1 = cs[e] + tv, s2 = fmaf(tv, yv[e] - mu[e], cq[e]);
+      cs[e] = x.ok ? s1 : cs[e];
+      cq[e] = x.ok ? s2 : cq[e];
+    }
+    const uint32_t so = x.ok ? x.off * ec : OOB;
+    if constexpr (G16) {
+      uint32_t w[4];
+#pragma unroll
+      for (int e = 0; e < 4; ++e)
+        w[e] = (__float_as_uint(v[2 * e]) >> 16) | (__float_as_uint(v[2 * e + 1]) & 0xffff0000u);
+      const u32x4_t q = {w[0], w[1], w[2], w[3]};
+      __builtin_amdgcn_raw_buffer_store_b128(q, rC, so, 0, 0);
+    } else {
+      const u32x4_t q0 = {__float_as_uint(v[0]), __float_as_uint(v[1]), __float_as_uint(v[2]),
+                          __float_as_uint(v[3])};
+      const u32x4_t q1 = {__float_as_uint(v[4]), __float_as_uint(v[5]), __float_as_uint(v[6]),
+                          __float_as_uint(v[7])};
+      __builtin_amdgcn_raw_buffer_store_b128(q0, rC, so, 0, 0);
+      __builtin_amdgcn_raw_buffer_store_b128(q1, rC, x.ok ? so + 16u : OOB, 0, 0);
+    }
+  };
+  float* red = nullptr;
+  auto put_red = [&](int gl) {
+    red = reinterpret_cast<float*>(smem + (gl % NST) * STAGE);
+#pragma unroll
+    for (int e = 0; e < 8; ++e) {
+      red[(rsub * BN + 8 * cg + e) * 2] = cs[e];
+      red[(rsub * BN + 8 * cg + e) * 2 + 1] = cq[e];
+      cs[e] = 0.f;
+      cq[e] = 0.f;
+    }
+  };
+  auto finalize = [&](int mi) {
+    if (etid < BN) {
+      float t0 = 0.f, t1 = 0.f;
+      for (int q = 0; q < RPP; ++q) {
+        t0 += red[(q * BN + etid) * 2];
+        t1 += red[(q * BN + etid) * 2 + 1];
+      }
+      a.bn_part[(long)mi * a.part_ld + n0 + etid] = make_float2(t0, t1);
+    }
+  };
+  if (ntl > 0) {
+#pragma unroll
+    for (int j = 0; j < NR; ++j) issue((mlo + ms) * BM, j, pf[j], true);
+    for (int kt = 0; kt < nk; ++kt) ws_barrier();
+    ws_barrier();
+    ws_barrier();
+    for (int i = 1; i <= ntl; ++i) {
+      const bool more = i < ntl;
+      const int m0 = (mlo + ms + i * mstr) * BM;
+      const int kg = more ? kpg : 0;
+#pragma unroll
+      for (int jj = 0; jj < NKC; ++jj) {
+        for (int u = 0; u < kg; ++u) ws_barrier();
+#pragma unroll
+        for (int r = 0; r < R; ++r) {
+          const int j = jj * R + r;
+          if constexpr (TMR_WS_EXP == 1) continue;
+          consume(pf[j], j);
+          __builtin_amdgcn_sched_barrier(0);
+          issue(m0, j, pf[j], more);
+          __builtin_amdgcn_sched_barrier(0);
+        }
+      }
+      ws_barrier();
+      put_red(more ? (i + 1) * nk - 1 : i * nk - 1);
+      ws_barrier();
+      finalize(mlo + ms + (i - 1) * mstr);
+    }
+  } else {
+    ws_barrier();
+    ws_barrier();
+  }
diff --git a/tmrnet_amd/csrc/gemm_conv.hip b/tmrnet_amd/csrc/gemm_conv.hip
--- a/tmrnet_amd/csrc/gemm_conv.hip
+++ b/tmrnet_amd/csrc/gemm_conv.hip
@@ -302,6 +302,7 @@
   int part_ld;
   const void* old;
   int old16;
+  int oldc;
 };
 
 static void tile_of(const GemmArgs& a, int mode, tmr_conv_tile* t) {
@@ -410,7 +411,8 @@
         pend_al[npend++] = al;
         continue;
       }
-      const int rc = launch_gemm<MODE_DGRAD>(a, al, 1, stream);
+      const int rc = fz && fz->oldc ? launch_gemm16_dgrad_oldc(a, stream)
+                                    : launch_gemm<MODE_DGRAD>(a, al, 1, stream);
       if (rc) return rc;
     }
   }
@@ -436,7 +438,7 @@
     s.y = adv(fz.y, px, esz_bn(d));
     s.z = fz.mask == 3 ? (const float*)((const uint32_t*)fz.z + px / 32) : adv(fz.z, px, esz_bn(d));
     s.sc = adv(fz.sc, o, 4); s.sh = adv(fz.sh, o, 4); s.mean = adv(fz.mean, o, 4);
-    s.old = adv(fz.old, px, fz.old16 ? 2 : 4);
+    s.old = fz.oldc ? adv(fz.old, px / 4, 4) : adv(fz.old, px, fz.old16 ? 2 : 4);
     s.part = part;
     s.nparts = 0;
     const int rc = conv_dgrad_impl(&c, adv(dy, y_off(c, g, f0), esz_dy(d)), adv(w_krsc, w_off(c, g), esz_w(d)),
@@ -527,6 +529,77 @@
                 "output (TMR_IO_G16) on the bf16 LDS-DMA engine (TMR_IO_WT_BF16)");
   return dgrad_bnbwd_entry(d, dy, w_krsc, (float*)dx, beta, dx_old, old_bf16 ? 1 : 0, y, z, scale,
                            shift, mean, mask, parts, parts_bytes, stream);
+}
+
+static const char* dgrad_oldc_why(const tmr_conv_desc* d, const void* dx, const void* old_compact,
+                                  size_t old_bytes, float beta, int mask) {
+  if (d->n <= 0 || d->k <= 0 || d->c <= 0 || d->h <= 0 || d->w <= 0) return "empty descriptor";
+  if (d->math != TMR_MATH_F32) return "fp32 math only";
+  if ((d->io & ~(TMR_IO_ENGINE | TMR_IO_CLASSES | TMR_IO_TILES)) != TMR_IO_WT_F32)
+    return "fp32 transposed weights (TMR_IO_WT_F32) only";
+  if (ngroups(d) > 1) return "grouped conv";
+  if (d->r != 1 || d->s != 1 || d->stride != 1 || d->pad != 0 || d->pad_w != 0 || d->ho != d->h ||
+      d->wo != d->w)
+    return "a 1x1 stride-1 unpadded conv only";
+  if ((d->h & 1) || (d->w & 1)) return "odd height or width";
+  if (beta != 1.f) return "beta must be 1";
+  if (mask != 3) return "ReLU-mask bits (mask 3) only";
+  if (xld_of(d) != d->c) return "dx must be dense";
+  if (ilog2_exact(d->k) < 2 || yld_of(d) % 4 != 0) return "dy channels: a power of two >= 4, 16-B rows";
+  if (d->c % 8 != 0 || ((long)d->h * d->w * d->c) % 32 != 0) return "dx channels: a multiple of 8";
+  if ((((uintptr_t)dx | (uintptr_t)old_compact) & 15) != 0) return "operands must be 16-B aligned";
+  const size_t dbytes = (size_t)d->n * (d->h / 2) * (d->w / 2) * d->c * sizeof(float);
+  if (old_bytes != dbytes) return "old_compact must hold n*(h/2)*(w/2)*c floats";
+  if (dx && old_compact) {
+    const char *a = (const char*)dx, *b = (const char*)old_compact;
+    if (!(a + 4 * dbytes <= b || b + dbytes <= a)) return "old_compact overlaps dx";
+  }
+  const char* why = nullptr;
+  for_slices(d, [&](const tmr_conv_desc& c, int, int) {
+    if (!dgrad_oldc_cfg(pick_cfg16((long)c.n * c.h * c.w, c.c, c.k, MODE_DGRAD, true)))
+      why = "tile config without the compact-old form";
+    return 0;
+  }, true);
+  return why;
+}
+
+TMR_API int tmr_conv2d_dgrad_bnbwd_oldc_ok(const tmr_conv_desc* d, const void* dx,
+                                           const void* old_compact, size_t old_bytes, float beta,
+                                           int mask) {
+  return d && !dgrad_oldc_why(d, dx, old_compact, old_bytes, beta, mask) ? 1 : 0;
+}
+
+long tmrg::g_dgrad_oldc_launches = 0;
+TMR_API long tmr_dgrad_oldc_launches(void) {
+  return __atomic_load_n(&g_dgrad_oldc_launches, __ATOMIC_RELAXED);
+}
+
+TMR_API int tmr_conv2d_dgrad_bnbwd_oldc(const tmr_conv_desc* d, const float* dy, const float* w_crsk,
+                                        float* dx, float beta, const float* old_compact,
+                                        size_t old_bytes, const float* y, const void* zbits,
+                                        const float* mean, int mask, void* parts, size_t parts_bytes,
+                                        hipStream_t stream) {
+  TMR_CHECK_ARG(d && dy && w_crsk && dx && old_compact && y && zbits && mean && parts,
+                "tmr_conv2d_dgrad_bnbwd_oldc: null operand");
+  const char* why = dgrad_oldc_why(d, dx, old_compact, old_bytes, beta, mask);
+  TMR_CHECK_ARG(!why, "tmr_conv2d_dgrad_bnbwd_oldc: not served (%s); ask "
+                "tmr_conv2d_dgrad_bnbwd_oldc_ok and keep the dense old dx", why);
+  TMR_CHECK_ARG(((((uintptr_t)dy | (uintptr_t)w_crsk | (uintptr_t)y)) & 15) == 0 &&
+                    ((uintptr_t)zbits & 3) == 0,
+                "tmr_conv2d_dgrad_bnbwd_oldc: dy, weights and y must be 16-B aligned");
+  const int np = tmr_conv2d_dgrad_bnbwd_parts(d);
+  TMR_CHECK_ARG(np >= 0 && parts_bytes >= (size_t)np * d->c * sizeof(float2),
+                "tmr_conv2d_dgrad_bnbwd_oldc: parts buffer too small");
+  BnBwdFuse fz{};
+  fz.y = y; fz.z = (const float*)zbits; fz.mean = mean; fz.mask = 3;
+  fz.part = (float2*)parts;
+  fz.part_ld = d->c;
+  fz.old = old_compact;
+  fz.oldc = 1;
+  const int rc = dgrad_bnbwd_run(d, dy, w_crsk, dx, 1.f, fz, nullptr, stream);
+  if (rc) return rc;
+  __atomic_fetch_add(&g_dgrad_oldc_launches, 1L, __ATOMIC_RELAXED);
+  return 0;
 }
 
 TMR_API int tmr_conv2d_dgrad(const tmr_conv_desc* d, const float* dy, const float* w_krsc,
diff --git a/tmrnet_amd/ops.py b/tmrnet_amd/ops.py
--- a/tmrnet_amd/ops.py
+++ b/tmrnet_amd/ops.py
@@ -339,6 +339,52 @@
     return out, parts, nparts
 
 
+def _oldc_desc(dy, w_crsk, in_hw):
+    n, ho, wo, k = dy.shape
+    k2, r, s, c = _dgrad_w(w_crsk, True)
+    h, w = in_hw
+    d = conv_desc(n, h, w, c, k, r, s, 1, 0, math="fp32", io=_io(None, w_crsk, dy, True))
+    d.y_ld = _nhwc_ld(dy, "dy")
+    return d, (n, h, w, c, k, r, s)
+
+
+def conv_dgrad_bnbwd_oldc_ok(dy, w_crsk, in_hw, old_compact, mask=3, beta=1.0, out=None):
+    if (dy.dtype != f32 or w_crsk.dtype != f32 or old_compact.dtype != f32
+            or not old_compact.is_contiguous() or w_crsk.dim() != 4
+            or tuple(w_crsk.shape[1:3]) != (1, 1) or tuple(dy.shape[1:3]) != tuple(in_hw)):
+        return False
+    d, _ = _oldc_desc(dy, w_crsk, in_hw)
+    return bool(query("tmr_conv2d_dgrad_bnbwd_oldc_ok", ctypes.byref(d), out, old_compact,
+                      ctypes.c_size_t(old_compact.numel() * 4), float(beta), int(mask)))
+
+
+def conv_dgrad_bnbwd_oldc_plan_ok(n, h, w, c, k):
+    d = conv_desc(n, h, w, c, k, 1, 1, 1, 0, math="fp32", io=IO_WT32)
+    return bool(query("tmr_conv2d_dgrad_bnbwd_oldc_ok", ctypes.byref(d), None, None,
+                      ctypes.c_size_t(n * (h // 2) * (w // 2) * c * 4), 1.0, 3))
+
+
+def conv_dgrad_bnbwd_oldc(dy, w_crsk, in_hw, y, mean, zbits, old_compact, mask=3, beta=1.0):
+    _req_op(w_crsk, "w"); _req(y, "y"); _req(mean, "mean"); _req(old_compact, "old_compact")
+    if zbits is None or zbits.dtype != torch.int32 or zbits.numel() * 32 < y.numel():
+        raise RuntimeError("conv_dgrad_bnbwd_oldc: takes the int32 ReLU-mask bits of y's shape")
+    d, (n, h, w, c, k, r, s) = _oldc_desc(dy, w_crsk, in_hw)
+    if tuple(y.shape) != (n, h, w, c):
+        raise RuntimeError("conv_dgrad_bnbwd_oldc: y must have dx's shape %s" % ((n, h, w, c),))
+    out = _empty((n, h, w, c), dy)
+    nparts = query("tmr_conv2d_dgrad_bnbwd_parts", ctypes.byref(d))
+    if nparts < 0:
+        raise RuntimeError("tmr_conv2d_dgrad_bnbwd_parts failed")
+    parts = torch.empty((max(nparts, 1), c, 2), dtype=f32, device=dy.device)
+    with _prof("conv_dgrad", 2.0 * n * h * w * k * c, (n, h, w, c, k, r, 1),
+               4 * n * h * w * k + 4 * w_crsk.numel() + 4 * n * h * w * c * 2
+               + n * h * w * c // 8 + 4 * old_compact.numel()):
+        call("tmr_conv2d_dgrad_bnbwd_oldc", ctypes.byref(d), dy, w_crsk, out, float(beta),
+             old_compact, ctypes.c_size_t(old_compact.numel() * 4), y, zbits, mean, int(mask),
+             parts, ctypes.c_size_t(parts.numel() * 4), stream_ptr())
+    return out, parts, nparts
+
+
 def bn_bwd_maxpool(dyp, am, y, scale, shift, mean, inv, gamma, bf16=False):
     n, h, w, c = y.shape
     _, ho, wo, _ = dyp.shape
diff --git a/tmrnet_amd/trunk.py b/tmrnet_amd/trunk.py
--- a/tmrnet_amd/trunk.py
+++ b/tmrnet_amd/trunk.py
@@ -75,6 +75,28 @@
 
 WGRAD_BNBWD_DS = True
 WGRAD_BNBWD_DS_MIN = 8_000_000
+
+
+DS_OLD_COMPACT = True
+DS_OLD_COMPACT_MIN = 250_000_000
+
+
+def _ds_old_compact(g, rd, r1, prev3):
+    if not (DS_OLD_COMPACT and prev3 is not None and g.dtype == torch.float32):
+        return False
+    for rec, st in ((rd, 2), (r1, 1)):
+        wt = rec.get("wt")
+        if (rec["math"] != "fp32" or rec.get("groups", 1) != 1 or rec["stride"] != st
+                or rec["pad"] != 0 or tuple(rec["conv"].weight.shape[2:]) != (1, 1)
+                or wt is None or wt.dtype != torch.float32):
+            return False
+    py = prev3["y"]
+    if not (prev3["relu"] and prev3.get("zbits") is not None and py.dtype == torch.float32
+            and rd["x"].shape == py.shape and r1["x"].shape == py.shape):
+        return False
+    n, h, w, c = py.shape
+    return (py.numel() >= DS_OLD_COMPACT_MIN
+            and ops.conv_dgrad_bnbwd_oldc_plan_ok(n, h, w, c, r1["conv"].weight.shape[0]))
 
 
 def _ds_fold(g, r3, rd):
@@ -210,7 +232,7 @@
 
 def _conv_bn_bwd(rec, dz, grads, want_dres=False, dx_out=None, dx_beta=0.0, need_dx=True,
                  dres_inplace=False, parts=None, fuse_prev=None, pool=None, dy=None, g16=False,
-                 r16=False, fold=False, gcoef=None):
+                 r16=False, fold=False, gcoef=None, compact_dx=False, old_compact=None):
     conv, bn = rec["conv"], rec["bn"]
     s16 = rec.get("dy16", False) or _store16(rec["math"])
     dy_given = dy is not None or gcoef is not None
@@ -274,12 +296,20 @@
             old = None
             if rb and dx_out.dtype != torch.bfloat16:
                 old, dx_out = dx_out, None
-            dx, pp, npp = ops.conv_dgrad_bnbwd(dy, wdg, hw, rec["stride"], rec["pad"],
-                                               p["y"], p["mean"], mask, z=zm,
-                                               scale=p["scale"], shift=p["shift"], out=dx_out,
-                                               beta=dx_beta, math=rec["math"],
-                                               wt=wt, groups=grp, g16=gb or rb, old=old)
+            if old_compact is not None:
+                if mask != 3 or dx_out is not None or gb or rb:
+                    raise RuntimeError("a compact old dx takes the fp32 mask-bits conv1 dgrad only")
+                dx, pp, npp = ops.conv_dgrad_bnbwd_oldc(dy, wdg, hw, p["y"], p["mean"], zm,
+                                                        old_compact)
+            else:
+                dx, pp, npp = ops.conv_dgrad_bnbwd(dy, wdg, hw, rec["stride"], rec["pad"],
+                                                   p["y"], p["mean"], mask, z=zm,
+                                                   scale=p["scale"], shift=p["shift"], out=dx_out,
+                                                   beta=dx_beta, math=rec["math"],
+                                                   wt=wt, groups=grp, g16=gb or rb, old=old)
             fused = (pp, npp)
+        elif compact_dx:
+            dx = ops.conv_dgrad(dy, wdg, (dy.shape[1], dy.shape[2]), 1, 0, math=rec["math"], wt=wt)
         else:
             dx = ops.conv_dgrad(dy, wdg, hw, rec["stride"], rec["pad"], out=dx_out,
                                 beta=dx_beta, math=rec["math"], wt=wt, groups=grp)
@@ -420,13 +450,19 @@
                                       fold=True)
             del dz2
             if has_ds:
+                oc = _ds_old_compact(g, rd, r1, prev3)
                 if dyd is not None or gcd is not None:
-                    dx, _, _ = _conv_bn_bwd(rd, None, grads, dy=dyd, gcoef=gcd)
+                    dx, _, _ = _conv_bn_bwd(rd, None, grads, dy=dyd, gcoef=gcd, compact_dx=oc)
                     del dyd, gcd
                 else:
-                    dx, _, _ = _conv_bn_bwd(rd, dres, grads)
-                dx, _, pending = _conv_bn_bwd(r1, dz1, grads, parts=fz1, dx_out=dx, dx_beta=1.0,
-                                              fuse_prev=prev3, r16=True, fold=True)
+                    dx, _, _ = _conv_bn_bwd(rd, dres, grads, compact_dx=oc)
+                if oc:
+                    dx, _, pending = _conv_bn_bwd(r1, dz1, grads, parts=fz1, old_compact=dx,
+                                                  fuse_prev=prev3, fold=True)
+                else:
+                    dx, _, pending = _conv_bn_bwd(r1, dz1, grads, parts=fz1, dx_out=dx,
+                                                  dx_beta=1.0, fuse_prev=prev3, r16=True,
+                                                  fold=True)
             else:
                 dx, _, pending = _conv_bn_bwd(r1, dz1, grads, parts=fz1, dx_out=dres, dx_beta=1.0,
                                               fuse_prev=prev3, r16=True, fold=True)
```
